# ray-project/anyscale-workshop-nyc-2023

Hardware: NVIDIA H100
Metric: generated tokens/sec (and prompts/sec) FLAN-T5-base 512->128 (higher is better)
Workload: dtype bf16

## Files before the change

### anyscale_workshop_nyc_2023_b200/csrc/b200t5.cu

```cuda
#include <cuda.h>
#include <cuda_bf16.h>
#include <cuda_fp16.h>
#include <cuda_runtime.h>
#include <math.h>
#include <stdarg.h>
#include <stdio.h>
#include <string.h>

#include <map>
#include <memory>
#include <string>
#include <vector>

#include "../../include/b200t5.h"
#include "attention_decode.cuh"
#include "attention_cross_stream.cuh"
#include "attention_encoder.cuh"
#include "elementwise.cuh"
#include "gemm.cuh"
#include "gemm_splitk.cuh"
#include "gemm_2cta.cuh"

using namespace b200;

static thread_local char g_err[512] = "";
static void set_gerr(const char* fmt, ...) {
  va_list ap;
  va_start(ap, fmt);
  vsnprintf(g_err, sizeof(g_err), fmt, ap);
  va_end(ap);
}

struct b200t5_ctx;
static int fail(b200t5_ctx* h, int code, const char* fmt, ...);

#define CU_OK(h, expr)                                                                         \
  do {                                                                                         \
    cudaError_t _e = (expr);                                                                   \
    if (_e != cudaSuccess)                                                                     \
      return fail(h, B200T5_ECUDA, "%s failed: %s (%s:%d)", #expr, cudaGetErrorString(_e), __FILE__, __LINE__); \
  } while (0)

typedef CUresult (*PFN_encodeTiled)(CUtensorMap*, CUtensorMapDataType, cuuint32_t, void*, const cuuint64_t*,
                                    const cuuint64_t*, const cuuint32_t*, const cuuint32_t*, CUtensorMapInterleave,
                                    CUtensorMapSwizzle, CUtensorMapL2promotion, CUtensorMapFloatOOBfill);
static PFN_encodeTiled get_encode_fn() {
  static PFN_encodeTiled fn = nullptr;
  if (!fn) {
    void* p = nullptr;
    cudaDriverEntryPointQueryResult q;
    if (cudaGetDriverEntryPoint("cuTensorMapEncodeTiled", &p, cudaEnableDefault, &q) == cudaSuccess &&
        q == cudaDriverEntryPointSuccess)
      fn = reinterpret_cast<PFN_encodeTiled>(p);
  }
  return fn;
}
static bool make_tmap(CUtensorMap* tm, const void* base, uint64_t rows, uint64_t cols, uint32_t box_rows, bool f32 = false) {
  PFN_encodeTiled enc = get_encode_fn();
  if (!enc) {
    set_gerr("cuTensorMapEncodeTiled entry point not available");
    return false;
  }
  cuuint64_t dims[2] = {cols, rows};
  cuuint64_t strides[1] = {cols * (f32 ? 4u : 2u)};
  cuuint32_t box[2] = {f32 ? 32u : 64u, box_rows};
  cuuint32_t estr[2] = {1, 1};
  const CUtensorMapDataType dt = f32 ? CU_TENSOR_MAP_DATA_TYPE_FLOAT32
                                     : (B200T5_F16 ? CU_TENSOR_MAP_DATA_TYPE_FLOAT16 : CU_TENSOR_MAP_DATA_TYPE_BFLOAT16);
  CUresult r = enc(tm, dt, 2, const_cast<void*>(base), dims, strides, box, estr,
                   CU_TENSOR_MAP_INTERLEAVE_NONE, CU_TENSOR_MAP_SWIZZLE_128B, CU_TENSOR_MAP_L2_PROMOTION_L2_256B,
                   CU_TENSOR_MAP_FLOAT_OOB_FILL_NONE);
  if (r != CUDA_SUCCESS) {
    set_gerr("cuTensorMapEncodeTiled failed with %d (rows=%llu cols=%llu box_rows=%u base=%p)", (int)r,
             (unsigned long long)rows, (unsigned long long)cols, box_rows, base);
    return false;
  }
  return true;
}

DEVINL float load_as_float(const void* src, int dtype, size_t i) {
  if (dtype == B200T5_DTYPE_F32) return reinterpret_cast<const float*>(src)[i];
  if (dtype == B200T5_DTYPE_F16) return __half2float(reinterpret_cast<const __half*>(src)[i]);
  return __bfloat162float(reinterpret_cast<const __nv_bfloat16*>(src)[i]);
}
__global__ void convert_to_act_kernel(const void* src, int dtype, act_t* dst, size_t n) {
  size_t i = blockIdx.x * static_cast<size_t>(blockDim.x) + threadIdx.x;
  const size_t stride = static_cast<size_t>(gridDim.x) * blockDim.x;
  for (; i < n; i += stride) dst[i] = float2act(load_as_float(src, dtype, i));
}
#if B200T5_F16
__global__ void convert_to_f32_kernel(const void* src, int dtype, float* dst, size_t n) {
  size_t i = blockIdx.x * static_cast<size_t>(blockDim.x) + threadIdx.x;
  const size_t stride = static_cast<size_t>(gridDim.x) * blockDim.x;
  for (; i < n; i += stride) dst[i] = load_as_float(src, dtype, i);
}
DEVINL float tf32_rn(float x) {
  uint32_t u = __float_as_uint(x);
  u += 0x0FFFu + ((u >> 13) & 1u);
  return __uint_as_float(u & 0xFFFFE000u);
}
__global__ void split_tf32_kernel(const float* __restrict__ w, float* __restrict__ out, int rows, int K, int Kp) {
  size_t i = blockIdx.x * static_cast<size_t>(blockDim.x) + threadIdx.x;
  const size_t n = static_cast<size_t>(rows) * Kp;
  if (i >= n) return;
  const int r = static_cast<int>(i / Kp), k = static_cast<int>(i % Kp);
  const float v = k < K ? w[static_cast<size_t>(r) * K + k] : 0.f;
  const float hi = tf32_rn(v);
  out[static_cast<size_t>(r) * 2 * Kp + k] = hi;
  out[static_cast<size_t>(r) * 2 * Kp + Kp + k] = tf32_rn(v - hi);
}
#endif
__global__ void geglu_elementwise_kernel(const act_t* gate, const act_t* up, act_t* out, long long n, int mode, GeluLut lut) {
  long long i = blockIdx.x * static_cast<long long>(blockDim.x) + threadIdx.x;
  if (i >= n) return;
  const float x = act2float(gate[i]);
  const float g = mode == 0 ? gelu_from_lut(x, lut.table, lut.lo, lut.hi) : gelu_new_act_exact(x, mode == 1 ? 1 : 0);
  out[i] = float2act(g * act2float(up[i]));
}
__global__ void build_gelu_table_kernel(uint16_t* full, int pow_mode) {
  const uint32_t bits = blockIdx.x * blockDim.x + threadIdx.x;
  if (bits >= 65536u) return;
  const float g = gelu_new_act_exact(__uint_as_float(bits << 16), pow_mode);
  full[bits] = static_cast<uint16_t>(__float_as_uint(g) >> 16);
}
__global__ void set_state_kernel(DecodeState* st, int step) {
  st->step = step;
  st->finished_rows = 0;
}

struct Cfg {
  int V, d, F, H, I, Le, Ld, nb, maxdist;
  float eps;
  int pad, eos, start;
};

struct DevBuf {
  void* p = nullptr;
  size_t bytes = 0;
  ~DevBuf() {
    if (p) cudaFree(p);
  }
  DevBuf() = default;
  DevBuf(const DevBuf&) = delete;
  DevBuf& operator=(const DevBuf&) = delete;
  DevBuf(DevBuf&& o) noexcept : p(o.p), bytes(o.bytes) {
    o.p = nullptr;
    o.bytes = 0;
  }
  cudaError_t alloc(size_t n) {
    if (p) cudaFree(p);
    p = nullptr;
    bytes = n;
    return cudaMalloc(&p, n ? n : 16);
  }
  template <class T>
  T* as() const {
    return reinterpret_cast<T*>(p);
  }
};

enum GemmKind { G_STORE256, G_RES256, G_GEGLU256, G_CROSSKV256, G_QKVDEC64, G_STORE32, G_RES32, G_GEGLU64, G_ARGMAX128, G_LOGITS128 };

struct GemmOp {
  CUtensorMap tmA, tmB;
  int M = 0, N = 0, K = 0;
  GemmKind kind = G_STORE256;
  int m_fastest = 0;
};

struct EncLayerW {
  DevBuf ln0, ln1, wqkv, wo, wi, wff_o;
  CUtensorMap tm_qkv, tm_o, tm_wi, tm_ffo;
  CUtensorMap tm2_qkv, tm2_o, tm2_wi, tm2_ffo;
};
struct DecLayerW {
  DevBuf ln0, ln1, ln2, wqkv, wo, wcq, wco, wi, wff_o;
  CUtensorMap tm_qkv, tm_o, tm_cq, tm_co, tm_wi, tm_ffo;
  int wi_rows = 0;
};

constexpr int kMaxChains = 8;
constexpr int kStepsPerGraph = 8;

struct Plan {
  int B = 0, S = 0, Tmax = 0;
  DevBuf x, xn, qkv, ctx, hff;
  DevBuf key_ok, extent, enc_bias;
  DevBuf cu, row_b, row_s;
  int* h_cu = nullptr;
  int packed_rows = 0;
  bool packed = false;
  DevBuf cross_kv;
  DevBuf dx, dxn, dq, dctx, dh;
  DevBuf self_kv;
  DevBuf dec_bias;
  DevBuf pval, pidx;
  DevBuf state, unfinished, out_ids, out_len, ids_dev, mask_dev;
  DevBuf live_extent, live_key_ok;
  DevBuf xs_stamps, xs_acc;
  DevBuf pos, out_row, admit;
  DevBuf stream_out, stream_len;
  size_t stream_cap = 0;
  bool stream_mode = false;
  int g_stream = -1;
  int g_xattn = -1;
  bool xattn_stream = false;
  long long rows_valid = 0;
  int* h_unf = nullptr;
  int* h_admit = nullptr;
  int n_vtiles = 0;
  CUtensorMap tm_xn, tm_ctx, tm_hff;
  CUtensorMap tm_cross_kv;
  struct Chain {
    int b0 = 0, nb = 0;
    CUtensorMap tm_dxn, tm_dctx, tm_dh;
  };
  int n_chains = 1;
  Chain chains[kMaxChains];
  cudaGraph_t graph = nullptr;
  cudaGraphExec_t gexec = nullptr;
  int graph_nodes = 0;
  cudaGraph_t graph8 = nullptr;
  cudaGraphExec_t gexec8 = nullptr;
  long long g_eos = -1, g_pad = -1;
  int g_min_new = -1;
  long long* h_ids = nullptr;
  long long* h_mask = nullptr;
  long long* h_out = nullptr;
  int* h_len = nullptr;
  DecodeState* h_state = nullptr;
  ~Plan() {
    if (gexec) cudaGraphExecDestroy(gexec);
    if (graph) cudaGraphDestroy(graph);
    if (gexec8) cudaGraphExecDestroy(gexec8);
    if (graph8) cudaGraphDestroy(graph8);
    if (h_ids) cudaFreeHost(h_ids);
    if (h_mask) cudaFreeHost(h_mask);
    if (h_out) cudaFreeHost(h_out);
    if (h_len) cudaFreeHost(h_len);
    if (h_state) cudaFreeHost(h_state);
    if (h_cu) cudaFreeHost(h_cu);
    if (h_unf) cudaFreeHost(h_unf);
    if (h_admit) cudaFreeHost(h_admit);
  }
};

struct b200t5_ctx {
  Cfg c;
  int device = 0;
  int num_sms = 132;
  bool finalized = false;
  int ffo_k = 0;
  char err[512] = "";
  std::map<std::string, std::unique_ptr<DevBuf>> raw;
  std::map<std::string, std::unique_ptr<DevBuf>> raw_f32;
  std::map<std::string, std::vector<int64_t>> raw_shape;
  DevBuf shared, lm_head, enc_final_ln, dec_final_ln, enc_relbias, dec_relbias, wcrosskv;
  CUtensorMap tm_lm, tm_crosskv, tm2_crosskv;
  std::vector<float> enc_relbias_h, dec_relbias_h;
  std::vector<EncLayerW> enc;
  std::vector<DecLayerW> dec;
  std::unique_ptr<Plan> plan;
  cudaStream_t cap_stream = nullptr, exec_stream = nullptr, enc_stream = nullptr;
  cudaEvent_t enc_done_ev = nullptr, admitted_ev = nullptr;
  bool admit_overlap = true;
  cudaEvent_t ev[4] = {nullptr, nullptr, nullptr, nullptr};
  bool ev_valid = false;
  int pow_mode = 0;
  bool use_pdl = true;
  GeluLut gelu_lut{nullptr, 0, 0};
  struct SkChoice {
    int bn, split;
  };
  bool pack_rows = true;
  bool use_2cta = true;
  bool self_block = true;
  int xattn_mode = 2;
  int xs_stages = 5;
  bool xs_late_pdl = true;
  bool xs_l2_prefetch = false;
  bool xattn_serialize = false;
  std::vector<cudaEvent_t> xattn_ev;
  bool profile_xattn = false;
  int small_prio = 0;
  bool sk_on = true;
  int sk_stages64 = 0, sk_stages128 = 0;
  SkChoice sk_qkv{64, 2}, sk_proj{64, 4}, sk_wi{128, 2}, sk_ffo{64, 4};
  int chains_override = 0;
  cudaStream_t chain_streams[kMaxChains] = {};
  cudaEvent_t chain_ev[kMaxChains + 1] = {};
  int64_t launches = 0;
  int last_steps = 0;
  double last_decode_bytes = 0, last_enc_flops = 0;
};

static int fail(b200t5_ctx* h, int code, const char* fmt, ...) {
  char buf[512];
  va_list ap;
  va_start(ap, fmt);
  vsnprintf(buf, sizeof(buf), fmt, ap);
  va_end(ap);
  if (h) snprintf(h->err, sizeof(h->err), "%s", buf);
  snprintf(g_err, sizeof(g_err), "%s", buf);
  return code;
}

static int check_device(b200t5_ctx* h, int device) {
  int n = 0;
  cudaError_t e = cudaGetDeviceCount(&n);
  if (e != cudaSuccess || n <= 0)
    return fail(h, B200T5_ENODEV, "no CUDA device available (%s); libb200t5 has no CPU fallback",
                e == cudaSuccess ? "count=0" : cudaGetErrorString(e));
  if (device < 0 || device >= n) return fail(h, B200T5_EINVAL, "device %d out of range (%d devices)", device, n);
  cudaDeviceProp p;
  CU_OK(h, cudaGetDeviceProperties(&p, device));
  if (p.major != 9)
    return fail(h, B200T5_ENODEV, "device %d is sm_%d%d; libb200t5 is built for sm_90a only", device, p.major, p.minor);
  CU_OK(h, cudaSetDevice(device));
  return p.multiProcessorCount;
}

extern "C" int b200t5_relative_bucket(int rel, int bidirectional, int num_buckets, int max_distance) {
  int ret = 0, n;
  if (bidirectional) {
    num_buckets /= 2;
    if (rel > 0) ret += num_buckets;
    n = rel < 0 ? -rel : rel;
  } else {
    n = rel < 0 ? -rel : 0;
  }
  const int max_exact = num_buckets / 2;
  if (n < max_exact) return ret + n;
  const float ratio = static_cast<float>(n) / static_cast<float>(max_exact);
  const float denom = static_cast<float>(log(static_cast<double>(max_distance) / static_cast<double>(max_exact)));
  const float scaled = logf(ratio) / denom * static_cast<float>(num_buckets - max_exact);
  int large = max_exact + static_cast<int>(scaled);
  if (large > num_buckets - 1) large = num_buckets - 1;
  return ret + large;
}

static cudaError_t run_gemm(b200t5_ctx* h, const GemmOp& g, const void* ep, cudaStream_t s, bool pdl = false) {
  h->launches++;
  switch (g.kind) {
    case G_STORE256:
      return launch_gemm<256, EpiStore>(g.tmA, g.tmB, g.M, g.N, g.K, g.m_fastest, *static_cast<const EpiStore::Params*>(ep), h->num_sms, s, pdl);
    case G_RES256:
      return launch_gemm<256, EpiResidual>(g.tmA, g.tmB, g.M, g.N, g.K, g.m_fastest, *static_cast<const EpiResidual::Params*>(ep), h->num_sms, s, pdl);
    case G_GEGLU256:
      return launch_gemm<256, EpiGeglu>(g.tmA, g.tmB, g.M, g.N, g.K, g.m_fastest, *static_cast<const EpiGeglu::Params*>(ep), h->num_sms, s, pdl);
    case G_CROSSKV256:
      return launch_gemm<256, EpiCrossKV>(g.tmA, g.tmB, g.M, g.N, g.K, g.m_fastest, *static_cast<const EpiCrossKV::Params*>(ep), h->num_sms, s, pdl);
    case G_QKVDEC64:
      return launch_gemm<64, EpiQkvDecode>(g.tmA, g.tmB, g.M, g.N, g.K, g.m_fastest, *static_cast<const EpiQkvDecode::Params*>(ep), h->num_sms, s, pdl);
    case G_STORE32:
      return launch_gemm<32, EpiStore>(g.tmA, g.tmB, g.M, g.N, g.K, g.m_fastest, *static_cast<const EpiStore::Params*>(ep), h->num_sms, s, pdl);
    case G_RES32:
      return launch_gemm<32, EpiResidual>(g.tmA, g.tmB, g.M, g.N, g.K, g.m_fastest, *static_cast<const EpiResidual::Params*>(ep), h->num_sms, s, pdl);
    case G_GEGLU64:
      return launch_gemm<64, EpiGeglu>(g.tmA, g.tmB, g.M, g.N, g.K, g.m_fastest, *static_cast<const EpiGeglu::Params*>(ep), h->num_sms, s, pdl);
    case G_ARGMAX128:
      return launch_gemm<128, EpiArgmax>(g.tmA, g.tmB, g.M, g.N, g.K, g.m_fastest, *static_cast<const EpiArgmax::Params*>(ep), h->num_sms, s, pdl);
    case G_LOGITS128:
      return launch_gemm<128, EpiStoreF32>(g.tmA, g.tmB, g.M, g.N, g.K, g.m_fastest, *static_cast<const EpiStoreF32::Params*>(ep), h->num_sms, s, pdl);
  }
  return cudaErrorInvalidValue;
}

template <class Epi>
static cudaError_t run_gemm_2cta(b200t5_ctx* h, const CUtensorMap& tmA, const CUtensorMap& tmB, int M, int N, int K,
                                 const typename Epi::Params& ep, cudaStream_t s) {
  h->launches++;
  return launch_gemm_2cta<Epi>(tmA, tmB, M, N, K, ep, h->num_sms, s);
}

template <class Epi>
static cudaError_t run_gemm_sk(b200t5_ctx* h, const b200t5_ctx::SkChoice& ch, const CUtensorMap& tmA,
                               const CUtensorMap& tmB, int M, int N, int K, const typename Epi::Params& ep,
                               cudaStream_t s, bool pdl) {
  h->launches++;
  const int split = splitk_factor(K, ch.split);
  if (ch.bn == 128) return launch_gemm_splitk<128, Epi>(tmA, tmB, M, N, K, split, ep, s, pdl, 0, h->sk_stages128);
  return launch_gemm_splitk<64, Epi>(tmA, tmB, M, N, K, split, ep, s, pdl, 0, h->sk_stages64);
}

static cudaError_t run_ffo_2cta(b200t5_ctx* h, const CUtensorMap& tmA, const CUtensorMap& tmB, int M, int N,
                                const EpiResidual::Params& ep, cudaStream_t s) {
  h->launches++;
  return launch_gemm_2cta<EpiResidual, B200T5_F16 != 0>(tmA, tmB, M, N, h->ffo_k, ep, h->num_sms, s, B200T5_F16 ? h->ffo_k / 64 : 0);
}
static cudaError_t run_ffo_sk(b200t5_ctx* h, const b200t5_ctx::SkChoice& ch, const CUtensorMap& tmA, const CUtensorMap& tmB,
                              int M, int N, const EpiResidual::Params& ep, cudaStream_t s, bool pdl) {
  h->launches++;
  constexpr bool tf = B200T5_F16 != 0;
  const int split = splitk_factor(h->ffo_k, ch.split, tf ? kBK / 2 : kBK);
  const int akb = tf ? h->ffo_k / 64 : 0;
  if (ch.bn == 128) return launch_gemm_splitk<128, EpiResidual, tf>(tmA, tmB, M, N, h->ffo_k, split, ep, s, pdl, akb, h->sk_stages128);
  return launch_gemm_splitk<64, EpiResidual, tf>(tmA, tmB, M, N, h->ffo_k, split, ep, s, pdl, akb, h->sk_stages64);
}

static cudaError_t run_rmsnorm(b200t5_ctx* h, const res_t* x, const act_t* w, act_t* y, int M, int d, float eps,
                               cudaStream_t s, bool pdl = false) {
  if (h) h->launches++;
  const int wpb = 8;
  const int grid = (M + wpb - 1) / wpb;
  if (d <= 1024) return launch_kernel(rmsnorm_kernel<4>, dim3(grid), dim3(wpb * 32), 0, s, pdl, x, w, y, M, d, eps);
  if (d <= 4096) return launch_kernel(rmsnorm_kernel<16>, dim3(grid), dim3(wpb * 32), 0, s, pdl, x, w, y, M, d, eps);
  return cudaErrorInvalidValue;
}

static cudaError_t init_kernel_attrs() {
  cudaError_t e;
#define PREP(BN, EPI)                         \
  if ((e = prepare_gemm<BN, EPI>()) != cudaSuccess) return e;
  PREP(256, EpiStore) PREP(256, EpiResidual) PREP(256, EpiGeglu) PREP(256, EpiCrossKV) PREP(64, EpiQkvDecode)
  PREP(32, EpiStore) PREP(32, EpiResidual) PREP(64, EpiGeglu) PREP(128, EpiArgmax) PREP(128, EpiStoreF32)
  PREP(64, EpiStore) PREP(128, EpiStore)
#undef PREP
  if ((e = prepare_gemm_2cta<EpiStore>()) != cudaSuccess) return e;
  if ((e = prepare_gemm_2cta<EpiResidual>()) != cudaSuccess) return e;
  if ((e = prepare_gemm_2cta<EpiGeglu>()) != cudaSuccess) return e;
  if ((e = prepare_gemm_2cta<EpiCrossKV>()) != cudaSuccess) return e;
#define PREPSK(BN, EPI) \
  if ((e = prepare_gemm_splitk<BN, EPI>()) != cudaSuccess) return e;
  PREPSK(64, EpiStore) PREPSK(128, EpiStore) PREPSK(64, EpiResidual) PREPSK(128, EpiResidual)
  PREPSK(64, EpiQkvDecode) PREPSK(128, EpiQkvDecode) PREPSK(64, EpiGeglu) PREPSK(128, EpiGeglu)
#undef PREPSK
  if ((e = prepare_gemm_2cta<EpiResidual, B200T5_F16 != 0>()) != cudaSuccess) return e;
  if ((e = prepare_gemm_splitk<64, EpiResidual, B200T5_F16 != 0>()) != cudaSuccess) return e;
  if ((e = prepare_gemm_splitk<128, EpiResidual, B200T5_F16 != 0>()) != cudaSuccess) return e;
  if ((e = cudaFuncSetAttribute(self_attn_decode_warp_kernel, cudaFuncAttributeMaxDynamicSharedMemorySize,
                                kSelfWarpsPerCta * 4096 * 4)) != cudaSuccess)
    return e;
  if ((e = cudaFuncSetAttribute(attn_cross_stream_kernel, cudaFuncAttributeMaxDynamicSharedMemorySize,
                                static_cast<int>(XsSmem::bytes(kXsMaxStages, 4096)))) != cudaSuccess)
    return e;
  return cudaFuncSetAttribute(encoder_attn_kernel, cudaFuncAttributeMaxDynamicSharedMemorySize, 96 * 1024);
}

struct GeluLutOwner {
  DevBuf table;
  GeluLut lut{nullptr, 0, 0};
  int pow_mode = -1;
};
static GeluLutOwner g_gelu;

[[maybe_unused]] static int ensure_gelu_lut(b200t5_ctx* h, int pow_mode, GeluLut* out) {
  if (g_gelu.lut.table && g_gelu.pow_mode == pow_mode) {
    *out = g_gelu.lut;
    return B200T5_OK;
  }
  DevBuf full;
  CU_OK(h, full.alloc(65536 * 2));
  build_gelu_table_kernel<<<256, 256>>>(full.as<uint16_t>(), pow_mode);
  CU_OK(h, cudaGetLastError());
  std::vector<uint16_t> t(65536);
  CU_OK(h, cudaMemcpy(t.data(), full.p, 65536 * 2, cudaMemcpyDeviceToHost));
  auto half_bits = [](uint16_t xb) {
    uint32_t u = static_cast<uint32_t>(xb) << 16;
    float f;
    memcpy(&f, &u, 4);
    f *= 0.5f;
    memcpy(&u, &f, 4);
    u += 0x7FFFu + ((u >> 16) & 1u);
    return static_cast<uint16_t>(u >> 16);
  };
  int lo = 0;
  while (lo < 0x7F80 && t[lo] == half_bits(static_cast<uint16_t>(lo)) && t[0x8000 | lo] == half_bits(static_cast<uint16_t>(0x8000 | lo))) ++lo;
  int hi = 0x7F80;
  while (hi > lo && t[hi - 1] == static_cast<uint16_t>(hi - 1) && t[0x8000 | (hi - 1)] == 0x8000) --hi;
  const int n = hi - lo;
  if (n < 0 || 2 * n * 2 > kEpiSmemBytes) return fail(h, B200T5_ECUDA, "gelu table window [%#x,%#x) does not fit the epilogue scratch", lo, hi);
  std::vector<uint16_t> compact(((static_cast<size_t>(2) * (n > 0 ? n : 1) + 7) / 8) * 8 + 8, 0);
  for (int i = 0; i < n; ++i) {
    compact[i] = t[lo + i];
    compact[n + i] = t[0x8000 | (lo + i)];
  }
  CU_OK(h, g_gelu.table.alloc(compact.size() * 2));
  CU_OK(h, cudaMemcpy(g_gelu.table.p, compact.data(), compact.size() * 2, cudaMemcpyHostToDevice));
  g_gelu.lut = GeluLut{g_gelu.table.as<uint16_t>(), lo, hi};
  g_gelu.pow_mode = pow_mode;
  *out = g_gelu.lut;
  return B200T5_OK;
}

extern "C" const char* b200t5_version(void) {
  return B200T5_F16 ? "b200t5 0.1 fp16 (sm_90a, wgmma/TMA)" : "b200t5 0.1 (sm_90a, wgmma/TMA)";
}
extern "C" const char* b200t5_last_global_error(void) { return g_err; }
extern "C" const char* b200t5_last_error(b200t5_handle h) { return h ? h->err : g_err; }

extern "C" int b200t5_create(const b200t5_config* cfg, int device, b200t5_handle* out) {
  if (!cfg || !out) return fail(nullptr, B200T5_EINVAL, "null argument");
  *out = nullptr;
  if (cfg->d_kv != 64) return fail(nullptr, B200T5_EINVAL, "d_kv=%d unsupported (kernels are specialised for 64)", cfg->d_kv);
  if (!cfg->is_gated_gelu) return fail(nullptr, B200T5_EINVAL, "only feed_forward_proj='gated-gelu' (T5 v1.1 / FLAN-T5) is supported");
  if (cfg->scale_decoder_outputs) return fail(nullptr, B200T5_EINVAL, "scale_decoder_outputs (tied-embedding T5 v1.0) is not supported");
  if (cfg->d_model % 8 || cfg->d_ff % 32 || cfg->d_model > 4096 || cfg->vocab_size < 2 || cfg->num_heads < 1 ||
      cfg->num_layers < 1 || cfg->num_decoder_layers < 1)
    return fail(nullptr, B200T5_EINVAL, "unsupported shape: d_model=%d d_ff=%d vocab=%d", cfg->d_model, cfg->d_ff, cfg->vocab_size);
  int sms = check_device(nullptr, device);
  if (sms < 0) return sms;
  b200t5_ctx* h = new (std::nothrow) b200t5_ctx();
  if (!h) return fail(nullptr, B200T5_ENOMEM, "out of host memory");
  h->c = Cfg{cfg->vocab_size, cfg->d_model, cfg->d_ff, cfg->num_heads, cfg->num_heads * 64, cfg->num_layers,
             cfg->num_decoder_layers, cfg->relative_attention_num_buckets, cfg->relative_attention_max_distance,
             cfg->layer_norm_epsilon, cfg->pad_token_id, cfg->eos_token_id, cfg->decoder_start_token_id};
  h->device = device;
  h->num_sms = sms;
  h->enc.resize(h->c.Le);
  h->dec.resize(h->c.Ld);
  const char* pm = getenv("B200T5_POW_MODE");
  h->pow_mode = pm ? atoi(pm) : 0;
  const char* pdl_env = getenv("B200T5_PDL");
  h->use_pdl = pdl_env ? atoi(pdl_env) != 0 : true;
  if (const char* pr_env = getenv("B200T5_PRIO")) h->small_prio = atoi(pr_env);
  if (const char* pk_env = getenv("B200T5_PACK")) h->pack_rows = atoi(pk_env) != 0;
  if (const char* tc_env = getenv("B200T5_2CTA")) h->use_2cta = atoi(tc_env) != 0;
  if (const char* sf_env = getenv("B200T5_SELF")) h->self_block = strcmp(sf_env, "warp") != 0;
  if (const char* xa_env = getenv("B200T5_XATTN")) h->xattn_mode = strcmp(xa_env, "ldg") == 0 ? 0 : strcmp(xa_env, "stream") == 0 ? 1 : 2;
  if (const char* xs_env = getenv("B200T5_XS_STAGES")) {
    const int v = atoi(xs_env);
    if (v >= 2 && v <= kXsMaxStages) h->xs_stages = v;
  }
  if (const char* lp_env = getenv("B200T5_XS_LATE_PDL")) h->xs_late_pdl = atoi(lp_env) != 0;
  if (const char* se_env = getenv("B200T5_XS_SERIALIZE")) h->xattn_serialize = atoi(se_env) != 0;
  if (const char* pf_env = getenv("B200T5_XS_L2PF")) h->xs_l2_prefetch = atoi(pf_env) != 0;
  if (const char* sk_env = getenv("B200T5_SK")) {
    int v[8];
    const int n = sscanf(sk_env, "%d,%d,%d,%d,%d,%d,%d,%d", &v[0], &v[1], &v[2], &v[3], &v[4], &v[5], &v[6], &v[7]);
    if (n == 1 && v[0] == 0) h->sk_on = false;
    if (n == 8) {
      b200t5_ctx::SkChoice* dst[4] = {&h->sk_qkv, &h->sk_proj, &h->sk_wi, &h->sk_ffo};
      for (int i = 0; i < 4; ++i) {
        dst[i]->bn = v[2 * i] == 128 ? 128 : 64;
        dst[i]->split = v[2 * i + 1] >= 8 ? 8 : (v[2 * i + 1] >= 4 ? 4 : (v[2 * i + 1] >= 2 ? 2 : 1));
      }
    }
  }
  if (const char* st_env = getenv("B200T5_SK_STAGES")) {
    int a = 0, b = 0;
    if (sscanf(st_env, "%d,%d", &a, &b) == 2) {
      h->sk_stages64 = a;
      h->sk_stages128 = b;
    }
  }
  const char* ch_env = getenv("B200T5_CHAINS");
  h->chains_override = ch_env ? atoi(ch_env) : 0;
#if B200T5_F16
  h->use_2cta = h->pack_rows = true;
  if (!h->sk_on) {
    delete h;
    return fail(nullptr, B200T5_EINVAL, "B200T5_SK=0 is not available in the fp16 build");
  }
#endif
  if (const char* ao_env = getenv("B200T5_ADMIT_OVERLAP")) h->admit_overlap = atoi(ao_env) != 0;
  int prio_lo = 0, prio_hi = 0;
  cudaDeviceGetStreamPriorityRange(&prio_lo, &prio_hi);
  if (cudaStreamCreateWithFlags(&h->cap_stream, cudaStreamNonBlocking) != cudaSuccess ||
      cudaStreamCreateWithFlags(&h->exec_stream, cudaStreamNonBlocking) != cudaSuccess ||
      cudaStreamCreateWithPriority(&h->enc_stream, cudaStreamNonBlocking, prio_lo) != cudaSuccess ||
      cudaEventCreateWithFlags(&h->enc_done_ev, cudaEventDisableTiming) != cudaSuccess ||
      cudaEventCreateWithFlags(&h->admitted_ev, cudaEventDisableTiming) != cudaSuccess) {
    delete h;
    return fail(nullptr, B200T5_ECUDA, "cudaStreamCreate failed");
  }
  {
    cudaError_t ke = init_kernel_attrs();
    if (ke != cudaSuccess) {
      delete h;
      return fail(nullptr, B200T5_ECUDA, "kernel attribute setup failed: %s", cudaGetErrorString(ke));
    }
  }
#if !B200T5_F16
  {
    int lrc = ensure_gelu_lut(nullptr, h->pow_mode, &h->gelu_lut);
    if (lrc != B200T5_OK) {
      delete h;
      return lrc;
    }
  }
#endif
  {
    cudaError_t ce = cudaSuccess;
    for (int i = 0; i < 4 && ce == cudaSuccess; ++i) ce = cudaEventCreate(&h->ev[i]);
    for (int i = 0; i < kMaxChains && ce == cudaSuccess; ++i) ce = cudaStreamCreateWithFlags(&h->chain_streams[i], cudaStreamNonBlocking);
    for (int i = 0; i <= kMaxChains && ce == cudaSuccess; ++i) ce = cudaEventCreateWithFlags(&h->chain_ev[i], cudaEventDisableTiming);
    if (ce != cudaSuccess) {
      b200t5_destroy(h);
      return fail(nullptr, B200T5_ECUDA, "stream/event creation failed: %s", cudaGetErrorString(ce));
    }
  }
  *out = h;
  return B200T5_OK;
}

extern "C" int b200t5_destroy(b200t5_handle h) {
  if (!h) return B200T5_OK;
  cudaSetDevice(h->device);
  cudaDeviceSynchronize();
  h->plan.reset();
  if (h->cap_stream) cudaStreamDestroy(h->cap_stream);
  if (h->exec_stream) cudaStreamDestroy(h->exec_stream);
  if (h->enc_stream) cudaStreamDestroy(h->enc_stream);
  if (h->enc_done_ev) cudaEventDestroy(h->enc_done_ev);
  if (h->admitted_ev) cudaEventDestroy(h->admitted_ev);
  for (int i = 0; i < kMaxChains; ++i)
    if (h->chain_streams[i]) cudaStreamDestroy(h->chain_streams[i]);
  for (int i = 0; i <= kMaxChains; ++i)
    if (h->chain_ev[i]) cudaEventDestroy(h->chain_ev[i]);
  for (cudaEvent_t e : h->xattn_ev)
    if (e) cudaEventDestroy(e);
  for (int i = 0; i < 4; ++i)
    if (h->ev[i]) cudaEventDestroy(h->ev[i]);
  delete h;
  return B200T5_OK;
}

extern "C" int b200t5_set_weight(b200t5_handle h, const char* name, const void* dev_ptr, int dtype,
                                 const int64_t* shape, int ndim) {
  if (!h || !name || !dev_ptr || !shape || ndim < 1 || ndim > 2) return fail(h, B200T5_EINVAL, "set_weight: bad argument");
  if (h->finalized) return fail(h, B200T5_ESTATE, "set_weight after finalize");
  if (dtype < 0 || dtype > 2) return fail(h, B200T5_EINVAL, "set_weight(%s): unknown dtype %d", name, dtype);
  CU_OK(h, cudaSetDevice(h->device));
  size_t n = 1;
  std::vector<int64_t> shp(shape, shape + ndim);
  for (int i = 0; i < ndim; ++i) {
    if (shape[i] <= 0) return fail(h, B200T5_EINVAL, "set_weight(%s): bad shape", name);
    n *= static_cast<size_t>(shape[i]);
  }
  std::unique_ptr<DevBuf> buf(new DevBuf());
  CU_OK(h, buf->alloc(n * sizeof(act_t)));
  if (dtype == (B200T5_F16 ? B200T5_DTYPE_F16 : B200T5_DTYPE_BF16)) {
    CU_OK(h, cudaMemcpy(buf->p, dev_ptr, n * sizeof(act_t), cudaMemcpyDeviceToDevice));
  } else {
    convert_to_act_kernel<<<1024, 256>>>(dev_ptr, dtype, buf->as<act_t>(), n);
    CU_OK(h, cudaGetLastError());
    CU_OK(h, cudaDeviceSynchronize());
  }
  h->raw[name] = std::move(buf);
  h->raw_shape[name] = shp;
#if B200T5_F16
  {
    const std::string nm(name);
    const std::string suffix = "DenseReluDense.wo.weight";
    if (nm.size() >= suffix.size() && nm.compare(nm.size() - suffix.size(), suffix.size(), suffix) == 0) {
      std::unique_ptr<DevBuf> f(new DevBuf());
      CU_OK(h, f->alloc(n * 4));
      convert_to_f32_kernel<<<1024, 256>>>(dev_ptr, dtype, f->as<float>(), n);
      CU_OK(h, cudaGetLastError());
      CU_OK(h, cudaDeviceSynchronize());
      h->raw_f32[nm] = std::move(f);
    }
  }
#endif
  return B200T5_OK;
}

static act_t* take(b200t5_ctx* h, const std::string& name, int64_t r, int64_t c, int* rc) {
  auto it = h->raw.find(name);
  if (it == h->raw.end()) {
    *rc = fail(h, B200T5_ESTATE, "finalize: missing weight '%s'", name.c_str());
    return nullptr;
  }
  const auto& s = h->raw_shape[name];
  const bool ok = (c == 0) ? (s.size() == 1 && s[0] == r) : (s.size() == 2 && s[0] == r && s[1] == c);
  if (!ok) {
    *rc = fail(h, B200T5_EINVAL, "finalize: weight '%s' has the wrong shape", name.c_str());
    return nullptr;
  }
  return it->second->as<act_t>();
}

static int interleave_geglu(b200t5_ctx* h, const act_t* wi0, const act_t* wi1, DevBuf& dst, int F, int d, int bn,
                            int* rows_out) {
  const int half = bn / 2;
  const int ntiles = (F + half - 1) / half;
  CU_OK(h, dst.alloc(static_cast<size_t>(ntiles) * bn * d * sizeof(act_t)));
  CU_OK(h, cudaMemset(dst.p, 0, dst.bytes));
  for (int j = 0; j < ntiles; ++j) {
    const int rows = (j + 1) * half <= F ? half : F - j * half;
    act_t* base = dst.as<act_t>() + static_cast<size_t>(j) * bn * d;
    CU_OK(h, cudaMemcpy(base, wi0 + static_cast<size_t>(j) * half * d, static_cast<size_t>(rows) * d * sizeof(act_t), cudaMemcpyDeviceToDevice));
    CU_OK(h, cudaMemcpy(base + static_cast<size_t>(half) * d, wi1 + static_cast<size_t>(j) * half * d, static_cast<size_t>(rows) * d * sizeof(act_t), cudaMemcpyDeviceToDevice));
  }
  *rows_out = ntiles * bn;
  return B200T5_OK;
}

static int build_ffo(b200t5_ctx* h, DevBuf& dst, const std::string& name, const act_t* src2, int d, int F, int* k_cols) {
#if B200T5_F16
  auto it = h->raw_f32.find(name);
  if (it == h->raw_f32.end()) return fail(h, B200T5_ESTATE, "finalize: missing fp32 copy of '%s'", name.c_str());
  const int Fp = (F + 31) / 32 * 32;
  CU_OK(h, dst.alloc(static_cast<size_t>(d) * 2 * Fp * 4));
  const size_t n = static_cast<size_t>(d) * Fp;
  split_tf32_kernel<<<static_cast<unsigned>((n + 255) / 256), 256>>>(it->second->as<float>(), dst.as<float>(), d, F, Fp);
  CU_OK(h, cudaGetLastError());
  CU_OK(h, cudaDeviceSynchronize());
  *k_cols = 2 * Fp;
  (void)src2;
  return B200T5_OK;
#else
  *k_cols = F;
  CU_OK(h, dst.alloc(static_cast<size_t>(d) * F * sizeof(act_t)));
  CU_OK(h, cudaMemcpy(dst.p, src2, static_cast<size_t>(d) * F * sizeof(act_t), cudaMemcpyDeviceToDevice));
  return B200T5_OK;
#endif
}

static int clone_buf(b200t5_ctx* h, DevBuf& dst, const act_t* src, size_t n) {
  CU_OK(h, dst.alloc(n * sizeof(act_t)));
  CU_OK(h, cudaMemcpy(dst.p, src, n * sizeof(act_t), cudaMemcpyDeviceToDevice));
  return B200T5_OK;
}

#define TRY(expr)            \
  do {                       \
    int _rc = (expr);        \
    if (_rc != B200T5_OK) return _rc; \
  } while (0)
#define TMAP(h, tm, base, rows, cols, box) \
  do {                                     \
    if (!make_tmap(tm, base, rows, cols, box)) return fail(h, B200T5_ECUDA, "%s", g_err); \
  } while (0)
#define TMAP_FFO(h, tm, base, rows, cols, box) \
  do {                                         \
    if (!make_tmap(tm, base, rows, cols, box, B200T5_F16 != 0)) return fail(h, B200T5_ECUDA, "%s", g_err); \
  } while (0)

extern "C" int b200t5_finalize(b200t5_handle h) {
  if (!h) return fail(nullptr, B200T5_EINVAL, "null handle");
  if (h->finalized) return B200T5_OK;
  CU_OK(h, cudaSetDevice(h->device));
  const Cfg& c = h->c;
  int rc = B200T5_OK;
  const int d = c.d, I = c.I, F = c.F;

  act_t* shared = take(h, "shared.weight", c.V, d, &rc);
  if (!shared) return rc;
  TRY(clone_buf(h, h->shared, shared, static_cast<size_t>(c.V) * d));
  const act_t* lm = h->raw.count("lm_head.weight") ? take(h, "lm_head.weight", c.V, d, &rc) : shared;
  if (!lm) return rc;
  TRY(clone_buf(h, h->lm_head, lm, static_cast<size_t>(c.V) * d));
  TMAP(h, &h->tm_lm, h->lm_head.p, c.V, d, 128);

  act_t* p;
  if (!(p = take(h, "encoder.final_layer_norm.weight", d, 0, &rc))) return rc;
  TRY(clone_buf(h, h->enc_final_ln, p, d));
  if (!(p = take(h, "decoder.final_layer_norm.weight", d, 0, &rc))) return rc;
  TRY(clone_buf(h, h->dec_final_ln, p, d));

  for (int side = 0; side < 2; ++side) {
    const std::string nm = std::string(side ? "decoder" : "encoder") + ".block.0.layer.0.SelfAttention.relative_attention_bias.weight";
    if (!(p = take(h, nm, c.nb, c.H, &rc))) return rc;
    std::vector<act_t> tmp(static_cast<size_t>(c.nb) * c.H);
    CU_OK(h, cudaMemcpy(tmp.data(), p, tmp.size() * sizeof(act_t), cudaMemcpyDeviceToHost));
    std::vector<float>& dst = side ? h->dec_relbias_h : h->enc_relbias_h;
    dst.resize(tmp.size());
    for (size_t i = 0; i < tmp.size(); ++i) dst[i] = act2float(tmp[i]);
  }

  char nm[256];
  for (int l = 0; l < c.Le; ++l) {
    EncLayerW& w = h->enc[l];
    auto key = [&](const char* suffix) {
      snprintf(nm, sizeof(nm), "encoder.block.%d.%s", l, suffix);
      return std::string(nm);
    };
    if (!(p = take(h, key("layer.0.layer_norm.weight"), d, 0, &rc))) return rc;
    TRY(clone_buf(h, w.ln0, p, d));
    if (!(p = take(h, key("layer.1.layer_norm.weight"), d, 0, &rc))) return rc;
    TRY(clone_buf(h, w.ln1, p, d));
    const act_t* q = take(h, key("layer.0.SelfAttention.q.weight"), I, d, &rc);
    const act_t* k = q ? take(h, key("layer.0.SelfAttention.k.weight"), I, d, &rc) : nullptr;
    const act_t* v = k ? take(h, key("layer.0.SelfAttention.v.weight"), I, d, &rc) : nullptr;
    if (!v) return rc;
    CU_OK(h, w.wqkv.alloc(static_cast<size_t>(3) * I * d * sizeof(act_t)));
    const size_t blk = static_cast<size_t>(I) * d;
    CU_OK(h, cudaMemcpy(w.wqkv.as<act_t>(), q, blk * 2, cudaMemcpyDeviceToDevice));
    CU_OK(h, cudaMemcpy(w.wqkv.as<act_t>() + blk, k, blk * 2, cudaMemcpyDeviceToDevice));
    CU_OK(h, cudaMemcpy(w.wqkv.as<act_t>() + 2 * blk, v, blk * 2, cudaMemcpyDeviceToDevice));
    if (!(p = take(h, key("layer.0.SelfAttention.o.weight"), d, I, &rc))) return rc;
    TRY(clone_buf(h, w.wo, p, static_cast<size_t>(d) * I));
    const act_t* wi0 = take(h, key("layer.1.DenseReluDense.wi_0.weight"), F, d, &rc);
    const act_t* wi1 = wi0 ? take(h, key("layer.1.DenseReluDense.wi_1.weight"), F, d, &rc) : nullptr;
    if (!wi1) return rc;
    int wi_rows = 0;
    TRY(interleave_geglu(h, wi0, wi1, w.wi, F, d, 256, &wi_rows));
    if (!(p = take(h, key("layer.1.DenseReluDense.wo.weight"), d, F, &rc))) return rc;
    TRY(build_ffo(h, w.wff_o, key("layer.1.DenseReluDense.wo.weight"), p, d, F, &h->ffo_k));
    TMAP(h, &w.tm_qkv, w.wqkv.p, 3 * I, d, 256);
    TMAP(h, &w.tm_o, w.wo.p, d, I, 256);
    TMAP(h, &w.tm_wi, w.wi.p, wi_rows, d, 256);
    TMAP_FFO(h, &w.tm_ffo, w.wff_o.p, d, h->ffo_k, 256);
    TMAP(h, &w.tm2_qkv, w.wqkv.p, 3 * I, d, 128);
    TMAP(h, &w.tm2_o, w.wo.p, d, I, 128);
    TMAP(h, &w.tm2_wi, w.wi.p, wi_rows, d, 128);
    TMAP_FFO(h, &w.tm2_ffo, w.wff_o.p, d, h->ffo_k, 128);
  }

  CU_OK(h, h->wcrosskv.alloc(static_cast<size_t>(c.Ld) * 2 * I * d * sizeof(act_t)));
  for (int l = 0; l < c.Ld; ++l) {
    DecLayerW& w = h->dec[l];
    auto key = [&](const char* suffix) {
      snprintf(nm, sizeof(nm), "decoder.block.%d.%s", l, suffix);
      return std::string(nm);
    };
    if (!(p = take(h, key("layer.0.layer_norm.weight"), d, 0, &rc))) return rc;
    TRY(clone_buf(h, w.ln0, p, d));
    if (!(p = take(h, key("layer.1.layer_norm.weight"), d, 0, &rc))) return rc;
    TRY(clone_buf(h, w.ln1, p, d));
    if (!(p = take(h, key("layer.2.layer_norm.weight"), d, 0, &rc))) return rc;
    TRY(clone_buf(h, w.ln2, p, d));
    const act_t* q = take(h, key("layer.0.SelfAttention.q.weight"), I, d, &rc);
    const act_t* k = q ? take(h, key("layer.0.SelfAttention.k.weight"), I, d, &rc) : nullptr;
    const act_t* v = k ? take(h, key("layer.0.SelfAttention.v.weight"), I, d, &rc) : nullptr;
    if (!v) return rc;
    const size_t blk = static_cast<size_t>(I) * d;
    CU_OK(h, w.wqkv.alloc(3 * blk * sizeof(act_t)));
    CU_OK(h, cudaMemcpy(w.wqkv.as<act_t>(), q, blk * 2, cudaMemcpyDeviceToDevice));
    CU_OK(h, cudaMemcpy(w.wqkv.as<act_t>() + blk, k, blk * 2, cudaMemcpyDeviceToDevice));
    CU_OK(h, cudaMemcpy(w.wqkv.as<act_t>() + 2 * blk, v, blk * 2, cudaMemcpyDeviceToDevice));
    if (!(p = take(h, key("layer.0.SelfAttention.o.weight"), d, I, &rc))) return rc;
    TRY(clone_buf(h, w.wo, p, static_cast<size_t>(d) * I));
    if (!(p = take(h, key("layer.1.EncDecAttention.q.weight"), I, d, &rc))) return rc;
    TRY(clone_buf(h, w.wcq, p, blk));
    const act_t* ck = take(h, key("layer.1.EncDecAttention.k.weight"), I, d, &rc);
    const act_t* cv = ck ? take(h, key("layer.1.EncDecAttention.v.weight"), I, d, &rc) : nullptr;
    if (!cv) return rc;
    CU_OK(h, cudaMemcpy(h->wcrosskv.as<act_t>() + (static_cast<size_t>(l) * 2 + 0) * blk, ck, blk * 2, cudaMemcpyDeviceToDevice));
    CU_OK(h, cudaMemcpy(h->wcrosskv.as<act_t>() + (static_cast<size_t>(l) * 2 + 1) * blk, cv, blk * 2, cudaMemcpyDeviceToDevice));
    if (!(p = take(h, key("layer.1.EncDecAttention.o.weight"), d, I, &rc))) return rc;
    TRY(clone_buf(h, w.wco, p, static_cast<size_t>(d) * I));
    const act_t* wi0 = take(h, key("layer.2.DenseReluDense.wi_0.weight"), F, d, &rc);
    const act_t* wi1 = wi0 ? take(h, key("layer.2.DenseReluDense.wi_1.weight"), F, d, &rc) : nullptr;
    if (!wi1) return rc;
    int wi_rows = 0;
    const int bn_qkv = h->sk_on ? h->sk_qkv.bn : 64, bn_proj = h->sk_on ? h->sk_proj.bn : 32;
    const int bn_wi = h->sk_on ? h->sk_wi.bn : 64, bn_ffo = h->sk_on ? h->sk_ffo.bn : 32;
    TRY(interleave_geglu(h, wi0, wi1, w.wi, F, d, bn_wi, &wi_rows));
    w.wi_rows = wi_rows;
    if (!(p = take(h, key("layer.2.DenseReluDense.wo.weight"), d, F, &rc))) return rc;
    TRY(build_ffo(h, w.wff_o, key("layer.2.DenseReluDense.wo.weight"), p, d, F, &h->ffo_k));
    TMAP(h, &w.tm_qkv, w.wqkv.p, 3 * I, d, bn_qkv);
    TMAP(h, &w.tm_o, w.wo.p, d, I, bn_proj);
    TMAP(h, &w.tm_cq, w.wcq.p, I, d, bn_proj);
    TMAP(h, &w.tm_co, w.wco.p, d, I, bn_proj);
    TMAP(h, &w.tm_wi, w.wi.p, wi_rows, d, bn_wi);
    TMAP_FFO(h, &w.tm_ffo, w.wff_o.p, d, h->ffo_k, bn_ffo);
  }
  TMAP(h, &h->tm_crosskv, h->wcrosskv.p, static_cast<uint64_t>(c.Ld) * 2 * I, d, 256);
  TMAP(h, &h->tm2_crosskv, h->wcrosskv.p, static_cast<uint64_t>(c.Ld) * 2 * I, d, 128);

  h->raw.clear();
  h->raw_f32.clear();
  h->raw_shape.clear();
  h->finalized = true;
  return B200T5_OK;
}


static int build_plan(b200t5_ctx* h, int B, int S, int Tmax) {
  const Cfg& c = h->c;
  std::unique_ptr<Plan> pl(new Plan());
  pl->B = B;
  pl->S = S;
  pl->Tmax = Tmax;
  const size_t M = static_cast<size_t>(B) * S;
  const int d = c.d, I = c.I, F = c.F, H = c.H;
  CU_OK(h, pl->x.alloc(M * d * sizeof(res_t)));
  CU_OK(h, pl->xn.alloc(M * d * 2));
  CU_OK(h, pl->qkv.alloc(M * 3 * I * 2));
  CU_OK(h, pl->ctx.alloc(M * I * 2));
  CU_OK(h, pl->hff.alloc(M * F * sizeof(ffh_t)));
  CU_OK(h, pl->key_ok.alloc(M));
  CU_OK(h, pl->extent.alloc(static_cast<size_t>(B) * 4));
  CU_OK(h, pl->cu.alloc(static_cast<size_t>(B + 1) * 4));
  CU_OK(h, pl->row_b.alloc(M * 4));
  CU_OK(h, pl->row_s.alloc(M * 4));
  CU_OK(h, cudaMallocHost(&pl->h_cu, 16));
  CU_OK(h, pl->cross_kv.alloc(static_cast<size_t>(c.Ld) * 2 * M * I * 2));
  CU_OK(h, cudaMemset(pl->cross_kv.p, 0, pl->cross_kv.bytes));
  CU_OK(h, pl->dx.alloc(static_cast<size_t>(B) * d * sizeof(res_t)));
  CU_OK(h, pl->dxn.alloc(static_cast<size_t>(B) * d * 2));
  CU_OK(h, pl->dq.alloc(static_cast<size_t>(B) * I * 2));
  CU_OK(h, pl->dctx.alloc(static_cast<size_t>(B) * I * 2));
  CU_OK(h, pl->dh.alloc(static_cast<size_t>(B) * F * sizeof(ffh_t)));
  CU_OK(h, pl->self_kv.alloc(static_cast<size_t>(c.Ld) * 2 * B * I * Tmax * 2));
  pl->n_vtiles = (c.V + 127) / 128;
  CU_OK(h, pl->pval.alloc(static_cast<size_t>(B) * pl->n_vtiles * 4));
  CU_OK(h, pl->pidx.alloc(static_cast<size_t>(B) * pl->n_vtiles * 4));
  CU_OK(h, pl->state.alloc(sizeof(DecodeState)));
  CU_OK(h, pl->unfinished.alloc(static_cast<size_t>(B) * 4));
  CU_OK(h, pl->out_ids.alloc(static_cast<size_t>(B) * (Tmax + 1) * 8));
  CU_OK(h, pl->out_len.alloc(static_cast<size_t>(B) * 4));
  CU_OK(h, pl->ids_dev.alloc(M * 8));
  CU_OK(h, pl->mask_dev.alloc(M * 8));
  CU_OK(h, cudaMallocHost(&pl->h_ids, M * 8));
  CU_OK(h, cudaMallocHost(&pl->h_mask, M * 8));
  CU_OK(h, cudaMallocHost(&pl->h_out, static_cast<size_t>(B) * (Tmax + 1) * 8));
  CU_OK(h, cudaMallocHost(&pl->h_len, static_cast<size_t>(B) * 4));
  CU_OK(h, cudaMallocHost(&pl->h_state, sizeof(DecodeState)));
  CU_OK(h, pl->live_extent.alloc(static_cast<size_t>(B) * 4));
  CU_OK(h, pl->live_key_ok.alloc(M));
  CU_OK(h, pl->pos.alloc(static_cast<size_t>(B) * 4));
  CU_OK(h, pl->out_row.alloc(static_cast<size_t>(B) * 4));
  CU_OK(h, pl->admit.alloc(static_cast<size_t>(3) * B * 4));
  CU_OK(h, cudaMemset(pl->pos.p, 0, pl->pos.bytes));
  CU_OK(h, pl->xs_stamps.alloc(static_cast<size_t>(c.Ld) * kMaxChains * 2 * 8));
  CU_OK(h, pl->xs_acc.alloc(static_cast<size_t>(c.Ld) * (kMaxChains + 1) * 2 * 8));
  CU_OK(h, cudaMemset(pl->xs_stamps.p, 0, pl->xs_stamps.bytes));
  CU_OK(h, cudaMemset(pl->xs_acc.p, 0, pl->xs_acc.bytes));
  CU_OK(h, cudaMemset(pl->out_row.p, 0, pl->out_row.bytes));
  CU_OK(h, cudaMallocHost(&pl->h_unf, static_cast<size_t>(B) * 4));
  CU_OK(h, cudaMallocHost(&pl->h_admit, static_cast<size_t>(3) * B * 4));

  {
    std::vector<float> eb(static_cast<size_t>(H) * (2 * S - 1));
    for (int rel = -(S - 1); rel <= S - 1; ++rel) {
      const int bk = b200t5_relative_bucket(rel, 1, c.nb, c.maxdist);
      for (int hh = 0; hh < H; ++hh) eb[static_cast<size_t>(hh) * (2 * S - 1) + rel + S - 1] = h->enc_relbias_h[static_cast<size_t>(bk) * H + hh];
    }
    CU_OK(h, pl->enc_bias.alloc(eb.size() * 4));
    CU_OK(h, cudaMemcpy(pl->enc_bias.p, eb.data(), eb.size() * 4, cudaMemcpyHostToDevice));
    std::vector<float> db(static_cast<size_t>(H) * Tmax);
    for (int n = 0; n < Tmax; ++n) {
      const int bk = b200t5_relative_bucket(-n, 0, c.nb, c.maxdist);
      for (int hh = 0; hh < H; ++hh) db[static_cast<size_t>(hh) * Tmax + n] = h->dec_relbias_h[static_cast<size_t>(bk) * H + hh];
    }
    CU_OK(h, pl->dec_bias.alloc(db.size() * 4));
    CU_OK(h, cudaMemcpy(pl->dec_bias.p, db.data(), db.size() * 4, cudaMemcpyHostToDevice));
  }
  TMAP(h, &pl->tm_xn, pl->xn.p, M, d, 128);
  TMAP(h, &pl->tm_ctx, pl->ctx.p, M, I, 128);
  TMAP_FFO(h, &pl->tm_hff, pl->hff.p, M, F, 128);
  TMAP(h, &pl->tm_cross_kv, pl->cross_kv.p, static_cast<uint64_t>(c.Ld) * 2 * B * H * S, 64, kXsChunkKeys);
  CU_OK(h, cudaMemset(pl->ctx.p, 0, pl->ctx.bytes));
  {
    int nc = B >= 512 ? 4 : (B >= 128 ? 2 : 1);
    if (h->chains_override > 0) nc = h->chains_override;
    if (nc > kMaxChains) nc = kMaxChains;
    if (nc > B) nc = B;
    pl->n_chains = nc;
    for (int i = 0; i < nc; ++i) {
      Plan::Chain& ch = pl->chains[i];
      ch.b0 = static_cast<int>(static_cast<long long>(B) * i / nc);
      ch.nb = static_cast<int>(static_cast<long long>(B) * (i + 1) / nc) - ch.b0;
      TMAP(h, &ch.tm_dxn, pl->dxn.as<act_t>() + static_cast<size_t>(ch.b0) * d, ch.nb, d, 128);
      TMAP(h, &ch.tm_dctx, pl->dctx.as<act_t>() + static_cast<size_t>(ch.b0) * I, ch.nb, I, 128);
      TMAP_FFO(h, &ch.tm_dh, pl->dh.as<ffh_t>() + static_cast<size_t>(ch.b0) * F, ch.nb, F, 128);
    }
  }
  h->plan = std::move(pl);
  return B200T5_OK;
}

static int ensure_plan(b200t5_ctx* h, int B, int S, int Tmax) {
  if (h->plan && h->plan->B == B && h->plan->S == S && h->plan->Tmax == Tmax) return B200T5_OK;
  CU_OK(h, cudaDeviceSynchronize());
  h->plan.reset();
  return build_plan(h, B, S, Tmax);
}

static GemmOp mk(const CUtensorMap& a, const CUtensorMap& b, int M, int N, int K, GemmKind k, int m_fastest) {
  GemmOp g;
  g.tmA = a;
  g.tmB = b;
  g.M = M;
  g.N = N;
  g.K = K;
  g.kind = k;
  g.m_fastest = m_fastest;
  return g;
}

static int run_encoder(b200t5_ctx* h, const long long* ids, const long long* mask, cudaStream_t s, const int* row_on = nullptr) {
  const Cfg& c = h->c;
  Plan& p = *h->plan;
  const int B = p.B, S = p.S, d = c.d, I = c.I, F = c.F, H = c.H;
  int M = B * S;
  prep_mask_kernel<<<B, 128, 0, s>>>(mask, p.key_ok.as<unsigned char>(), p.extent.as<int>(), B, S, row_on);
  h->launches++;
  p.packed = h->pack_rows && S <= kEncPackMaxS;
  if (row_on && !p.packed)
    return fail(h, B200T5_EINVAL, "slot-pool admission needs the packed encoder path (S <= %d, B200T5_PACK at its default)", kEncPackMaxS);
  const int* cu = nullptr;
  p.rows_valid = M;
  if (p.packed) {
    pack_offsets_kernel<<<1, 256, 0, s>>>(p.extent.as<int>(), p.cu.as<int>(), B);
    CU_OK(h, cudaMemcpyAsync(p.h_cu, p.cu.as<int>() + B, 4, cudaMemcpyDeviceToHost, s));
    CU_OK(h, cudaStreamSynchronize(s));
    M = *p.h_cu;
    p.rows_valid = M;
    cu = p.cu.as<int>();
    embed_rows_packed_kernel<<<dim3((S + 7) / 8, B), 256, 0, s>>>(ids, h->shared.as<act_t>(), p.x.as<res_t>(), cu, p.row_b.as<int>(),
                                                               p.row_s.as<int>(), S, d, c.V);
    h->launches += 2;
  } else {
    embed_rows_kernel<<<(M + 7) / 8, 256, 0, s>>>(ids, h->shared.as<act_t>(), p.x.as<res_t>(), M, d, c.V);
    h->launches++;
  }
  p.packed_rows = M;
  CU_OK(h, cudaGetLastError());
  const size_t attn_smem = encoder_attn_smem_bytes(S);
  if (attn_smem > 96 * 1024) return fail(h, B200T5_EINVAL, "encoder length S=%d too long for the attention kernel", S);
  const int wi_tiles = (F + 127) / 128;
  for (int l = 0; l < c.Le; ++l) {
    EncLayerW& w = h->enc[l];
    CU_OK(h, run_rmsnorm(h, p.x.as<res_t>(), w.ln0.as<act_t>(), p.xn.as<act_t>(), M, d, c.eps, s));
    {
      EpiStore::Params ep{p.qkv.as<act_t>(), 3 * I};
      if (h->use_2cta) CU_OK(h, run_gemm_2cta<EpiStore>(h, p.tm_xn, w.tm2_qkv, M, 3 * I, d, ep, s));
      else CU_OK(h, run_gemm(h, mk(p.tm_xn, w.tm_qkv, M, 3 * I, d, G_STORE256, 0), &ep, s));
    }
    encoder_attn_kernel<<<dim3((S + kEncQ - 1) / kEncQ, B * H), kEncThreads, attn_smem, s>>>(
        p.qkv.as<act_t>(), p.ctx.as<act_t>(), p.enc_bias.as<float>(), p.key_ok.as<unsigned char>(), p.extent.as<int>(), cu, S, H);
    h->launches++;
    CU_OK(h, cudaGetLastError());
    {
      EpiResidual::Params ep{p.x.as<res_t>(), p.x.as<res_t>(), d};
      ep.round_out = l == 0;
      if (h->use_2cta) CU_OK(h, run_gemm_2cta<EpiResidual>(h, p.tm_ctx, w.tm2_o, M, d, I, ep, s));
      else CU_OK(h, run_gemm(h, mk(p.tm_ctx, w.tm_o, M, d, I, G_RES256, 0), &ep, s));
    }
    CU_OK(h, run_rmsnorm(h, p.x.as<res_t>(), w.ln1.as<act_t>(), p.xn.as<act_t>(), M, d, c.eps, s));
    {
      EpiGeglu::Params ep{p.hff.as<ffh_t>(), F, h->gelu_lut};
      if (h->use_2cta) CU_OK(h, run_gemm_2cta<EpiGeglu>(h, p.tm_xn, w.tm2_wi, M, wi_tiles * 256, d, ep, s));
      else CU_OK(h, run_gemm(h, mk(p.tm_xn, w.tm_wi, M, wi_tiles * 256, d, G_GEGLU256, 0), &ep, s));
    }
    {
      EpiResidual::Params ep{p.x.as<res_t>(), p.x.as<res_t>(), d};
      ep.round_acc = B200T5_F16 ? 0 : 1;
      ep.round_out = B200T5_F16 ? 0 : 1;
      if (h->use_2cta) CU_OK(h, run_ffo_2cta(h, p.tm_hff, w.tm2_ffo, M, d, ep, s));
      else CU_OK(h, run_gemm(h, mk(p.tm_hff, w.tm_ffo, M, d, F, G_RES256, 0), &ep, s));
    }
  }
  CU_OK(h, run_rmsnorm(h, p.x.as<res_t>(), h->enc_final_ln.as<act_t>(), p.xn.as<act_t>(), M, d, c.eps, s));
  return B200T5_OK;
}

static int run_cross_kv(b200t5_ctx* h, cudaStream_t s) {
  const Cfg& c = h->c;
  Plan& p = *h->plan;
  EpiCrossKV::Params ep{p.cross_kv.as<act_t>(), p.B, c.H, p.S};
  if (p.packed) {
    ep.row_b = p.row_b.as<int>();
    ep.row_s = p.row_s.as<int>();
  }
  const int M = p.packed ? p.packed_rows : p.B * p.S;
  if (h->use_2cta) CU_OK(h, run_gemm_2cta<EpiCrossKV>(h, p.tm_xn, h->tm2_crosskv, M, c.Ld * 2 * c.I, c.d, ep, s));
  else CU_OK(h, run_gemm(h, mk(p.tm_xn, h->tm_crosskv, M, c.Ld * 2 * c.I, c.d, G_CROSSKV256, 0), &ep, s));
  return B200T5_OK;
}

struct ChainView {
  int b0, nb;
  res_t* dx;
  ffh_t* dh;
  act_t *dxn, *dq, *dctx;
  const Plan::Chain* ch;
};
static ChainView chain_view(b200t5_ctx* h, const Plan::Chain& ch) {
  Plan& p = *h->plan;
  const Cfg& c = h->c;
  ChainView v;
  v.b0 = ch.b0;
  v.nb = ch.nb;
  v.dx = p.dx.as<res_t>() + static_cast<size_t>(ch.b0) * c.d;
  v.dxn = p.dxn.as<act_t>() + static_cast<size_t>(ch.b0) * c.d;
  v.dq = p.dq.as<act_t>() + static_cast<size_t>(ch.b0) * c.I;
  v.dctx = p.dctx.as<act_t>() + static_cast<size_t>(ch.b0) * c.I;
  v.dh = p.dh.as<ffh_t>() + static_cast<size_t>(ch.b0) * c.F;
  v.ch = &ch;
  return v;
}

static int chain_layer_pre(b200t5_ctx* h, cudaStream_t s, const ChainView& v, int l) {
  const Cfg& c = h->c;
  Plan& p = *h->plan;
  const int B = p.B, d = c.d, I = c.I, H = c.H, T = p.Tmax;
  const bool pdl = h->use_pdl;
  const int sstride = p.stream_mode ? 1 : 0;
  const int* step = p.stream_mode ? p.pos.as<int>() + v.b0 : &p.state.as<DecodeState>()->step;
  DecLayerW& w = h->dec[l];
  act_t* skv = p.self_kv.as<act_t>() + l * (static_cast<size_t>(2) * B * I * T) + static_cast<size_t>(v.b0) * I * T;
  CU_OK(h, run_rmsnorm(h, v.dx, w.ln0.as<act_t>(), v.dxn, v.nb, d, c.eps, s, pdl));
  {
    EpiQkvDecode::Params ep{v.dq, skv, step, B, H, T, sstride};
    if (h->sk_on) CU_OK(h, run_gemm_sk<EpiQkvDecode>(h, h->sk_qkv, v.ch->tm_dxn, w.tm_qkv, v.nb, 3 * I, d, ep, s, pdl));
    else CU_OK(h, run_gemm(h, mk(v.ch->tm_dxn, w.tm_qkv, v.nb, 3 * I, d, G_QKVDEC64, 1), &ep, s, pdl));
  }
  if (h->self_block)
    CU_OK(h, launch_kernel(attn_decode_kernel<true>, dim3(v.nb * H), dim3(kAttnDecThreads), T * sizeof(float), s, pdl, v.dq, skv,
                           skv + static_cast<size_t>(B) * I * T, v.dctx, H, T, nullptr, nullptr, step, p.dec_bias.as<float>(),
                           XsStamps{nullptr, 0}, sstride));
  else
    CU_OK(h, launch_kernel(self_attn_decode_warp_kernel, dim3((v.nb * H + kSelfWarpsPerCta - 1) / kSelfWarpsPerCta),
                           dim3(kSelfWarpsPerCta * 32), kSelfWarpsPerCta * T * sizeof(float), s, pdl, v.dq, skv,
                           skv + static_cast<size_t>(B) * I * T, v.dctx, v.nb * H, H, T, step, p.dec_bias.as<float>(), sstride));
  h->launches++;
  {
    EpiResidual::Params ep{v.dx, v.dx, d};
    ep.round_out = l == 0;
    if (h->sk_on) CU_OK(h, run_gemm_sk<EpiResidual>(h, h->sk_proj, v.ch->tm_dctx, w.tm_o, v.nb, d, I, ep, s, pdl));
    else CU_OK(h, run_gemm(h, mk(v.ch->tm_dctx, w.tm_o, v.nb, d, I, G_RES32, 1), &ep, s, pdl));
  }
  CU_OK(h, run_rmsnorm(h, v.dx, w.ln1.as<act_t>(), v.dxn, v.nb, d, c.eps, s, pdl));
  {
    EpiStore::Params ep{v.dq, I};
    if (h->sk_on) CU_OK(h, run_gemm_sk<EpiStore>(h, h->sk_proj, v.ch->tm_dxn, w.tm_cq, v.nb, I, d, ep, s, pdl));
    else CU_OK(h, run_gemm(h, mk(v.ch->tm_dxn, w.tm_cq, v.nb, I, d, G_STORE32, 1), &ep, s, pdl));
  }
  return B200T5_OK;
}

static cudaError_t launch_cross_attention(b200t5_ctx* h, cudaStream_t s, bool pdl, int l, int b0, int nb, const act_t* q,
                                          act_t* ctx, const int* ext, const unsigned char* ok, int slot) {
  const Cfg& c = h->c;
  Plan& p = *h->plan;
  const int B = p.B, S = p.S, I = c.I;
  XsStamps st{slot >= 0 && p.xs_stamps.p ? p.xs_stamps.as<unsigned long long>() : nullptr, slot >= 0 ? slot : 0};
  if (p.xattn_stream) {
    const int items = nb * c.H;
    const int k_row0 = ((l * 2) * B + b0) * c.H * S, v_row0 = ((l * 2 + 1) * B + b0) * c.H * S;
    const act_t* arena = p.cross_kv.as<act_t>();
    return launch_kernel(attn_cross_stream_kernel, dim3(xs_grid(items, h->num_sms)), dim3(kXsThreads),
                         XsSmem::bytes(h->xs_stages, S), s, pdl, p.tm_cross_kv, p.tm_cross_kv, k_row0, v_row0,
                         arena + static_cast<size_t>(k_row0) * 64, arena + static_cast<size_t>(v_row0) * 64, q, ctx, items, c.H, S,
                         ext, ok, h->xs_stages, h->xs_late_pdl ? 1 : 0, h->xs_l2_prefetch ? 1 : 0, st);
  }
  const act_t* kplane = p.cross_kv.as<act_t>() + l * (static_cast<size_t>(2) * B * I * S) + static_cast<size_t>(b0) * I * S;
  return launch_kernel(attn_decode_kernel<false>, dim3(nb * c.H), dim3(kAttnDecThreads), S * sizeof(float), s, pdl, q, kplane,
                       kplane + static_cast<size_t>(B) * I * S, ctx, c.H, S, ext, ok, nullptr, nullptr, st, 0);
}

static int chain_layer_cross(b200t5_ctx* h, cudaStream_t s, const ChainView& v, int l, int chain_index, bool pdl) {
  Plan& p = *h->plan;
  const int S = p.S;
  struct PrioGuard {
    int saved;
    PrioGuard() : saved(launch_priority()) { launch_priority() = 0; }
    ~PrioGuard() { launch_priority() = saved; }
  } guard;
  CU_OK(h, launch_cross_attention(h, s, pdl, l, v.b0, v.nb, v.dq, v.dctx, p.live_extent.as<int>() + v.b0,
                                  p.live_key_ok.as<unsigned char>() + static_cast<size_t>(v.b0) * S,
                                  h->profile_xattn ? l * p.n_chains + chain_index : -1));
  h->launches++;
  return B200T5_OK;
}

static int chain_layer_post(b200t5_ctx* h, cudaStream_t s, const ChainView& v, int l) {
  const Cfg& c = h->c;
  const int d = c.d, I = c.I, F = c.F;
  const bool pdl = h->use_pdl;
  const int wi_tiles = (F + 31) / 32;
  DecLayerW& w = h->dec[l];
  {
    EpiResidual::Params ep{v.dx, v.dx, d};
    ep.round_out = l == 0;
    if (h->sk_on) CU_OK(h, run_gemm_sk<EpiResidual>(h, h->sk_proj, v.ch->tm_dctx, w.tm_co, v.nb, d, I, ep, s, pdl));
    else CU_OK(h, run_gemm(h, mk(v.ch->tm_dctx, w.tm_co, v.nb, d, I, G_RES32, 1), &ep, s, pdl));
  }
  CU_OK(h, run_rmsnorm(h, v.dx, w.ln2.as<act_t>(), v.dxn, v.nb, d, c.eps, s, pdl));
  {
    EpiGeglu::Params ep{v.dh, F, h->gelu_lut};
    if (h->sk_on) CU_OK(h, run_gemm_sk<EpiGeglu>(h, h->sk_wi, v.ch->tm_dxn, w.tm_wi, v.nb, w.wi_rows, d, ep, s, pdl));
    else CU_OK(h, run_gemm(h, mk(v.ch->tm_dxn, w.tm_wi, v.nb, wi_tiles * 64, d, G_GEGLU64, 1), &ep, s, pdl));
  }
  {
    EpiResidual::Params ep{v.dx, v.dx, d};
    ep.round_acc = B200T5_F16 ? 0 : 1;
    ep.round_out = B200T5_F16 ? 0 : 1;
    if (h->sk_on) CU_OK(h, run_ffo_sk(h, h->sk_ffo, v.ch->tm_dh, w.tm_ffo, v.nb, d, ep, s, pdl));
    else CU_OK(h, run_gemm(h, mk(v.ch->tm_dh, w.tm_ffo, v.nb, d, F, G_RES32, 1), &ep, s, pdl));
  }
  return B200T5_OK;
}

static int chain_head(b200t5_ctx* h, cudaStream_t s, const ChainView& v, float* logits_out, int ldl, long long eos,
                      long long pad, int min_new) {
  const Cfg& c = h->c;
  Plan& p = *h->plan;
  const int d = c.d, T = p.Tmax;
  const bool pdl = h->use_pdl;
  DecodeState* st = p.state.as<DecodeState>();
  CU_OK(h, run_rmsnorm(h, v.dx, h->dec_final_ln.as<act_t>(), v.dxn, v.nb, d, c.eps, s, pdl));
  if (logits_out) {
    EpiStoreF32::Params ep{logits_out + static_cast<size_t>(v.b0) * ldl, ldl};
    CU_OK(h, run_gemm(h, mk(v.ch->tm_dxn, h->tm_lm, v.nb, c.V, d, G_LOGITS128, 1), &ep, s, pdl));
  } else {
    float* pval = p.pval.as<float>() + static_cast<size_t>(v.b0) * p.n_vtiles;
    int* pidx = p.pidx.as<int>() + static_cast<size_t>(v.b0) * p.n_vtiles;
    const bool sm = p.stream_mode;
    EpiArgmax::Params ep{pval, pidx, p.n_vtiles, sm ? p.pos.as<int>() + v.b0 : &st->step, static_cast<int>(eos), min_new, sm ? 1 : 0};
    CU_OK(h, run_gemm(h, mk(v.ch->tm_dxn, h->tm_lm, v.nb, c.V, d, G_ARGMAX128, 1), &ep, s, pdl));
    long long* oid = sm ? p.stream_out.as<long long>() : p.out_ids.as<long long>() + static_cast<size_t>(v.b0) * (T + 1);
    int* olen = sm ? p.stream_len.as<int>() : p.out_len.as<int>() + v.b0;
    CU_OK(h, launch_kernel(finalize_step_kernel, dim3(v.nb), dim3(128), 0, s, pdl, pval, pidx, p.n_vtiles, st,
                           p.unfinished.as<int>() + v.b0, oid, olen, T + 1, eos, pad, h->shared.as<act_t>(), v.dx, d,
                           p.live_extent.as<int>() + v.b0, sm ? p.pos.as<int>() + v.b0 : static_cast<int*>(nullptr),
                           sm ? p.out_row.as<int>() + v.b0 : static_cast<const int*>(nullptr), T));
    h->launches++;
  }
  return B200T5_OK;
// ... 414 lines not shown
                                               p.key_ok.as<unsigned char>() + static_cast<size_t>(b0) * p.S, -1);
        if (e != cudaSuccess) le = e;
        ++launches;
      }
    }
  };
  sweep();
  CU_OK(h, le);
  cudaEvent_t e0 = nullptr, e1 = nullptr;
  struct EvGuard {
    cudaEvent_t &a, &b;
    ~EvGuard() {
      if (a) cudaEventDestroy(a);
      if (b) cudaEventDestroy(b);
    }
  } guard{e0, e1};
  CU_OK(h, cudaEventCreate(&e0));
  CU_OK(h, cudaEventCreate(&e1));
  CU_OK(h, cudaEventRecord(e0, s));
  for (int r = 0; r < reps; ++r) sweep();
  CU_OK(h, cudaEventRecord(e1, s));
  CU_OK(h, cudaEventSynchronize(e1));
  CU_OK(h, le);
  float ms = 0.f;
  CU_OK(h, cudaEventElapsedTime(&ms, e0, e1));
  CU_OK(h, cudaGetLastError());
  *avg_ms_per_launch = ms / (static_cast<float>(reps) * launches);
  std::vector<int> ext(p.B);
  CU_OK(h, cudaMemcpy(ext.data(), p.extent.p, p.B * 4, cudaMemcpyDeviceToHost));
  double sum_s = 0;
  for (int v : ext) sum_s += v;
  *bytes_per_launch = 2.0 * 2.0 * c.I * sum_s / (static_cast<double>(launches) / c.Ld);
  return B200T5_OK;
}

extern "C" int b200t5_set_option(b200t5_handle h, const char* name, int value) {
  if (!h || !name) return fail(h, B200T5_EINVAL, "null argument");
  const std::string n(name);
  if (n == "chains") h->chains_override = value < 0 ? 0 : value;
  else if (n == "xattn") h->xattn_mode = value < 0 || value > 2 ? 2 : value;
  else if (n == "xattn_stages") {
    if (value < 2 || value > kXsMaxStages) return fail(h, B200T5_EINVAL, "xattn_stages must be in [2, %d]", kXsMaxStages);
    h->xs_stages = value;
  } else if (n == "xattn_late_pdl") h->xs_late_pdl = value != 0;
  else if (n == "xattn_serialize") h->xattn_serialize = value != 0;
  else if (n == "xattn_l2pf") h->xs_l2_prefetch = value != 0;
  else if (n == "pdl") h->use_pdl = value != 0;
  else if (n == "admit_overlap") h->admit_overlap = value != 0;
  else if (n == "sk_stages64") h->sk_stages64 = value;
  else if (n == "sk_stages128") h->sk_stages128 = value;
  else if (n == "profile_xattn") h->profile_xattn = value != 0;
  else return fail(h, B200T5_EINVAL, "unknown option '%s'", name);
  CU_OK(h, cudaSetDevice(h->device));
  CU_OK(h, cudaDeviceSynchronize());
  h->plan.reset();
  return B200T5_OK;
}

extern "C" int b200t5_get_xattn_profile(b200t5_handle h, double* avg_us_per_launch, int64_t* launches, double* bytes_per_launch,
                                        double* busy_us_per_layer, double* bytes_per_layer) {
  if (!h || !avg_us_per_launch || !launches || !bytes_per_launch || !busy_us_per_layer || !bytes_per_layer)
    return fail(h, B200T5_EINVAL, "null argument");
  if (!h->plan || !h->profile_xattn) return fail(h, B200T5_ESTATE, "profiling is off (b200t5_set_option(h, \"profile_xattn\", 1), then generate)");
  CU_OK(h, cudaSetDevice(h->device));
  CU_OK(h, cudaDeviceSynchronize());
  Plan& p = *h->plan;
  const int n = h->c.Ld * p.n_chains;
  std::vector<unsigned long long> acc(static_cast<size_t>(n + h->c.Ld) * 2);
  CU_OK(h, cudaMemcpy(acc.data(), p.xs_acc.p, acc.size() * 8, cudaMemcpyDeviceToHost));
  unsigned long long ns = 0, cnt = 0, busy = 0, layers = 0;
  for (int i = 0; i < n; ++i) {
    ns += acc[2 * i];
    cnt += acc[2 * i + 1];
  }
  for (int l = 0; l < h->c.Ld; ++l) {
    busy += acc[2 * (n + l)];
    layers += acc[2 * (n + l) + 1];
  }
  *avg_us_per_launch = cnt ? static_cast<double>(ns) / static_cast<double>(cnt) / 1e3 : 0.0;
  *busy_us_per_layer = layers ? static_cast<double>(busy) / static_cast<double>(layers) / 1e3 : 0.0;
  *launches = static_cast<int64_t>(cnt);
  std::vector<int> ext(p.B);
  CU_OK(h, cudaMemcpy(ext.data(), p.extent.p, p.B * 4, cudaMemcpyDeviceToHost));
  double sum_s = 0;
  for (int v : ext) sum_s += v;
  *bytes_per_layer = 2.0 * 2.0 * h->c.I * sum_s;
  *bytes_per_launch = *bytes_per_layer / p.n_chains;
  return B200T5_OK;
}

extern "C" int b200t5_encode(b200t5_handle h, const int64_t* input_ids, const int64_t* attention_mask, int B, int S,
                             void* enc_out_bf16, void* stream) {
  TRY(validate(h, B, S, nullptr));
  if (!input_ids || !enc_out_bf16) return fail(h, B200T5_EINVAL, "null argument");
  CU_OK(h, cudaSetDevice(h->device));
  cudaStream_t s = static_cast<cudaStream_t>(stream);
  const int T = h->plan && h->plan->B == B && h->plan->S == S ? h->plan->Tmax : 1;
  TRY(ensure_plan(h, B, S, T));
  TRY(run_encoder(h, reinterpret_cast<const long long*>(input_ids), reinterpret_cast<const long long*>(attention_mask), s));
  if (h->plan->packed) {
    unpack_rows_kernel<<<dim3((S + 7) / 8, B), 256, 0, s>>>(h->plan->xn.as<act_t>(), h->plan->cu.as<int>(), static_cast<act_t*>(enc_out_bf16), S, h->c.d);
    CU_OK(h, cudaGetLastError());
  } else {
    CU_OK(h, cudaMemcpyAsync(enc_out_bf16, h->plan->xn.p, static_cast<size_t>(B) * S * h->c.d * 2, cudaMemcpyDeviceToDevice, s));
  }
  return B200T5_OK;
}

extern "C" int b200t5_decode_logits(b200t5_handle h, const int64_t* input_ids, const int64_t* attention_mask, int B,
                                    int S, const int64_t* decoder_input_ids, int T, float* logits, void* stream) {
  TRY(validate(h, B, S, nullptr));
  if (!input_ids || !decoder_input_ids || !logits || T < 1) return fail(h, B200T5_EINVAL, "bad argument");
  CU_OK(h, cudaSetDevice(h->device));
  cudaStream_t s = static_cast<cudaStream_t>(stream);
  TRY(ensure_plan(h, B, S, T));
  Plan& p = *h->plan;
  const Cfg& c = h->c;
  TRY(run_encoder(h, reinterpret_cast<const long long*>(input_ids), reinterpret_cast<const long long*>(attention_mask), s));
  TRY(run_cross_kv(h, s));
  p.stream_mode = false;
  p.xattn_stream = pick_xattn(h, static_cast<double>(p.rows_valid) / (static_cast<double>(B) * S)) != 0;
  CU_OK(h, cudaMemcpyAsync(p.live_extent.p, p.extent.p, static_cast<size_t>(B) * 4, cudaMemcpyDeviceToDevice, s));
  CU_OK(h, cudaMemcpyAsync(p.live_key_ok.p, p.key_ok.p, static_cast<size_t>(B) * S, cudaMemcpyDeviceToDevice, s));
  set_state_kernel<<<1, 1, 0, s>>>(p.state.as<DecodeState>(), 0);
  DevBuf col;
  CU_OK(h, col.alloc(static_cast<size_t>(B) * 8));
  for (int t = 0; t < T; ++t) {
    CU_OK(h, cudaMemcpy2DAsync(col.p, 8, reinterpret_cast<const long long*>(decoder_input_ids) + t, static_cast<size_t>(T) * 8, 8, B, cudaMemcpyDeviceToDevice, s));
    force_token_kernel<<<B, 128, 0, s>>>(col.as<long long>(), h->shared.as<act_t>(), p.dx.as<res_t>(), c.d);
    TRY(run_decode_step(h, s, false, logits + static_cast<size_t>(t) * c.V, T * c.V, c.eos, c.pad, 0));
  }
  CU_OK(h, cudaStreamSynchronize(s));
  return B200T5_OK;
}

[[maybe_unused]] static int hook_device(int device) {
  int sms = check_device(nullptr, device);
  if (sms < 0) return sms;
  cudaError_t e = init_kernel_attrs();
  if (e != cudaSuccess) return fail(nullptr, B200T5_ECUDA, "kernel attribute setup failed: %s", cudaGetErrorString(e));
  return sms;
}

extern "C" int b200t5_test_gemm(int device, const void* A, const void* W, void* C, int M, int N, int K, int bn, int mode,
                                int pow_mode, void* stream) {
#if B200T5_F16
  return fail(nullptr, B200T5_EINVAL, "the single-kernel test hooks exist in the bf16 build only (libb200t5.so)");
#else
  const int sms = hook_device(device);
  if (sms < 0) return sms;
  if (K % 8) return fail(nullptr, B200T5_EINVAL, "K must be a multiple of 8");
  cudaStream_t s = static_cast<cudaStream_t>(stream);
  CUtensorMap ta, tb;
  if (!make_tmap(&ta, A, M, K, 128) || !make_tmap(&tb, W, N, K, bn == 512 ? 128 : bn)) return fail(nullptr, B200T5_ECUDA, "%s", g_err);
  b200t5_ctx dummy;
  dummy.num_sms = sms;
  cudaError_t e = cudaErrorInvalidValue;
  act_t* Cb = static_cast<act_t*>(C);
  if (bn == 512) {
    if (mode == 0) {
      EpiStore::Params ep{Cb, N};
      e = run_gemm_2cta<EpiStore>(&dummy, ta, tb, M, N, K, ep, s);
    } else if (mode == 1) {
      EpiResidual::Params ep{Cb, Cb, N};
      e = run_gemm_2cta<EpiResidual>(&dummy, ta, tb, M, N, K, ep, s);
    } else if (mode == 2) {
      GeluLut lut;
      int lrc = ensure_gelu_lut(nullptr, pow_mode, &lut);
      if (lrc != B200T5_OK) return lrc;
      EpiGeglu::Params ep{Cb, N / 2, lut};
      e = run_gemm_2cta<EpiGeglu>(&dummy, ta, tb, M, N, K, ep, s);
    }
    if (e != cudaSuccess) return fail(nullptr, B200T5_ECUDA, "test_gemm(pair, mode=%d): %s", mode, cudaGetErrorString(e));
    return B200T5_OK;
  }
  if (mode == 0) {
    EpiStore::Params ep{Cb, N};
    if (bn == 256) e = run_gemm(&dummy, mk(ta, tb, M, N, K, G_STORE256, 0), &ep, s);
    else if (bn == 32) e = run_gemm(&dummy, mk(ta, tb, M, N, K, G_STORE32, 1), &ep, s);
    else if (bn == 64) e = launch_gemm<64, EpiStore>(ta, tb, M, N, K, 0, ep, sms, s);
    else if (bn == 128) e = launch_gemm<128, EpiStore>(ta, tb, M, N, K, 0, ep, sms, s);
  } else if (mode == 1) {
    EpiResidual::Params ep{Cb, Cb, N};
    if (bn == 256) e = run_gemm(&dummy, mk(ta, tb, M, N, K, G_RES256, 0), &ep, s);
    else if (bn == 32) e = run_gemm(&dummy, mk(ta, tb, M, N, K, G_RES32, 1), &ep, s);
  } else if (mode == 2) {
    GeluLut lut;
    int lrc = ensure_gelu_lut(nullptr, pow_mode, &lut);
    if (lrc != B200T5_OK) return lrc;
    EpiGeglu::Params ep{Cb, N / 2, lut};
    if (bn == 256) e = run_gemm(&dummy, mk(ta, tb, M, N, K, G_GEGLU256, 0), &ep, s);
    else if (bn == 64) e = run_gemm(&dummy, mk(ta, tb, M, N, K, G_GEGLU64, 1), &ep, s);
  } else if (mode == 3) {
    EpiStoreF32::Params ep{static_cast<float*>(C), N};
    if (bn == 128) e = run_gemm(&dummy, mk(ta, tb, M, N, K, G_LOGITS128, 1), &ep, s);
  }
  if (e != cudaSuccess) return fail(nullptr, B200T5_ECUDA, "test_gemm(bn=%d, mode=%d): %s", bn, mode, cudaGetErrorString(e));
  return B200T5_OK;
#endif
}

extern "C" int b200t5_test_lm_argmax(int device, const void* x, const void* W, int M, int V, int K, int step, int eos,
                                     int min_new, int64_t* tokens, void* stream) {
  const int sms = hook_device(device);
  if (sms < 0) return sms;
  if (!x || !W || !tokens || M < 1 || V < 2 || K % 8 || step < 0) return fail(nullptr, B200T5_EINVAL, "test_lm_argmax: bad argument");
  cudaStream_t s = static_cast<cudaStream_t>(stream);
  CUtensorMap ta, tb;
  if (!make_tmap(&ta, x, M, K, 128) || !make_tmap(&tb, W, V, K, 128)) return fail(nullptr, B200T5_ECUDA, "%s", g_err);
  const int n_tiles = (V + 127) / 128, out_ld = step + 2;
  DevBuf pval, pidx, st, unf, out, len, xn, ext;
  if (pval.alloc(static_cast<size_t>(M) * n_tiles * 4) != cudaSuccess || pidx.alloc(static_cast<size_t>(M) * n_tiles * 4) != cudaSuccess ||
      st.alloc(sizeof(DecodeState)) != cudaSuccess || unf.alloc(static_cast<size_t>(M) * 4) != cudaSuccess ||
      out.alloc(static_cast<size_t>(M) * out_ld * 8) != cudaSuccess || len.alloc(static_cast<size_t>(M) * 4) != cudaSuccess ||
      xn.alloc(static_cast<size_t>(M) * K * sizeof(res_t)) != cudaSuccess || ext.alloc(static_cast<size_t>(M) * 4) != cudaSuccess)
    return fail(nullptr, B200T5_ENOMEM, "test_lm_argmax: allocation failed");
  b200t5_ctx dummy;
  dummy.num_sms = sms;
  decode_init_kernel<<<M, 128, 0, s>>>(st.as<DecodeState>(), unf.as<int>(), out.as<long long>(), len.as<int>(), out_ld, M, 0, 0,
                                       static_cast<const act_t*>(W), xn.as<res_t>(), K);
  set_state_kernel<<<1, 1, 0, s>>>(st.as<DecodeState>(), step);
  EpiArgmax::Params ep{pval.as<float>(), pidx.as<int>(), n_tiles, &st.as<DecodeState>()->step, eos, min_new, 0};
  cudaError_t e = run_gemm(&dummy, mk(ta, tb, M, V, K, G_ARGMAX128, 1), &ep, s, false);
  if (e == cudaSuccess)
    e = launch_kernel(finalize_step_kernel, dim3(M), dim3(128), 0, s, false, pval.as<float>(), pidx.as<int>(), n_tiles, st.as<DecodeState>(),
                      unf.as<int>(), out.as<long long>(), len.as<int>(), out_ld, static_cast<long long>(-1), static_cast<long long>(0),
                      static_cast<const act_t*>(W), xn.as<res_t>(), K, ext.as<int>(), static_cast<int*>(nullptr),
                      static_cast<const int*>(nullptr), 1 << 30);
  if (e == cudaSuccess)
    e = cudaMemcpy2DAsync(tokens, 8, out.as<long long>() + step + 1, static_cast<size_t>(out_ld) * 8, 8, M, cudaMemcpyDeviceToDevice, s);
  if (e == cudaSuccess) e = cudaStreamSynchronize(s);
  if (e != cudaSuccess) return fail(nullptr, B200T5_ECUDA, "test_lm_argmax: %s", cudaGetErrorString(e));
  return B200T5_OK;
}

extern "C" int b200t5_test_gemm_splitk(int device, const void* A, const void* W, void* C, int M, int N, int K, int bn,
                                       int split, int mode, int pow_mode, void* aux, int Tmax, int step, void* stream) {
#if B200T5_F16
  return fail(nullptr, B200T5_EINVAL, "the single-kernel test hooks exist in the bf16 build only (libb200t5.so)");
#else
  const int sms = hook_device(device);
  if (sms < 0) return sms;
  if (K % 8) return fail(nullptr, B200T5_EINVAL, "K must be a multiple of 8");
  cudaStream_t s = static_cast<cudaStream_t>(stream);
  if ((bn != 64 && bn != 128) || (split != 1 && split != 2 && split != 4 && split != 8))
    return fail(nullptr, B200T5_EINVAL, "test_gemm_splitk: bn in {64,128}, split in {1,2,4,8}");
  CUtensorMap ta, tb;
  if (!make_tmap(&ta, A, M, K, 128) || !make_tmap(&tb, W, N, K, bn)) return fail(nullptr, B200T5_ECUDA, "%s", g_err);
  b200t5_ctx dummy;
  dummy.num_sms = sms;
  b200t5_ctx::SkChoice ch{bn, split};
  cudaError_t e = cudaErrorInvalidValue;
  act_t* Cb = static_cast<act_t*>(C);
  DevBuf st;
  if (mode == 0) {
    EpiStore::Params ep{Cb, N};
    e = run_gemm_sk<EpiStore>(&dummy, ch, ta, tb, M, N, K, ep, s, false);
  } else if (mode == 1) {
    EpiResidual::Params ep{Cb, Cb, N};
    e = run_gemm_sk<EpiResidual>(&dummy, ch, ta, tb, M, N, K, ep, s, false);
  } else if (mode == 2) {
    GeluLut lut;
    int lrc = ensure_gelu_lut(nullptr, pow_mode, &lut);
    if (lrc != B200T5_OK) return lrc;
    EpiGeglu::Params ep{Cb, N / 2, lut};
    e = run_gemm_sk<EpiGeglu>(&dummy, ch, ta, tb, M, N, K, ep, s, false);
  } else if (mode == 4) {
    if (!aux || N % 192 || Tmax <= step) return fail(nullptr, B200T5_EINVAL, "test_gemm_splitk: bad QKV arguments");
    if (st.alloc(sizeof(DecodeState)) != cudaSuccess) return fail(nullptr, B200T5_ECUDA, "alloc");
    set_state_kernel<<<1, 1, 0, s>>>(st.as<DecodeState>(), step);
    EpiQkvDecode::Params ep{Cb, static_cast<act_t*>(aux), &st.as<DecodeState>()->step, M, N / 192, Tmax};
    e = run_gemm_sk<EpiQkvDecode>(&dummy, ch, ta, tb, M, N, K, ep, s, false);
    if (e == cudaSuccess) e = cudaStreamSynchronize(s);
  }
  if (e != cudaSuccess) return fail(nullptr, B200T5_ECUDA, "test_gemm_splitk(bn=%d, split=%d, mode=%d): %s", bn, split, mode, cudaGetErrorString(e));
  return B200T5_OK;
#endif
}

extern "C" int b200t5_test_ffo(int device, const void* A, const void* W, void* R, int M, int N, int F, int kernel, int bn,
                               int split, void* stream) {
#if !B200T5_F16
  return fail(nullptr, B200T5_EINVAL, "b200t5_test_ffo exists in the fp16 build only (libb200t5_f16.so)");
#else
  const int sms = hook_device(device);
  if (sms < 0) return sms;
  if (F % 4 || N % 4) return fail(nullptr, B200T5_EINVAL, "F and N must be multiples of 4");
  cudaStream_t s = static_cast<cudaStream_t>(stream);
  const int Fp = (F + 31) / 32 * 32;
  DevBuf wsplit;
  if (wsplit.alloc(static_cast<size_t>(N) * 2 * Fp * 4) != cudaSuccess) return fail(nullptr, B200T5_ENOMEM, "alloc failed");
  const size_t n = static_cast<size_t>(N) * Fp;
  split_tf32_kernel<<<static_cast<unsigned>((n + 255) / 256), 256, 0, s>>>(static_cast<const float*>(W), wsplit.as<float>(), N, F, Fp);
  CUtensorMap ta, tb;
  const int box_b = kernel == 0 ? 128 : bn;
  if (!make_tmap(&ta, A, M, F, 128, true) || !make_tmap(&tb, wsplit.p, N, 2 * Fp, box_b, true))
    return fail(nullptr, B200T5_ECUDA, "%s", g_err);
  EpiResidual::Params ep{static_cast<float*>(R), static_cast<const float*>(R), N};
  ep.round_acc = 0;
  ep.round_out = 0;
  cudaError_t e;
  if (kernel == 0) {
    e = launch_gemm_2cta<EpiResidual, true>(ta, tb, M, N, 2 * Fp, ep, sms, s, Fp / 32);
  } else {
    const int sp = splitk_factor(2 * Fp, split, kBK / 2);
    e = bn == 128 ? launch_gemm_splitk<128, EpiResidual, true>(ta, tb, M, N, 2 * Fp, sp, ep, s, false, Fp / 32)
                  : launch_gemm_splitk<64, EpiResidual, true>(ta, tb, M, N, 2 * Fp, sp, ep, s, false, Fp / 32);
  }
  if (e == cudaSuccess) e = cudaStreamSynchronize(s);
  if (e != cudaSuccess) return fail(nullptr, B200T5_ECUDA, "test_ffo: %s", cudaGetErrorString(e));
  return B200T5_OK;
#endif
}

extern "C" int b200t5_test_rmsnorm(int device, const void* x, const void* w, void* y, int M, int d, float eps, void* stream) {
#if B200T5_F16
  return fail(nullptr, B200T5_EINVAL, "the single-kernel test hooks exist in the bf16 build only (libb200t5.so)");
#else
  const int sms = hook_device(device);
  if (sms < 0) return sms;
  cudaError_t e = run_rmsnorm(nullptr, static_cast<const act_t*>(x), static_cast<const act_t*>(w), static_cast<act_t*>(y), M, d, eps, static_cast<cudaStream_t>(stream));
  if (e != cudaSuccess) return fail(nullptr, B200T5_ECUDA, "rmsnorm: %s", cudaGetErrorString(e));
  return B200T5_OK;
#endif
}

extern "C" int b200t5_test_attn_decode(int device, int self, const void* q, const void* K, const void* V, void* ctx,
                                       int B, int H, int Tk, const int32_t* extent, const uint8_t* key_ok, int step,
                                       const float* dist_bias, void* stream) {
#if B200T5_F16
  return fail(nullptr, B200T5_EINVAL, "the single-kernel test hooks exist in the bf16 build only (libb200t5.so)");
#else
  const int sms = hook_device(device);
  if (sms < 0) return sms;
  cudaStream_t s = static_cast<cudaStream_t>(stream);
  if (self == 1) {
    DevBuf st;
    if (st.alloc(sizeof(DecodeState)) != cudaSuccess) return fail(nullptr, B200T5_ECUDA, "alloc");
    set_state_kernel<<<1, 1, 0, s>>>(st.as<DecodeState>(), step);
    self_attn_decode_warp_kernel<<<(B * H + kSelfWarpsPerCta - 1) / kSelfWarpsPerCta, kSelfWarpsPerCta * 32,
                                   kSelfWarpsPerCta * Tk * sizeof(float), s>>>(
        static_cast<const act_t*>(q), static_cast<const act_t*>(K), static_cast<const act_t*>(V), static_cast<act_t*>(ctx),
        B * H, H, Tk, &st.as<DecodeState>()->step, dist_bias);
    cudaStreamSynchronize(s);
  } else if (self == 2) {
    const int stages = step > 0 ? step : 5;
    if (stages < 2 || stages > kXsMaxStages || Tk > 4096) return fail(nullptr, B200T5_EINVAL, "attn_decode(stream): 2 <= stages <= %d, Tk <= 4096", kXsMaxStages);
    const int items = B * H;
    CUtensorMap tk, tv;
    if (!make_tmap(&tk, K, static_cast<uint64_t>(items) * Tk, 64, kXsChunkKeys) || !make_tmap(&tv, V, static_cast<uint64_t>(items) * Tk, 64, kXsChunkKeys))
      return fail(nullptr, B200T5_ECUDA, "%s", g_err);
    attn_cross_stream_kernel<<<xs_grid(items, sms), kXsThreads, XsSmem::bytes(stages, Tk), s>>>(
        tk, tv, 0, 0, static_cast<const act_t*>(K), static_cast<const act_t*>(V), static_cast<const act_t*>(q), static_cast<act_t*>(ctx), items, H,
        Tk, extent, key_ok, stages, 1, 1, XsStamps{nullptr, 0});
  } else {
    attn_decode_kernel<false><<<B * H, kAttnDecThreads, Tk * sizeof(float), s>>>(
        static_cast<const act_t*>(q), static_cast<const act_t*>(K), static_cast<const act_t*>(V), static_cast<act_t*>(ctx), H,
        Tk, extent, key_ok, nullptr, nullptr, XsStamps{nullptr, 0});
  }
  cudaError_t e = cudaGetLastError();
  if (e != cudaSuccess) return fail(nullptr, B200T5_ECUDA, "attn_decode: %s", cudaGetErrorString(e));
  return B200T5_OK;
#endif
}

extern "C" int b200t5_test_encoder_attn(int device, const void* qkv, void* ctx, const float* rel_bias,
                                        const uint8_t* key_ok, const int32_t* extent, int B, int S, int H, int impl,
                                        void* stream) {
#if B200T5_F16
  return fail(nullptr, B200T5_EINVAL, "the single-kernel test hooks exist in the bf16 build only (libb200t5.so)");
#else
  const int sms = hook_device(device);
  if (sms < 0) return sms;
  DevBuf cu;
  if (impl == 1) {
    std::vector<int> hcu(B);
    for (int b = 0; b < B; ++b) hcu[b] = b * S;
    if (cu.alloc(B * sizeof(int)) != cudaSuccess || cudaMemcpy(cu.p, hcu.data(), B * sizeof(int), cudaMemcpyHostToDevice) != cudaSuccess)
      return fail(nullptr, B200T5_ECUDA, "encoder_attn: offsets");
  }
  const size_t smem = encoder_attn_smem_bytes(S);
  cudaError_t e = smem <= 96 * 1024 ? cudaSuccess : cudaErrorInvalidValue;
  if (e == cudaSuccess) {
    encoder_attn_kernel<<<dim3((S + kEncQ - 1) / kEncQ, B * H), kEncThreads, smem, static_cast<cudaStream_t>(stream)>>>(
        static_cast<const act_t*>(qkv), static_cast<act_t*>(ctx), rel_bias, key_ok, extent, impl == 1 ? cu.as<int>() : nullptr, S, H);
    e = cudaGetLastError();
  }
  if (e != cudaSuccess) return fail(nullptr, B200T5_ECUDA, "encoder_attn: %s", cudaGetErrorString(e));
  return B200T5_OK;
#endif
}

extern "C" int b200t5_test_geglu(int device, const void* gate, const void* up, void* out, int64_t n, int pow_mode, void* stream) {
#if B200T5_F16
  return fail(nullptr, B200T5_EINVAL, "the single-kernel test hooks exist in the bf16 build only (libb200t5.so)");
#else
  const int sms = hook_device(device);
  if (sms < 0) return sms;
  GeluLut lut;
  int lrc = ensure_gelu_lut(nullptr, 0, &lut);
  if (lrc != B200T5_OK) return lrc;
  geglu_elementwise_kernel<<<static_cast<unsigned>((n + 255) / 256), 256, 0, static_cast<cudaStream_t>(stream)>>>(
      static_cast<const act_t*>(gate), static_cast<const act_t*>(up), static_cast<act_t*>(out), n, pow_mode, lut);
  cudaError_t e = cudaGetLastError();
  if (e != cudaSuccess) return fail(nullptr, B200T5_ECUDA, "geglu: %s", cudaGetErrorString(e));
  return B200T5_OK;
#endif
}
```

### anyscale_workshop_nyc_2023_b200/csrc/gemm.cuh

```cuda
#pragma once
#include "ptx.cuh"

namespace b200 {

constexpr int kBM = 128;
constexpr int kBK = 64;
constexpr int kGemmThreads = 288;
constexpr int kGemmConsumers = 256;
constexpr int kEpiSmemBytes = 8192;

template <int BN>
struct GemmCfg {
  static_assert(BN == 32 || BN == 64 || BN == 128 || BN == 256, "BN");
  static constexpr int kABytes = kBM * kBK * 2;
  static constexpr int kBBytes = BN * kBK * 2;
  static constexpr int kStageBytes = kABytes + kBBytes;
  static constexpr int kStages = BN >= 256 ? 4 : (96 * 1024) / kStageBytes;
  static constexpr int kRingBytes = kStages * kStageBytes;
  static constexpr int kStageLd = BN + 4;
  static constexpr int kStagingBytes = kBM * kStageLd * 4;
  static_assert(kStagingBytes <= kRingBytes, "the staged tile aliases the ring");
  static constexpr int kSmemBytes = kRingBytes + 1024  + 256  + kEpiSmemBytes;
  static constexpr int kCtasPerSm = BN <= 128 ? 2 : 1;
};
// ... 22 lines not shown
#pragma unroll
  for (int k = 0; k < kBK / 16; ++k) wgmma_k32B<BN, kTf32>(acc, a_desc + 2 * k, b_desc + 2 * k);
}

template <int BN>
DEVINL void stage_acc(float* stg, int row0, const float (&acc)[BN / 2]) {
  const int t = threadIdx.x & 127;
  const int r = row0 + 16 * (t >> 5) + ((t & 31) >> 2);
  const int c = 2 * (t & 3);
#pragma unroll
  for (int j = 0; j < BN / 8; ++j) {
    *reinterpret_cast<float2*>(stg + r * GemmCfg<BN>::kStageLd + 8 * j + c) = make_float2(acc[4 * j], acc[4 * j + 1]);
    *reinterpret_cast<float2*>(stg + (r + 8) * GemmCfg<BN>::kStageLd + 8 * j + c) = make_float2(acc[4 * j + 2], acc[4 * j + 3]);
  }
}

template <int BN, class Epi, bool kTf32 = false, int kBBox = BN>
__global__ void __launch_bounds__(kGemmThreads, GemmCfg<BN>::kCtasPerSm)
gemm_bf16_tn_kernel(const __grid_constant__ CUtensorMap tmA, const __grid_constant__ CUtensorMap tmB, int M, int N,
                    int K, int m_fastest, typename Epi::Params ep, int a_kblocks) {
  using Cfg = GemmCfg<BN>;
  static_assert(BN % kBBox == 0, "box");
  constexpr int kbk = kTf32 ? kBK / 2 : kBK;
  extern __shared__ uint8_t smem_raw[];
  uint8_t* smem = reinterpret_cast<uint8_t*>((reinterpret_cast<uintptr_t>(smem_raw) + 1023) & ~uintptr_t(1023));
  uint64_t* bars = reinterpret_cast<uint64_t*>(smem + Cfg::kRingBytes);
  uint64_t* full = bars;
  uint64_t* empty = bars + Cfg::kStages;
  uint64_t* stg_free = bars + 2 * Cfg::kStages;
  uint8_t* epi_smem = smem + Cfg::kRingBytes + 256;
  float* stg = reinterpret_cast<float*>(smem);

  const int warp = threadIdx.x >> 5;
  const int lane = threadIdx.x & 31;
  const int tiles_m = (M + kBM - 1) / kBM;
  const int tiles_n = (N + BN - 1) / BN;
  const int num_tiles = tiles_m * tiles_n;
  const int kblocks = (K + kbk - 1) / kbk;
  if (a_kblocks <= 0) a_kblocks = kblocks;

  pdl_launch_dependents();
  if (threadIdx.x == 0) {
    for (int i = 0; i < Cfg::kStages; ++i) {
      mbar_init(&full[i], 1);
      mbar_init(&empty[i], 2);
    }
    mbar_init(stg_free, kGemmConsumers);
    mbar_fence_init();
  }
  __syncthreads();

  if (warp == 8) {
    if (lane == 0) {
      tma_prefetch_desc(&tmA);
      tma_prefetch_desc(&tmB);
      if (static_cast<int>(blockIdx.x) < num_tiles) {
        const TileCoord tc0 = tile_coord(blockIdx.x, tiles_m, tiles_n, m_fastest);
        for (int kb = 0; kb < kblocks; ++kb)
          for (int p = 0; p < BN / kBBox; ++p) tma_prefetch_l2_2d(&tmB, kb * kbk, tc0.n_tile * BN + p * kBBox);
      }
      pdl_wait();
      int stage = 0;
      uint32_t phase = 0, sphase = 0;
      for (int tile = blockIdx.x; tile < num_tiles; tile += gridDim.x) {
        if (tile != static_cast<int>(blockIdx.x)) {
          mbar_wait(stg_free, sphase);
          sphase ^= 1u;
        }
        const TileCoord tc = tile_coord(tile, tiles_m, tiles_n, m_fastest);
        const int m0 = tc.m_tile * kBM, n0 = tc.n_tile * BN;
        for (int kb = 0; kb < kblocks; ++kb) {
          mbar_wait(&empty[stage], phase ^ 1u);
          uint8_t* sA = smem + stage * Cfg::kStageBytes;
          uint8_t* sB = sA + Cfg::kABytes;
          mbar_arrive_expect_tx(&full[stage], Cfg::kStageBytes);
          tma_load_2d(sA, &tmA, &full[stage], (kb % a_kblocks) * kbk, m0);
#pragma unroll
          for (int p = 0; p < BN / kBBox; ++p) tma_load_2d(sB + p * kBBox * 128, &tmB, &full[stage], kb * kbk, n0 + p * kBBox);
          if (++stage == Cfg::kStages) {
            stage = 0;
            phase ^= 1u;
          }
        }
      }
    }
  } else {
    const int wg = warp >> 2;
    const int et = threadIdx.x;
    Epi::prologue(ep, epi_smem, et, kGemmConsumers);
    pdl_wait();
    int stage = 0;
    uint32_t phase = 0;
    for (int tile = blockIdx.x; tile < num_tiles; tile += gridDim.x) {
      const TileCoord tc = tile_coord(tile, tiles_m, tiles_n, m_fastest);
      float acc[BN / 2];
#pragma unroll
      for (int i = 0; i < BN / 2; ++i) acc[i] = 0.f;
      int prev = -1;
      for (int kb = 0; kb < kblocks; ++kb) {
        mbar_wait(&full[stage], phase);
        const uint32_t a_addr = smem_u32(smem + stage * Cfg::kStageBytes) + wg * 64 * 128;
        wgmma_fence_acc(acc);
        wgmma_fence();
        wgmma_kblock<BN, kTf32>(acc, a_addr, smem_u32(smem + stage * Cfg::kStageBytes + Cfg::kABytes));
        wgmma_commit();
        wgmma_wait<1>();
        wgmma_fence_acc(acc);
        if (prev >= 0 && (threadIdx.x & 127) == 0) mbar_arrive(&empty[prev]);
        prev = stage;
        if (++stage == Cfg::kStages) {
          stage = 0;
          phase ^= 1u;
        }
      }
      wgmma_wait<0>();
      wgmma_fence_acc(acc);
      if (prev >= 0 && (threadIdx.x & 127) == 0) mbar_arrive(&empty[prev]);
      consumers_sync();
      stage_acc<BN>(stg, wg * 64, acc);
      consumers_sync();
      const int row = et & (kBM - 1), part = et >> 7;
      const int m = tc.m_tile * kBM + row;
      const uint32_t waddr = (smem_u32(stg) >> 2) + static_cast<uint32_t>(row * Cfg::kStageLd);
      Epi::template run<BN>(ep, waddr, m, m < M, tc.n_tile, N, epi_smem, part, 2);
      mbar_arrive(stg_free);
    }
  }
}


DEVINL void round_pack_32(const uint32_t (&acc)[32], uint32_t (&out)[16]) {
#pragma unroll
  for (int i = 0; i < 16; ++i) out[i] = pack_act2(__uint_as_float(acc[2 * i]), __uint_as_float(acc[2 * i + 1]));
}

DEVINL void store_row_chunk(act_t* dst, const uint32_t (&p)[16], int n0, int N) {
  uint4* d4 = reinterpret_cast<uint4*>(dst);
#pragma unroll
  for (int g = 0; g < 4; ++g) {
    if (n0 + g * 8 + 8 <= N) d4[g] = make_uint4(p[4 * g], p[4 * g + 1], p[4 * g + 2], p[4 * g + 3]);
  }
}

DEVINL void store_row_chunk_f32(float* dst, const float (&v)[32], int n0, int N) {
  float4* d4 = reinterpret_cast<float4*>(dst);
#pragma unroll
  for (int g = 0; g < 8; ++g) {
    if (n0 + g * 4 + 4 <= N) d4[g] = make_float4(v[4 * g], v[4 * g + 1], v[4 * g + 2], v[4 * g + 3]);
  }
}

struct NoPre {};

template <int BN, class Epi>
DEVINL void run_chunks(const typename Epi::Params& p, uint32_t taddr, int m, bool m_ok, int n_tile, int N,
                                 const uint8_t* epi_smem, int part, int parts) {
  constexpr int C = BN / 32;
  const int c_lo = part * C / parts, c_hi = (part + 1) * C / parts;
  typename Epi::ChunkPre pre[2];
  if (m_ok && n_tile * BN + c_lo * 32 < N) Epi::chunk_pre(p, m, n_tile * BN + c_lo * 32, N, pre[0]);
#pragma unroll 1
  for (int c = c_lo; c < c_hi; c += 2) {
#pragma unroll
    for (int u = 0; u < 2; ++u) {
      if (c + u < c_hi) {
        uint32_t acc[32];
        acc_ld_32(taddr + (c + u) * 32, acc);
        const int n0 = n_tile * BN + (c + u) * 32;
        if (m_ok && c + u + 1 < c_hi && n0 + 32 < N) Epi::chunk_pre(p, m, n0 + 32, N, pre[(u + 1) & 1]);
        if (m_ok && n0 < N) Epi::chunk(p, acc, m, n0, N, epi_smem, pre[u & 1]);
      }
    }
  }
}

struct EpiStore {
  struct Params {
    act_t* C;
    int ldc;
  };
  static constexpr bool kPaired = false;
  typedef NoPre ChunkPre;
  static DEVINL void prologue(const Params&, uint8_t*, int, int = 128) {}
  static DEVINL void chunk_pre(const Params&, int, int, int, ChunkPre&) {}
  static DEVINL void chunk(const Params& p, const uint32_t (&acc)[32], int m, int n0, int N, const uint8_t*,
                           const ChunkPre&) {
    uint32_t o[16];
    round_pack_32(acc, o);
    store_row_chunk(p.C + static_cast<size_t>(m) * p.ldc + n0, o, n0, N);
  }
  template <int BN>
  static DEVINL void run(const Params& p, uint32_t taddr, int m, bool m_ok, int n_tile, int N, const uint8_t* es,
                         int part, int parts) {
    run_chunks<BN, EpiStore>(p, taddr, m, m_ok, n_tile, N, es, part, parts);
  }
};

#if B200T5_F16
struct EpiResidual {
  struct Params {
    res_t* C;
    const res_t* R;
    int ld;
    float* ss = nullptr;
    int ss_ld = 0;
    int round_acc = 1;
    int round_out = 0;
  };
  static constexpr bool kPaired = false;
  struct ChunkPre {
    float4 r[8];
  };
  static DEVINL void prologue(const Params&, uint8_t*, int, int = 128) {}
  static DEVINL void chunk_pre(const Params& p, int m, int n0, int N, ChunkPre& pre) {
    const float4* r4 = reinterpret_cast<const float4*>(p.R + static_cast<size_t>(m) * p.ld + n0);
#pragma unroll
    for (int g = 0; g < 8; ++g) pre.r[g] = (n0 + g * 4 + 4 <= N) ? r4[g] : make_float4(0.f, 0.f, 0.f, 0.f);
  }
  static DEVINL void chunk(const Params& p, const uint32_t (&acc)[32], int m, int n0, int N, const uint8_t*,
                           const ChunkPre& pre) {
    float o[32];
#pragma unroll
    for (int g = 0; g < 8; ++g) {
      const float rw[4] = {pre.r[g].x, pre.r[g].y, pre.r[g].z, pre.r[g].w};
#pragma unroll
      for (int j = 0; j < 4; ++j) {
        float y = __uint_as_float(acc[g * 4 + j]);
        if (p.round_acc) y = act_round(y);
        float v = rw[j] + y;
        if (p.round_out) v = act_round(v);
        o[g * 4 + j] = v;
      }
    }
    store_row_chunk_f32(p.C + static_cast<size_t>(m) * p.ld + n0, o, n0, N);
  }
  template <int BN>
  static DEVINL void run(const Params& p, uint32_t taddr, int m, bool m_ok, int n_tile, int N, const uint8_t* es,
                         int part, int parts) {
    run_chunks<BN, EpiResidual>(p, taddr, m, m_ok, n_tile, N, es, part, parts);
  }
};
#else
struct EpiResidual {
  struct Params {
    act_t* C;
    const act_t* R;
    int ld;
    float* ss = nullptr;
    int ss_ld = 0;
    int round_acc = 1, round_out = 1;
  };
  static constexpr bool kPaired = false;
  struct ChunkPre {
    uint4 r[4];
  };
  static DEVINL void prologue(const Params&, uint8_t*, int, int = 128) {}
  static DEVINL void chunk_pre(const Params& p, int m, int n0, int N, ChunkPre& pre) {
    const uint4* r4 = reinterpret_cast<const uint4*>(p.R + static_cast<size_t>(m) * p.ld + n0);
#pragma unroll
    for (int g = 0; g < 4; ++g) pre.r[g] = (n0 + g * 8 + 8 <= N) ? r4[g] : make_uint4(0, 0, 0, 0);
  }
  static DEVINL void chunk(const Params& p, const uint32_t (&acc)[32], int m, int n0, int N, const uint8_t*,
                           const ChunkPre& pre) {
    uint32_t o[16];
#pragma unroll
    for (int g = 0; g < 4; ++g) {
      const uint32_t rw[4] = {pre.r[g].x, pre.r[g].y, pre.r[g].z, pre.r[g].w};
#pragma unroll
      for (int j = 0; j < 4; ++j) {
        const float y0 = act_round(__uint_as_float(acc[g * 8 + 2 * j]));
        const float y1 = act_round(__uint_as_float(acc[g * 8 + 2 * j + 1]));
        o[g * 4 + j] = pack_act2(act_lo(rw[j]) + y0, act_hi(rw[j]) + y1);
      }
    }
    store_row_chunk(p.C + static_cast<size_t>(m) * p.ld + n0, o, n0, N);
    if (p.ss) {
      float sq = 0.f;
#pragma unroll
      for (int i = 0; i < 16; ++i) {
        if (n0 + 2 * i + 2 <= N) {
          const float a = act_lo(o[i]), b = act_hi(o[i]);
          sq = fmaf(a, a, sq);
          sq = fmaf(b, b, sq);
        }
      }
      p.ss[static_cast<size_t>(m) * p.ss_ld + (n0 >> 5)] = sq;
    }
  }
  template <int BN>
  static DEVINL void run(const Params& p, uint32_t taddr, int m, bool m_ok, int n_tile, int N, const uint8_t* es,
                         int part, int parts) {
    run_chunks<BN, EpiResidual>(p, taddr, m, m_ok, n_tile, N, es, part, parts);
  }
};

#endif

DEVINL float gelu_new_act_exact(float x, int pow_mode) {
  const float half_x = act_round(0.5f * x);
  const float x3 = (pow_mode == 0 && !B200T5_F16) ? act_round(act_round(x * x) * x) : act_round(x * x * x);
  const float t1 = act_round(0.044715f * x3);
  const float t2 = act_round(x + t1);
  const float t3 = act_round(0.7978845608028654f * t2);
  const float t4 = act_round(tanhf(t3));
  const float t5 = act_round(1.0f + t4);
  return act_round(half_x * t5);
}

struct GeluLut {
  const uint16_t* table;
  int lo, hi;
};

DEVINL float gelu_from_lut_sel(float x, const uint16_t* lut, int lo, int n ) {
  const uint32_t bits = __float_as_uint(x) >> 16;
  const int mag = static_cast<int>(bits & 0x7FFFu);
  const bool neg = (bits >> 15) != 0;
  const int rel = mag - lo;
  const int idx = min(max(rel, 0), n - 1) + (neg ? n : 0);
  const float tab = __uint_as_float(static_cast<uint32_t>(lut[idx]) << 16);
  const float half = act_round(0.5f * x);
  float sat = neg ? (mag == 0x7F80 ? __int_as_float(0x7FC00000) : -0.0f) : x;
  sat = mag > 0x7F80 ? x : sat;
  return rel < 0 ? half : (rel >= n ? sat : tab);
}

DEVINL float gelu_from_lut(float x, const uint16_t* lut, int lo, int hi) {
  const uint32_t bits = __float_as_uint(x) >> 16;
  const int mag = static_cast<int>(bits & 0x7FFFu);
  const int neg = static_cast<int>(bits >> 15);
  if (mag < lo) return act_round(0.5f * x);
  if (mag >= hi) {
    if (mag > 0x7F80) return x;
    if (!neg) return x;
    return mag == 0x7F80 ? __int_as_float(0x7FC00000) : -0.0f;
  }
  return __uint_as_float(static_cast<uint32_t>(lut[neg * (hi - lo) + (mag - lo)]) << 16);
}

struct EpiGeglu {
  struct Params {
    ffh_t* out;
    int F;
    GeluLut lut;
  };
  static constexpr bool kPaired = true;
  typedef NoPre ChunkPre;
  static DEVINL void prologue(const Params& p, uint8_t* epi_smem, int tid, int nthreads = 128) {
#if B200T5_F16
    return;
#endif
    const int nvec = (2 * (p.lut.hi - p.lut.lo) * 2 + 15) / 16;
    const uint4* src = reinterpret_cast<const uint4*>(p.lut.table);
    uint4* dst = reinterpret_cast<uint4*>(epi_smem);
    for (int i = tid; i < nvec; i += nthreads) dst[i] = src[i];
    asm volatile("bar.sync 2, %0;" ::"r"(nthreads) : "memory");
  }
  static DEVINL void chunk2(const Params& p, const uint32_t (&g)[32], const uint32_t (&u)[32], int m, int f0,
                            const uint8_t* epi_smem) {
#if B200T5_F16
    float o[32];
#pragma unroll
    for (int i = 0; i < 32; ++i) {
      const float x = act_round(__uint_as_float(g[i]));
      const float lin = act_round(__uint_as_float(u[i]));
      o[i] = act_round(gelu_new_act_exact(x, 1) * lin);
    }
    store_row_chunk_f32(p.out + static_cast<size_t>(m) * p.F + f0, o, f0, p.F);
#else
    const uint16_t* lut = reinterpret_cast<const uint16_t*>(epi_smem);
    const int lo = p.lut.lo, n = p.lut.hi - p.lut.lo;
    uint32_t o[16];
#pragma unroll
    for (int i = 0; i < 16; ++i) {
      float r[2];
#pragma unroll
      for (int e = 0; e < 2; ++e) {
        const float x = act_round(__uint_as_float(g[2 * i + e]));
        const float lin = act_round(__uint_as_float(u[2 * i + e]));
        r[e] = (n > 0 ? gelu_from_lut_sel(x, lut, lo, n) : gelu_from_lut(x, lut, lo, p.lut.hi)) * lin;
      }
      o[i] = pack_act2(r[0], r[1]);
    }
    store_row_chunk(p.out + static_cast<size_t>(m) * p.F + f0, o, f0, p.F);
#endif
  }
  template <int BN>
  static DEVINL void run(const Params& p, uint32_t taddr, int m, bool m_ok, int n_tile, int , const uint8_t* epi_smem,
                         int part, int parts) {
    constexpr int HALF = BN / 2;
    constexpr int C = HALF / 32;
#pragma unroll 1
    for (int c = part * C / parts; c < (part + 1) * C / parts; ++c) {
      uint32_t g[32], u[32];
      acc_ld_32(taddr + c * 32, g);
      acc_ld_32(taddr + HALF + c * 32, u);
      const int f0 = n_tile * HALF + c * 32;
      if (m_ok && f0 < p.F) chunk2(p, g, u, m, f0, epi_smem);
    }
  }
};

struct EpiCrossKV {
  struct Params {
    act_t* arena;
    int B, H, S;
    const int* row_b = nullptr;
    const int* row_s = nullptr;
  };
  static constexpr bool kPaired = false;
  typedef NoPre ChunkPre;
  static DEVINL void prologue(const Params&, uint8_t*, int, int = 128) {}
  static DEVINL void chunk_pre(const Params&, int, int, int, ChunkPre&) {}
  static DEVINL void chunk(const Params& p, const uint32_t (&acc)[32], int m, int n0, int N, const uint8_t*,
                           const ChunkPre&) {
    const int b = p.row_b ? p.row_b[m] : m / p.S;
    const int s = p.row_s ? p.row_s[m] : m - b * p.S;
    const int hd = p.H * 64;
    const int lkv = n0 / hd;
    const int rem = n0 - lkv * hd;
    const int h = rem >> 6, d0 = rem & 63;
    uint32_t o[16];
    round_pack_32(acc, o);
    act_t* dst = p.arena + ((((static_cast<size_t>(lkv) * p.B + b) * p.H + h) * p.S + s) << 6) + d0;
    store_row_chunk(dst, o, n0, N);
  }
  template <int BN>
  static DEVINL void run(const Params& p, uint32_t taddr, int m, bool m_ok, int n_tile, int N, const uint8_t* es,
                         int part, int parts) {
    run_chunks<BN, EpiCrossKV>(p, taddr, m, m_ok, n_tile, N, es, part, parts);
  }
};

struct EpiQkvDecode {
  struct Params {
    act_t* q;
    act_t* cache;
    const int* step;
    int B, H, Tmax;
    int step_stride = 0;
  };
  static constexpr bool kPaired = false;
  typedef NoPre ChunkPre;
  static DEVINL void prologue(const Params&, uint8_t*, int, int = 128) {}
  static DEVINL void chunk_pre(const Params&, int, int, int, ChunkPre&) {}
  static DEVINL void chunk(const Params& p, const uint32_t (&acc)[32], int m, int n0, int N, const uint8_t*,
                           const ChunkPre&) {
    const int I = p.H * 64;
    uint32_t o[16];
    round_pack_32(acc, o);
    act_t* dst;
    if (n0 < I) {
      dst = p.q + static_cast<size_t>(m) * I + n0;
    } else {
      const int t = p.step[m * p.step_stride];
      const int r = n0 - I;
      const int kv = r / I;
      const int rem = r - kv * I;
      const int h = rem >> 6, d0 = rem & 63;
      dst = p.cache + ((((static_cast<size_t>(kv) * p.B + m) * p.H + h) * p.Tmax + t) << 6) + d0;
    }
    store_row_chunk(dst, o, n0, N);
  }
  template <int BN>
  static DEVINL void run(const Params& p, uint32_t taddr, int m, bool m_ok, int n_tile, int N, const uint8_t* es,
                         int part, int parts) {
    run_chunks<BN, EpiQkvDecode>(p, taddr, m, m_ok, n_tile, N, es, part, parts);
  }
};

struct EpiArgmax {
  struct Params {
    float* pval;
    int* pidx;
    int n_tiles;
    const int* step;
    int eos, min_new;
    int step_stride = 0;
  };
  static DEVINL void prologue(const Params&, uint8_t*, int, int = 128) {}
  template <int BN>
  static DEVINL void run(const Params& p, uint32_t taddr, int m, bool m_ok, int n_tile, int N, const uint8_t*, int part, int) {
    if (part != 0) return;
    float best = -INFINITY;
    int bidx = n_tile * BN;
    const bool block_eos = m_ok && p.step[m * p.step_stride] < p.min_new;
#pragma unroll 1
    for (int c = 0; c < BN / 32; ++c) {
      uint32_t acc[32];
      acc_ld_32(taddr + c * 32, acc);
      const int n0 = n_tile * BN + c * 32;
#pragma unroll
      for (int j = 0; j < 32; ++j) {
        const int n = n0 + j;
        float v = act_round(__uint_as_float(acc[j]));
        if (n >= N || (block_eos && n == p.eos)) v = -INFINITY;
        if (v > best) {
          best = v;
          bidx = n;
        }
      }
    }
    if (m_ok) {
      p.pval[static_cast<size_t>(m) * p.n_tiles + n_tile] = best;
      p.pidx[static_cast<size_t>(m) * p.n_tiles + n_tile] = bidx;
    }
  }
};

struct EpiStoreF32 {
  struct Params {
    float* C;
    int ldc;
  };
  static DEVINL void prologue(const Params&, uint8_t*, int, int = 128) {}
  template <int BN>
  static DEVINL void run(const Params& p, uint32_t taddr, int m, bool m_ok, int n_tile, int N, const uint8_t*, int part, int parts) {
#pragma unroll 1
    for (int c = part * (BN / 32) / parts; c < (part + 1) * (BN / 32) / parts; ++c) {
      uint32_t acc[32];
      acc_ld_32(taddr + c * 32, acc);
      const int n0 = n_tile * BN + c * 32;
      if (m_ok) {
#pragma unroll
        for (int j = 0; j < 32; ++j)
          if (n0 + j < N) p.C[static_cast<size_t>(m) * p.ldc + n0 + j] = act_round(__uint_as_float(acc[j]));
      }
    }
  }
};

template <int BN, class Epi, bool kTf32 = false, int kBBox = BN>
cudaError_t prepare_gemm() {
  return cudaFuncSetAttribute(gemm_bf16_tn_kernel<BN, Epi, kTf32, kBBox>, cudaFuncAttributeMaxDynamicSharedMemorySize,
                              GemmCfg<BN>::kSmemBytes);
}

inline int& launch_priority() {
  static thread_local int prio = 0;
  return prio;
}

template <class... KArgs, class... Args>
cudaError_t launch_kernel(void (*kern)(KArgs...), dim3 grid, dim3 block, size_t smem, cudaStream_t stream, bool pdl,
                          Args... args) {
  cudaLaunchConfig_t cfg{};
  cfg.gridDim = grid;
  cfg.blockDim = block;
  cfg.dynamicSmemBytes = smem;
  cfg.stream = stream;
  cudaLaunchAttribute attr[2];
  int na = 0;
  if (pdl) {
    attr[na].id = cudaLaunchAttributeProgrammaticStreamSerialization;
    attr[na].val.programmaticStreamSerializationAllowed = 1;
    ++na;
  }
  if (launch_priority() != 0) {
    attr[na].id = cudaLaunchAttributePriority;
    attr[na].val.priority = launch_priority();
    ++na;
  }
  cfg.attrs = attr;
  cfg.numAttrs = na;
  return cudaLaunchKernelEx(&cfg, kern, static_cast<KArgs>(args)...);
}

template <int BN, class Epi, bool kTf32 = false, int kBBox = BN>
cudaError_t launch_gemm(const CUtensorMap& tmA, const CUtensorMap& tmB, int M, int N, int K, int m_fastest,
                        const typename Epi::Params& ep, int num_sms, cudaStream_t stream, bool pdl = false, int a_kblocks = 0) {
  using Cfg = GemmCfg<BN>;
  const int tiles = ((M + kBM - 1) / kBM) * ((N + BN - 1) / BN);
  const int slots = num_sms * Cfg::kCtasPerSm;
  const int grid = tiles < slots ? tiles : slots;
  return launch_kernel(gemm_bf16_tn_kernel<BN, Epi, kTf32, kBBox>, dim3(grid), dim3(kGemmThreads), Cfg::kSmemBytes, stream, pdl,
                       tmA, tmB, M, N, K, m_fastest, ep, a_kblocks);
}

}
```

### anyscale_workshop_nyc_2023_b200/csrc/gemm_2cta.cuh

```cuda
#pragma once
#include "gemm.cuh"

namespace b200 {

constexpr int k2ctaBN = 256;
constexpr int k2ctaBox = 128;

template <class Epi, bool kTf32 = false>
cudaError_t prepare_gemm_2cta() {
  return prepare_gemm<k2ctaBN, Epi, kTf32, k2ctaBox>();
}

template <class Epi, bool kTf32 = false>
cudaError_t launch_gemm_2cta(const CUtensorMap& tmA, const CUtensorMap& tmB, int M, int N, int K,
                             const typename Epi::Params& ep, int num_sms, cudaStream_t stream, int a_kblocks = 0) {
  return launch_gemm<k2ctaBN, Epi, kTf32, k2ctaBox>(tmA, tmB, M, N, K, 0, ep, num_sms, stream, false, a_kblocks);
}

}
```

### anyscale_workshop_nyc_2023_b200/csrc/gemm_splitk.cuh

```cuda
#pragma once
#include "gemm.cuh"

namespace b200 {

constexpr int kSkThreads = kGemmThreads;
constexpr int kSkMaxRegs = 152;
constexpr int kSkMaxSplit = 8;
constexpr int kSkMaxStages = 4;

template <int BN>
struct SkCfg {
  static_assert(BN == 64 || BN == 128, "BN");
  static constexpr int kABytes = kBM * kBK * 2;
  static constexpr int kBBytes = BN * kBK * 2;
  static constexpr int kStageBytes = kABytes + kBBytes;
  static constexpr int kDefaultStages = BN == 64 ? 4 : 3;
  static constexpr int kRedLd = BN + 4;
  static constexpr int kRedBytes = kBM * kRedLd * 4;
  static constexpr int smem_bytes(int stages, bool epi) {
    return stages * kStageBytes + 1024  + 256  + kRedBytes + (epi ? kEpiSmemBytes : 0);
  }
  static constexpr int kMaxSmemBytes = smem_bytes(kSkMaxStages, true);
};

DEVINL uint32_t cluster_ctarank() {
  uint32_t r;
  asm volatile("mov.u32 %0, %%cluster_ctarank;" : "=r"(r));
  return r;
}
DEVINL uint32_t cluster_nctarank() {
  uint32_t r;
  asm volatile("mov.u32 %0, %%cluster_nctarank;" : "=r"(r));
  return r;
}
DEVINL void cluster_arrive_relaxed() { asm volatile("barrier.cluster.arrive.relaxed.aligned;" ::: "memory"); }
DEVINL void cluster_arrive_release() { asm volatile("barrier.cluster.arrive.release.aligned;" ::: "memory"); }
DEVINL void cluster_wait_acquire() { asm volatile("barrier.cluster.wait.acquire.aligned;" ::: "memory"); }
DEVINL uint32_t mapa_shared(uint32_t cta_addr, uint32_t rank) {
  uint32_t r;
  asm volatile("mapa.shared::cluster.u32 %0, %1, %2;" : "=r"(r) : "r"(cta_addr), "r"(rank));
  return r;
}
DEVINL void st_cluster_v2(uint32_t addr, float a, float b) {
  asm volatile("st.shared::cluster.v2.f32 [%0], {%1, %2};" ::"r"(addr), "f"(a), "f"(b) : "memory");
}

DEVINL void add32_smem(uint32_t (&acc)[32], const float* src) {
  const float4* r4 = reinterpret_cast<const float4*>(src);
#pragma unroll
  for (int v = 0; v < 8; ++v) {
    const float4 a = r4[v];
    acc[4 * v] = __float_as_uint(__uint_as_float(acc[4 * v]) + a.x);
    acc[4 * v + 1] = __float_as_uint(__uint_as_float(acc[4 * v + 1]) + a.y);
    acc[4 * v + 2] = __float_as_uint(__uint_as_float(acc[4 * v + 2]) + a.z);
    acc[4 * v + 3] = __float_as_uint(__uint_as_float(acc[4 * v + 3]) + a.w);
  }
}

template <int BN, class Epi, bool kTf32 = false>
__global__ void __maxnreg__(kSkMaxRegs)
gemm_splitk_kernel(const __grid_constant__ CUtensorMap tmA, const __grid_constant__ CUtensorMap tmB, int M, int N,
                   int K, typename Epi::Params ep, int a_kblocks, int stages) {
  using Cfg = SkCfg<BN>;
  constexpr int kbk = kTf32 ? kBK / 2 : kBK;
  extern __shared__ uint8_t smem_raw[];
  uint8_t* smem = reinterpret_cast<uint8_t*>((reinterpret_cast<uintptr_t>(smem_raw) + 1023) & ~uintptr_t(1023));
  uint64_t* bars = reinterpret_cast<uint64_t*>(smem + stages * Cfg::kStageBytes);
  uint64_t* full = bars;
  uint64_t* empty = bars + kSkMaxStages;
  float* red = reinterpret_cast<float*>(smem + stages * Cfg::kStageBytes + 256);

  const int warp = threadIdx.x >> 5;
  const int lane = threadIdx.x & 31;
  const int S = static_cast<int>(cluster_nctarank());
  const int rank = static_cast<int>(cluster_ctarank());
  uint8_t* epi_smem = reinterpret_cast<uint8_t*>(red) + Cfg::kRedBytes;
  const int n_tile = blockIdx.y, m_tile = blockIdx.z;
  const int kblocks = (K + kbk - 1) / kbk;
  if (a_kblocks <= 0) a_kblocks = kblocks;
  const int kb_per = (kblocks + S - 1) / S;
  const int kb0 = rank * kb_per;
  const int kb1 = (kb0 + kb_per) < kblocks ? (kb0 + kb_per) : kblocks;
  const int nkb = kb1 - kb0;
  const int m0 = m_tile * kBM, n0t = n_tile * BN;

  pdl_launch_dependents();
  cluster_arrive_relaxed();
  if (threadIdx.x == 0) {
    for (int i = 0; i < stages; ++i) {
      mbar_init(&full[i], 1);
      mbar_init(&empty[i], 2);
    }
    mbar_fence_init();
  }
  __syncthreads();

  if (warp == 8) {
    if (lane == 0) {
      tma_prefetch_desc(&tmA);
      tma_prefetch_desc(&tmB);
      const int first = nkb < stages ? nkb : stages;
      for (int i = 0; i < first; ++i) {
        uint8_t* sA = smem + i * Cfg::kStageBytes;
        mbar_arrive_expect_tx(&full[i], Cfg::kStageBytes);
        tma_load_2d(sA + Cfg::kABytes, &tmB, &full[i], (kb0 + i) * kbk, n0t);
      }
      pdl_wait();
      for (int i = 0; i < first; ++i) tma_load_2d(smem + i * Cfg::kStageBytes, &tmA, &full[i], ((kb0 + i) % a_kblocks) * kbk, m0);
      int stage = first == stages ? 0 : first;
      uint32_t phase = first == stages ? 1u : 0u;
      for (int i = first; i < nkb; ++i) {
        mbar_wait(&empty[stage], phase ^ 1u);
        uint8_t* sA = smem + stage * Cfg::kStageBytes;
        mbar_arrive_expect_tx(&full[stage], Cfg::kStageBytes);
        tma_load_2d(sA, &tmA, &full[stage], ((kb0 + i) % a_kblocks) * kbk, m0);
        tma_load_2d(sA + Cfg::kABytes, &tmB, &full[stage], (kb0 + i) * kbk, n0t);
        if (++stage == stages) {
          stage = 0;
          phase ^= 1u;
        }
      }
    }
    __syncwarp();
    cluster_wait_acquire();
    cluster_arrive_release();
    cluster_wait_acquire();
  } else {
    const int et = threadIdx.x;
    const int wg = warp >> 2;
    const int rows_per = kBM / S;
    if constexpr (Epi::kPaired) Epi::prologue(ep, epi_smem, et, kGemmConsumers);
    constexpr int kChunks = Epi::kPaired ? BN / 64 : BN / 32;
    const int items = rows_per * kChunks;
    pdl_wait();
    typename Epi::ChunkPre pre0;
    {
      const int rl = et / kChunks, c = et - rl * kChunks;
      const int m = m0 + rank * rows_per + rl;
      if constexpr (!Epi::kPaired) {
        if (et < items && m < M && n0t + c * 32 < N) Epi::chunk_pre(ep, m, n0t + c * 32, N, pre0);
      }
    }
    float acc[BN / 2];
#pragma unroll
    for (int i = 0; i < BN / 2; ++i) acc[i] = 0.f;
    {
      int stage = 0, prev = -1;
      uint32_t phase = 0;
      for (int i = 0; i < nkb; ++i) {
        mbar_wait(&full[stage], phase);
        const uint32_t a_addr = smem_u32(smem + stage * Cfg::kStageBytes) + wg * 64 * 128;
        wgmma_fence_acc(acc);
        wgmma_fence();
        wgmma_kblock<BN, kTf32>(acc, a_addr, smem_u32(smem + stage * Cfg::kStageBytes + Cfg::kABytes));
        wgmma_commit();
        wgmma_wait<1>();
        wgmma_fence_acc(acc);
        if (prev >= 0 && (et & 127) == 0) mbar_arrive(&empty[prev]);
        prev = stage;
        if (++stage == stages) {
          stage = 0;
          phase ^= 1u;
        }
      }
      wgmma_wait<0>();
      wgmma_fence_acc(acc);
    }
    cluster_wait_acquire();
    {
      const int t = et & 127;
      const int rbase = wg * 64 + 16 * (t >> 5) + ((t & 31) >> 2);
      const int c = 2 * (t & 3);
#pragma unroll
      for (int half = 0; half < 2; ++half) {
        const int row = rbase + 8 * half;
        const int dst_rank = row / rows_per;
        const int slot = rank * rows_per + (row - dst_rank * rows_per);
        const uint32_t dst = mapa_shared(smem_u32(red + static_cast<size_t>(slot) * Cfg::kRedLd + c), static_cast<uint32_t>(dst_rank));
#pragma unroll
        for (int j = 0; j < BN / 8; ++j) st_cluster_v2(dst + 32 * j, acc[4 * j + 2 * half], acc[4 * j + 2 * half + 1]);
      }
    }
    cluster_arrive_release();
    cluster_wait_acquire();
#pragma unroll 1
    for (int it = et; it < items; it += kGemmConsumers) {
      const int rl = it / kChunks, c = it - rl * kChunks;
      const int m = m0 + rank * rows_per + rl;
      if (m >= M) continue;
      if constexpr (Epi::kPaired) {
        constexpr int HALF = BN / 2;
        const int f0 = n_tile * HALF + c * 32;
        if (f0 >= ep.F) continue;
        uint32_t g[32], u[32];
#pragma unroll
        for (int j = 0; j < 32; ++j) g[j] = u[j] = 0u;
        for (int src = 0; src < S; ++src) {
          const float* base = red + static_cast<size_t>(src * rows_per + rl) * Cfg::kRedLd;
// ... 71 lines not shown
```

### anyscale_workshop_nyc_2023_b200/csrc/ptx.cuh

```cuda
#pragma once
#include <cuda.h>
#include <cuda_bf16.h>
#include <cuda_fp16.h>
#include <cuda_runtime.h>
#include <stdint.h>

namespace b200 {

#define DEVINL __device__ __forceinline__

DEVINL uint32_t smem_u32(const void* p) {
  return static_cast<uint32_t>(__cvta_generic_to_shared(p));
}

DEVINL uint32_t lane_id() { return threadIdx.x & 31u; }

DEVINL bool elect_one() {
  uint32_t pred = 0;
  asm volatile(
      "{\n\t.reg .pred P;\n\t"
      "elect.sync _|P, 0xffffffff;\n\t"
      "selp.b32 %0, 1, 0, P;\n\t}\n"
      : "=r"(pred));
  return pred != 0;
}

DEVINL void pdl_launch_dependents() { asm volatile("griddepcontrol.launch_dependents;" ::: "memory"); }
DEVINL void pdl_wait() { asm volatile("griddepcontrol.wait;" ::: "memory"); }

DEVINL void mbar_init(uint64_t* bar, uint32_t count) {
  asm volatile("mbarrier.init.shared::cta.b64 [%0], %1;" ::"r"(smem_u32(bar)), "r"(count) : "memory");
}
DEVINL void mbar_fence_init() {
  asm volatile("fence.mbarrier_init.release.cluster;" ::: "memory");
}
DEVINL void mbar_arrive(uint64_t* bar) {
  asm volatile("mbarrier.arrive.shared::cta.b64 _, [%0];" ::"r"(smem_u32(bar)) : "memory");
}
DEVINL void mbar_arrive_expect_tx(uint64_t* bar, uint32_t bytes) {
  asm volatile("mbarrier.arrive.expect_tx.shared::cta.b64 _, [%0], %1;" ::"r"(smem_u32(bar)), "r"(bytes)
               : "memory");
}
DEVINL bool mbar_try_wait(uint64_t* bar, uint32_t parity) {
  uint32_t ok;
  asm volatile(
      "{\n\t.reg .pred P;\n\t"
      "mbarrier.try_wait.parity.shared::cta.b64 P, [%1], %2;\n\t"
      "selp.b32 %0, 1, 0, P;\n\t}\n"
      : "=r"(ok)
      : "r"(smem_u32(bar)), "r"(parity)
      : "memory");
  return ok != 0;
}
DEVINL uint64_t global_timer_ns() {
  uint64_t t;
  asm volatile("mov.u64 %0, %%globaltimer;" : "=l"(t));
  return t;
}
DEVINL void mbar_wait(uint64_t* bar, uint32_t parity) {
  uint32_t spins = 0;
  uint64_t t0 = 0;
  while (!mbar_try_wait(bar, parity)) {
    if ((++spins & 0x3FFu) == 0) {
      const uint64_t now = global_timer_ns();
      if (t0 == 0) t0 = now;
      else if (now - t0 > 2000000000ull) __trap();
    }
  }
}

DEVINL void fence_proxy_async_smem() { asm volatile("fence.proxy.async.shared::cta;" ::: "memory"); }

DEVINL void tma_prefetch_desc(const CUtensorMap* m) {
  asm volatile("prefetch.tensormap [%0];" ::"l"(reinterpret_cast<uint64_t>(m)) : "memory");
}
DEVINL void tma_load_2d(void* smem_dst, const CUtensorMap* m, uint64_t* bar, int32_t c0, int32_t c1) {
  asm volatile(
      "cp.async.bulk.tensor.2d.shared::cluster.global.mbarrier::complete_tx::bytes"
      " [%0], [%1, {%3, %4}], [%2];"
      ::"r"(smem_u32(smem_dst)), "l"(reinterpret_cast<uint64_t>(m)), "r"(smem_u32(bar)), "r"(c0), "r"(c1)
      : "memory");
}
DEVINL void tma_prefetch_l2_2d(const CUtensorMap* m, int32_t c0, int32_t c1) {
  asm volatile("cp.async.bulk.prefetch.tensor.2d.L2.global.tile [%0, {%1, %2}];" ::"l"(reinterpret_cast<uint64_t>(m)),
               "r"(c0), "r"(c1)
               : "memory");
}
DEVINL void tma_load_3d(void* smem_dst, const CUtensorMap* m, uint64_t* bar, int32_t c0, int32_t c1,
                        int32_t c2) {
  asm volatile(
      "cp.async.bulk.tensor.3d.shared::cluster.global.mbarrier::complete_tx::bytes"
      " [%0], [%1, {%3, %4, %5}], [%2];"
      ::"r"(smem_u32(smem_dst)), "l"(reinterpret_cast<uint64_t>(m)), "r"(smem_u32(bar)), "r"(c0), "r"(c1),
      "r"(c2)
      : "memory");
}
DEVINL void bulk_load_1d(void* smem_dst, const void* gsrc, uint32_t bytes, uint64_t* bar) {
  asm volatile(
      "cp.async.bulk.shared::cluster.global.mbarrier::complete_tx::bytes [%0], [%1], %2, [%3];"
      ::"r"(smem_u32(smem_dst)), "l"(reinterpret_cast<uint64_t>(gsrc)), "r"(bytes), "r"(smem_u32(bar))
      : "memory");
}

DEVINL void wgmma_fence() { asm volatile("wgmma.fence.sync.aligned;" ::: "memory"); }
DEVINL void wgmma_commit() { asm volatile("wgmma.commit_group.sync.aligned;" ::: "memory"); }
template <int N>
DEVINL void wgmma_wait() { asm volatile("wgmma.wait_group.sync.aligned %0;" ::"n"(N) : "memory"); }
template <int R>
DEVINL void wgmma_fence_acc(float (&d)[R]) {
#pragma unroll
  for (int i = 0; i < R; ++i) asm volatile("" : "+f"(d[i])::"memory");
}

#if B200T5_F16
#define WGMMA_ACT_TYPES ".f32.f16.f16"
#else
#define WGMMA_ACT_TYPES ".f32.bf16.bf16"
#endif
DEVINL void wgmma_act_n32(float (&d)[16], uint64_t desc_a, uint64_t desc_b) {
  asm volatile(
      "{\n\t.reg .pred p;\n\tsetp.ne.b32 p, 1, 0;\n\t"
      "wgmma.mma_async.sync.aligned.m64n32k16" WGMMA_ACT_TYPES " "
      "{" 
      "%0, %1, %2, %3, %4, %5, %6, %7, %8, %9, %10, %11, %12, %13, %14, %15"
      "}, %16, %17, p, 1, 1, 0, 0;\n\t}\n"
      : "+f"(d[0]), "+f"(d[1]), "+f"(d[2]), "+f"(d[3]), "+f"(d[4]), "+f"(d[5]), "+f"(d[6]), "+f"(d[7]),
        "+f"(d[8]), "+f"(d[9]), "+f"(d[10]), "+f"(d[11]), "+f"(d[12]), "+f"(d[13]), "+f"(d[14]), "+f"(d[15])
      : "l"(desc_a), "l"(desc_b));
}
DEVINL void wgmma_tf32_n32(float (&d)[16], uint64_t desc_a, uint64_t desc_b) {
  asm volatile(
      "{\n\t.reg .pred p;\n\tsetp.ne.b32 p, 1, 0;\n\t"
      "wgmma.mma_async.sync.aligned.m64n32k8" ".f32.tf32.tf32" " "
      "{" 
      "%0, %1, %2, %3, %4, %5, %6, %7, %8, %9, %10, %11, %12, %13, %14, %15"
      "}, %16, %17, p, 1, 1;\n\t}\n"
      : "+f"(d[0]), "+f"(d[1]), "+f"(d[2]), "+f"(d[3]), "+f"(d[4]), "+f"(d[5]), "+f"(d[6]), "+f"(d[7]),
        "+f"(d[8]), "+f"(d[9]), "+f"(d[10]), "+f"(d[11]), "+f"(d[12]), "+f"(d[13]), "+f"(d[14]), "+f"(d[15])
      : "l"(desc_a), "l"(desc_b));
}
DEVINL void wgmma_act_n64(float (&d)[32], uint64_t desc_a, uint64_t desc_b) {
  asm volatile(
      "{\n\t.reg .pred p;\n\tsetp.ne.b32 p, 1, 0;\n\t"
      "wgmma.mma_async.sync.aligned.m64n64k16" WGMMA_ACT_TYPES " "
      "{" 
      "%0, %1, %2, %3, %4, %5, %6, %7, %8, %9, %10, %11, %12, %13, %14, %15, "
      "%16, %17, %18, %19, %20, %21, %22, %23, %24, %25, %26, %27, %28, %29, %30, %31"
      "}, %32, %33, p, 1, 1, 0, 0;\n\t}\n"
      : "+f"(d[0]), "+f"(d[1]), "+f"(d[2]), "+f"(d[3]), "+f"(d[4]), "+f"(d[5]), "+f"(d[6]), "+f"(d[7]),
        "+f"(d[8]), "+f"(d[9]), "+f"(d[10]), "+f"(d[11]), "+f"(d[12]), "+f"(d[13]), "+f"(d[14]), "+f"(d[15]),
        "+f"(d[16]), "+f"(d[17]), "+f"(d[18]), "+f"(d[19]), "+f"(d[20]), "+f"(d[21]), "+f"(d[22]), "+f"(d[23]),
        "+f"(d[24]), "+f"(d[25]), "+f"(d[26]), "+f"(d[27]), "+f"(d[28]), "+f"(d[29]), "+f"(d[30]), "+f"(d[31])
      : "l"(desc_a), "l"(desc_b));
}
DEVINL void wgmma_tf32_n64(float (&d)[32], uint64_t desc_a, uint64_t desc_b) {
  asm volatile(
      "{\n\t.reg .pred p;\n\tsetp.ne.b32 p, 1, 0;\n\t"
      "wgmma.mma_async.sync.aligned.m64n64k8" ".f32.tf32.tf32" " "
      "{" 
      "%0, %1, %2, %3, %4, %5, %6, %7, %8, %9, %10, %11, %12, %13, %14, %15, "
      "%16, %17, %18, %19, %20, %21, %22, %23, %24, %25, %26, %27, %28, %29, %30, %31"
      "}, %32, %33, p, 1, 1;\n\t}\n"
      : "+f"(d[0]), "+f"(d[1]), "+f"(d[2]), "+f"(d[3]), "+f"(d[4]), "+f"(d[5]), "+f"(d[6]), "+f"(d[7]),
        "+f"(d[8]), "+f"(d[9]), "+f"(d[10]), "+f"(d[11]), "+f"(d[12]), "+f"(d[13]), "+f"(d[14]), "+f"(d[15]),
        "+f"(d[16]), "+f"(d[17]), "+f"(d[18]), "+f"(d[19]), "+f"(d[20]), "+f"(d[21]), "+f"(d[22]), "+f"(d[23]),
        "+f"(d[24]), "+f"(d[25]), "+f"(d[26]), "+f"(d[27]), "+f"(d[28]), "+f"(d[29]), "+f"(d[30]), "+f"(d[31])
      : "l"(desc_a), "l"(desc_b));
}
DEVINL void wgmma_act_n128(float (&d)[64], uint64_t desc_a, uint64_t desc_b) {
  asm volatile(
      "{\n\t.reg .pred p;\n\tsetp.ne.b32 p, 1, 0;\n\t"
      "wgmma.mma_async.sync.aligned.m64n128k16" WGMMA_ACT_TYPES " "
      "{" 
      "%0, %1, %2, %3, %4, %5, %6, %7, %8, %9, %10, %11, %12, %13, %14, %15, "
      "%16, %17, %18, %19, %20, %21, %22, %23, %24, %25, %26, %27, %28, %29, %30, %31, "
      "%32, %33, %34, %35, %36, %37, %38, %39, %40, %41, %42, %43, %44, %45, %46, %47, "
      "%48, %49, %50, %51, %52, %53, %54, %55, %56, %57, %58, %59, %60, %61, %62, %63"
      "}, %64, %65, p, 1, 1, 0, 0;\n\t}\n"
      : "+f"(d[0]), "+f"(d[1]), "+f"(d[2]), "+f"(d[3]), "+f"(d[4]), "+f"(d[5]), "+f"(d[6]), "+f"(d[7]),
        "+f"(d[8]), "+f"(d[9]), "+f"(d[10]), "+f"(d[11]), "+f"(d[12]), "+f"(d[13]), "+f"(d[14]), "+f"(d[15]),
        "+f"(d[16]), "+f"(d[17]), "+f"(d[18]), "+f"(d[19]), "+f"(d[20]), "+f"(d[21]), "+f"(d[22]), "+f"(d[23]),
        "+f"(d[24]), "+f"(d[25]), "+f"(d[26]), "+f"(d[27]), "+f"(d[28]), "+f"(d[29]), "+f"(d[30]), "+f"(d[31]),
        "+f"(d[32]), "+f"(d[33]), "+f"(d[34]), "+f"(d[35]), "+f"(d[36]), "+f"(d[37]), "+f"(d[38]), "+f"(d[39]),
        "+f"(d[40]), "+f"(d[41]), "+f"(d[42]), "+f"(d[43]), "+f"(d[44]), "+f"(d[45]), "+f"(d[46]), "+f"(d[47]),
        "+f"(d[48]), "+f"(d[49]), "+f"(d[50]), "+f"(d[51]), "+f"(d[52]), "+f"(d[53]), "+f"(d[54]), "+f"(d[55]),
        "+f"(d[56]), "+f"(d[57]), "+f"(d[58]), "+f"(d[59]), "+f"(d[60]), "+f"(d[61]), "+f"(d[62]), "+f"(d[63])
      : "l"(desc_a), "l"(desc_b));
}
DEVINL void wgmma_tf32_n128(float (&d)[64], uint64_t desc_a, uint64_t desc_b) {
  asm volatile(
      "{\n\t.reg .pred p;\n\tsetp.ne.b32 p, 1, 0;\n\t"
      "wgmma.mma_async.sync.aligned.m64n128k8" ".f32.tf32.tf32" " "
      "{" 
      "%0, %1, %2, %3, %4, %5, %6, %7, %8, %9, %10, %11, %12, %13, %14, %15, "
      "%16, %17, %18, %19, %20, %21, %22, %23, %24, %25, %26, %27, %28, %29, %30, %31, "
      "%32, %33, %34, %35, %36, %37, %38, %39, %40, %41, %42, %43, %44, %45, %46, %47, "
      "%48, %49, %50, %51, %52, %53, %54, %55, %56, %57, %58, %59, %60, %61, %62, %63"
      "}, %64, %65, p, 1, 1;\n\t}\n"
      : "+f"(d[0]), "+f"(d[1]), "+f"(d[2]), "+f"(d[3]), "+f"(d[4]), "+f"(d[5]), "+f"(d[6]), "+f"(d[7]),
        "+f"(d[8]), "+f"(d[9]), "+f"(d[10]), "+f"(d[11]), "+f"(d[12]), "+f"(d[13]), "+f"(d[14]), "+f"(d[15]),
        "+f"(d[16]), "+f"(d[17]), "+f"(d[18]), "+f"(d[19]), "+f"(d[20]), "+f"(d[21]), "+f"(d[22]), "+f"(d[23]),
        "+f"(d[24]), "+f"(d[25]), "+f"(d[26]), "+f"(d[27]), "+f"(d[28]), "+f"(d[29]), "+f"(d[30]), "+f"(d[31]),
        "+f"(d[32]), "+f"(d[33]), "+f"(d[34]), "+f"(d[35]), "+f"(d[36]), "+f"(d[37]), "+f"(d[38]), "+f"(d[39]),
        "+f"(d[40]), "+f"(d[41]), "+f"(d[42]), "+f"(d[43]), "+f"(d[44]), "+f"(d[45]), "+f"(d[46]), "+f"(d[47]),
        "+f"(d[48]), "+f"(d[49]), "+f"(d[50]), "+f"(d[51]), "+f"(d[52]), "+f"(d[53]), "+f"(d[54]), "+f"(d[55]),
        "+f"(d[56]), "+f"(d[57]), "+f"(d[58]), "+f"(d[59]), "+f"(d[60]), "+f"(d[61]), "+f"(d[62]), "+f"(d[63])
      : "l"(desc_a), "l"(desc_b));
}
DEVINL void wgmma_act_n256(float (&d)[128], uint64_t desc_a, uint64_t desc_b) {
  asm volatile(
      "{\n\t.reg .pred p;\n\tsetp.ne.b32 p, 1, 0;\n\t"
      "wgmma.mma_async.sync.aligned.m64n256k16" WGMMA_ACT_TYPES " "
      "{" 
      "%0, %1, %2, %3, %4, %5, %6, %7, %8, %9, %10, %11, %12, %13, %14, %15, "
      "%16, %17, %18, %19, %20, %21, %22, %23, %24, %25, %26, %27, %28, %29, %30, %31, "
      "%32, %33, %34, %35, %36, %37, %38, %39, %40, %41, %42, %43, %44, %45, %46, %47, "
      "%48, %49, %50, %51, %52, %53, %54, %55, %56, %57, %58, %59, %60, %61, %62, %63, "
      "%64, %65, %66, %67, %68, %69, %70, %71, %72, %73, %74, %75, %76, %77, %78, %79, "
      "%80, %81, %82, %83, %84, %85, %86, %87, %88, %89, %90, %91, %92, %93, %94, %95, "
      "%96, %97, %98, %99, %100, %101, %102, %103, %104, %105, %106, %107, %108, %109, %110, %111, "
      "%112, %113, %114, %115, %116, %117, %118, %119, %120, %121, %122, %123, %124, %125, %126, %127"
      "}, %128, %129, p, 1, 1, 0, 0;\n\t}\n"
      : "+f"(d[0]), "+f"(d[1]), "+f"(d[2]), "+f"(d[3]), "+f"(d[4]), "+f"(d[5]), "+f"(d[6]), "+f"(d[7]),
        "+f"(d[8]), "+f"(d[9]), "+f"(d[10]), "+f"(d[11]), "+f"(d[12]), "+f"(d[13]), "+f"(d[14]), "+f"(d[15]),
        "+f"(d[16]), "+f"(d[17]), "+f"(d[18]), "+f"(d[19]), "+f"(d[20]), "+f"(d[21]), "+f"(d[22]), "+f"(d[23]),
        "+f"(d[24]), "+f"(d[25]), "+f"(d[26]), "+f"(d[27]), "+f"(d[28]), "+f"(d[29]), "+f"(d[30]), "+f"(d[31]),
        "+f"(d[32]), "+f"(d[33]), "+f"(d[34]), "+f"(d[35]), "+f"(d[36]), "+f"(d[37]), "+f"(d[38]), "+f"(d[39]),
        "+f"(d[40]), "+f"(d[41]), "+f"(d[42]), "+f"(d[43]), "+f"(d[44]), "+f"(d[45]), "+f"(d[46]), "+f"(d[47]),
        "+f"(d[48]), "+f"(d[49]), "+f"(d[50]), "+f"(d[51]), "+f"(d[52]), "+f"(d[53]), "+f"(d[54]), "+f"(d[55]),
        "+f"(d[56]), "+f"(d[57]), "+f"(d[58]), "+f"(d[59]), "+f"(d[60]), "+f"(d[61]), "+f"(d[62]), "+f"(d[63]),
        "+f"(d[64]), "+f"(d[65]), "+f"(d[66]), "+f"(d[67]), "+f"(d[68]), "+f"(d[69]), "+f"(d[70]), "+f"(d[71]),
        "+f"(d[72]), "+f"(d[73]), "+f"(d[74]), "+f"(d[75]), "+f"(d[76]), "+f"(d[77]), "+f"(d[78]), "+f"(d[79]),
        "+f"(d[80]), "+f"(d[81]), "+f"(d[82]), "+f"(d[83]), "+f"(d[84]), "+f"(d[85]), "+f"(d[86]), "+f"(d[87]),
        "+f"(d[88]), "+f"(d[89]), "+f"(d[90]), "+f"(d[91]), "+f"(d[92]), "+f"(d[93]), "+f"(d[94]), "+f"(d[95]),
        "+f"(d[96]), "+f"(d[97]), "+f"(d[98]), "+f"(d[99]), "+f"(d[100]), "+f"(d[101]), "+f"(d[102]), "+f"(d[103]),
        "+f"(d[104]), "+f"(d[105]), "+f"(d[106]), "+f"(d[107]), "+f"(d[108]), "+f"(d[109]), "+f"(d[110]), "+f"(d[111]),
        "+f"(d[112]), "+f"(d[113]), "+f"(d[114]), "+f"(d[115]), "+f"(d[116]), "+f"(d[117]), "+f"(d[118]), "+f"(d[119]),
        "+f"(d[120]), "+f"(d[121]), "+f"(d[122]), "+f"(d[123]), "+f"(d[124]), "+f"(d[125]), "+f"(d[126]), "+f"(d[127])
      : "l"(desc_a), "l"(desc_b));
}
DEVINL void wgmma_tf32_n256(float (&d)[128], uint64_t desc_a, uint64_t desc_b) {
  asm volatile(
      "{\n\t.reg .pred p;\n\tsetp.ne.b32 p, 1, 0;\n\t"
      "wgmma.mma_async.sync.aligned.m64n256k8" ".f32.tf32.tf32" " "
      "{" 
      "%0, %1, %2, %3, %4, %5, %6, %7, %8, %9, %10, %11, %12, %13, %14, %15, "
      "%16, %17, %18, %19, %20, %21, %22, %23, %24, %25, %26, %27, %28, %29, %30, %31, "
      "%32, %33, %34, %35, %36, %37, %38, %39, %40, %41, %42, %43, %44, %45, %46, %47, "
      "%48, %49, %50, %51, %52, %53, %54, %55, %56, %57, %58, %59, %60, %61, %62, %63, "
      "%64, %65, %66, %67, %68, %69, %70, %71, %72, %73, %74, %75, %76, %77, %78, %79, "
      "%80, %81, %82, %83, %84, %85, %86, %87, %88, %89, %90, %91, %92, %93, %94, %95, "
      "%96, %97, %98, %99, %100, %101, %102, %103, %104, %105, %106, %107, %108, %109, %110, %111, "
      "%112, %113, %114, %115, %116, %117, %118, %119, %120, %121, %122, %123, %124, %125, %126, %127"
      "}, %128, %129, p, 1, 1;\n\t}\n"
      : "+f"(d[0]), "+f"(d[1]), "+f"(d[2]), "+f"(d[3]), "+f"(d[4]), "+f"(d[5]), "+f"(d[6]), "+f"(d[7]),
        "+f"(d[8]), "+f"(d[9]), "+f"(d[10]), "+f"(d[11]), "+f"(d[12]), "+f"(d[13]), "+f"(d[14]), "+f"(d[15]),
        "+f"(d[16]), "+f"(d[17]), "+f"(d[18]), "+f"(d[19]), "+f"(d[20]), "+f"(d[21]), "+f"(d[22]), "+f"(d[23]),
        "+f"(d[24]), "+f"(d[25]), "+f"(d[26]), "+f"(d[27]), "+f"(d[28]), "+f"(d[29]), "+f"(d[30]), "+f"(d[31]),
        "+f"(d[32]), "+f"(d[33]), "+f"(d[34]), "+f"(d[35]), "+f"(d[36]), "+f"(d[37]), "+f"(d[38]), "+f"(d[39]),
        "+f"(d[40]), "+f"(d[41]), "+f"(d[42]), "+f"(d[43]), "+f"(d[44]), "+f"(d[45]), "+f"(d[46]), "+f"(d[47]),
        "+f"(d[48]), "+f"(d[49]), "+f"(d[50]), "+f"(d[51]), "+f"(d[52]), "+f"(d[53]), "+f"(d[54]), "+f"(d[55]),
        "+f"(d[56]), "+f"(d[57]), "+f"(d[58]), "+f"(d[59]), "+f"(d[60]), "+f"(d[61]), "+f"(d[62]), "+f"(d[63]),
        "+f"(d[64]), "+f"(d[65]), "+f"(d[66]), "+f"(d[67]), "+f"(d[68]), "+f"(d[69]), "+f"(d[70]), "+f"(d[71]),
        "+f"(d[72]), "+f"(d[73]), "+f"(d[74]), "+f"(d[75]), "+f"(d[76]), "+f"(d[77]), "+f"(d[78]), "+f"(d[79]),
        "+f"(d[80]), "+f"(d[81]), "+f"(d[82]), "+f"(d[83]), "+f"(d[84]), "+f"(d[85]), "+f"(d[86]), "+f"(d[87]),
        "+f"(d[88]), "+f"(d[89]), "+f"(d[90]), "+f"(d[91]), "+f"(d[92]), "+f"(d[93]), "+f"(d[94]), "+f"(d[95]),
        "+f"(d[96]), "+f"(d[97]), "+f"(d[98]), "+f"(d[99]), "+f"(d[100]), "+f"(d[101]), "+f"(d[102]), "+f"(d[103]),
        "+f"(d[104]), "+f"(d[105]), "+f"(d[106]), "+f"(d[107]), "+f"(d[108]), "+f"(d[109]), "+f"(d[110]), "+f"(d[111]),
        "+f"(d[112]), "+f"(d[113]), "+f"(d[114]), "+f"(d[115]), "+f"(d[116]), "+f"(d[117]), "+f"(d[118]), "+f"(d[119]),
        "+f"(d[120]), "+f"(d[121]), "+f"(d[122]), "+f"(d[123]), "+f"(d[124]), "+f"(d[125]), "+f"(d[126]), "+f"(d[127])
      : "l"(desc_a), "l"(desc_b));
}

template <int N, bool kTf32>
DEVINL void wgmma_k32B(float (&d)[N / 2], uint64_t desc_a, uint64_t desc_b) {
  if constexpr (kTf32) {
    if constexpr (N == 32) wgmma_tf32_n32(d, desc_a, desc_b);
    else if constexpr (N == 64) wgmma_tf32_n64(d, desc_a, desc_b);
    else if constexpr (N == 128) wgmma_tf32_n128(d, desc_a, desc_b);
    else wgmma_tf32_n256(d, desc_a, desc_b);
  } else {
    if constexpr (N == 32) wgmma_act_n32(d, desc_a, desc_b);
    else if constexpr (N == 64) wgmma_act_n64(d, desc_a, desc_b);
    else if constexpr (N == 128) wgmma_act_n128(d, desc_a, desc_b);
    else wgmma_act_n256(d, desc_a, desc_b);
  }
}

DEVINL uint64_t make_desc_sw128_kmajor(uint32_t smem_addr) {
  uint64_t d = 0;
  d |= static_cast<uint64_t>((smem_addr & 0x3FFFFu) >> 4);
  d |= static_cast<uint64_t>(1) << 16;
  d |= static_cast<uint64_t>(1024 >> 4) << 32;
  d |= static_cast<uint64_t>(1) << 62;
  return d;
}

DEVINL void acc_ld_32(uint32_t waddr, uint32_t (&r)[32]) {
#pragma unroll
  for (int v = 0; v < 8; ++v)
    asm volatile("ld.shared.v4.b32 {%0, %1, %2, %3}, [%4];"
                 : "=r"(r[4 * v]), "=r"(r[4 * v + 1]), "=r"(r[4 * v + 2]), "=r"(r[4 * v + 3])
                 : "r"((waddr + 4u * v) << 2)
                 : "memory");
}
#ifndef B200T5_F16
#define B200T5_F16 0
#endif
#if B200T5_F16
typedef __half act_t;
typedef __half2 act2_t;
typedef float res_t;
typedef float ffh_t;
DEVINL act_t float2act(float x) { return __float2half_rn(x); }
__host__ __device__ inline float act2float(act_t x) { return __half2float(x); }
DEVINL act2_t floats2act2(float lo, float hi) { return __floats2half2_rn(lo, hi); }
DEVINL float act_lo(uint32_t w) { return __half2float(__ushort_as_half(static_cast<unsigned short>(w & 0xFFFFu))); }
DEVINL float act_hi(uint32_t w) { return __half2float(__ushort_as_half(static_cast<unsigned short>(w >> 16))); }
#else
typedef __nv_bfloat16 act_t;
typedef __nv_bfloat162 act2_t;
typedef __nv_bfloat16 res_t;
typedef __nv_bfloat16 ffh_t;
DEVINL act_t float2act(float x) { return __float2bfloat16_rn(x); }
__host__ __device__ inline float act2float(act_t x) { return __bfloat162float(x); }
DEVINL act2_t floats2act2(float lo, float hi) { return __floats2bfloat162_rn(lo, hi); }
DEVINL float act_lo(uint32_t w) { return __uint_as_float(w << 16); }
DEVINL float act_hi(uint32_t w) { return __uint_as_float(w & 0xFFFF0000u); }
#endif
DEVINL float act_round(float x) { return act2float(float2act(x)); }
DEVINL uint32_t pack_act2(float lo, float hi) {
  act2_t v = floats2act2(lo, hi);
  return *reinterpret_cast<uint32_t*>(&v);
}

DEVINL uint4 ldg_nc_v4(const void* p) {
  uint4 r;
  asm volatile("ld.global.nc.L1::no_allocate.v4.u32 {%0, %1, %2, %3}, [%4];"
               : "=r"(r.x), "=r"(r.y), "=r"(r.z), "=r"(r.w)
               : "l"(p));
  return r;
}

DEVINL uint64_t l2_policy_evict_first() {
  uint64_t p;
  asm volatile("createpolicy.fractional.L2::evict_first.b64 %0, 1.0;" : "=l"(p));
  return p;
}
DEVINL uint64_t l2_policy_evict_last() {
  uint64_t p;
  asm volatile("createpolicy.fractional.L2::evict_last.b64 %0, 1.0;" : "=l"(p));
  return p;
}
DEVINL uint4 ldg_nc_v4_hint(const void* p, uint64_t policy) {
  uint4 r;
  asm volatile("ld.global.nc.L1::no_allocate.L2::cache_hint.v4.u32 {%0, %1, %2, %3}, [%4], %5;"
               : "=r"(r.x), "=r"(r.y), "=r"(r.z), "=r"(r.w)
               : "l"(p), "l"(policy));
  return r;
}
DEVINL void prefetch_l2_bulk(const void* p, uint32_t bytes, uint64_t policy) {
  asm volatile("cp.async.bulk.prefetch.L2.global.L2::cache_hint [%0], %1, %2;" ::"l"(p), "r"(bytes), "l"(policy) : "memory");
}

}
```

Before: 80060.

## Replace encoder 256/2CTA GEMM paths with a clustered wgmma encoder GEMM

Removes the BN=256 single-CTA and 2-CTA encoder GEMM variants and routes all encoder projections, the FFN and the cross-KV GEMM through a new 2-CTA cluster kernel. The new kernel multicasts the shared weight tile over TMA, runs a warp-specialized wgmma mainloop, and stages accumulators in shared memory as bf16 so a separate epilogue warp group overlaps with the next tile's math. The aim is to halve weight-tile loads per cluster and hide epilogue cost. The trade-off is a rounding of accumulators to activation precision before the epilogue, plus cross-CTA barrier overhead, and the loss of the env toggle back to the old path.

After: 79670 (median of 6 runs). About the same (-0.5%).

```diff
diff --git a/anyscale_workshop_nyc_2023_b200/csrc/b200t5.cu b/anyscale_workshop_nyc_2023_b200/csrc/b200t5.cu
--- a/anyscale_workshop_nyc_2023_b200/csrc/b200t5.cu
+++ b/anyscale_workshop_nyc_2023_b200/csrc/b200t5.cu
@@ -19,7 +19,7 @@
 #include "elementwise.cuh"
 #include "gemm.cuh"
 #include "gemm_splitk.cuh"
-#include "gemm_2cta.cuh"
+#include "gemm_encoder.cuh"
 
 using namespace b200;
 
@@ -159,19 +159,18 @@
   }
 };
 
-enum GemmKind { G_STORE256, G_RES256, G_GEGLU256, G_CROSSKV256, G_QKVDEC64, G_STORE32, G_RES32, G_GEGLU64, G_ARGMAX128, G_LOGITS128 };
+enum GemmKind { G_QKVDEC64, G_STORE32, G_RES32, G_GEGLU64, G_ARGMAX128, G_LOGITS128 };
 
 struct GemmOp {
   CUtensorMap tmA, tmB;
   int M = 0, N = 0, K = 0;
-  GemmKind kind = G_STORE256;
+  GemmKind kind = G_STORE32;
   int m_fastest = 0;
 };
 
 struct EncLayerW {
   DevBuf ln0, ln1, wqkv, wo, wi, wff_o;
   CUtensorMap tm_qkv, tm_o, tm_wi, tm_ffo;
-  CUtensorMap tm2_qkv, tm2_o, tm2_wi, tm2_ffo;
 };
 struct DecLayerW {
   DevBuf ln0, ln1, ln2, wqkv, wo, wcq, wco, wi, wff_o;
@@ -256,7 +255,7 @@
   std::map<std::string, std::unique_ptr<DevBuf>> raw_f32;
   std::map<std::string, std::vector<int64_t>> raw_shape;
   DevBuf shared, lm_head, enc_final_ln, dec_final_ln, enc_relbias, dec_relbias, wcrosskv;
-  CUtensorMap tm_lm, tm_crosskv, tm2_crosskv;
+  CUtensorMap tm_lm, tm_crosskv;
   std::vector<float> enc_relbias_h, dec_relbias_h;
   std::vector<EncLayerW> enc;
   std::vector<DecLayerW> dec;
@@ -273,7 +272,6 @@
     int bn, split;
   };
   bool pack_rows = true;
-  bool use_2cta = true;
   bool self_block = true;
   int xattn_mode = 2;
   int xs_stages = 5;
@@ -342,14 +340,6 @@
 static cudaError_t run_gemm(b200t5_ctx* h, const GemmOp& g, const void* ep, cudaStream_t s, bool pdl = false) {
   h->launches++;
   switch (g.kind) {
-    case G_STORE256:
-      return launch_gemm<256, EpiStore>(g.tmA, g.tmB, g.M, g.N, g.K, g.m_fastest, *static_cast<const EpiStore::Params*>(ep), h->num_sms, s, pdl);
-    case G_RES256:
-      return launch_gemm<256, EpiResidual>(g.tmA, g.tmB, g.M, g.N, g.K, g.m_fastest, *static_cast<const EpiResidual::Params*>(ep), h->num_sms, s, pdl);
-    case G_GEGLU256:
-      return launch_gemm<256, EpiGeglu>(g.tmA, g.tmB, g.M, g.N, g.K, g.m_fastest, *static_cast<const EpiGeglu::Params*>(ep), h->num_sms, s, pdl);
-    case G_CROSSKV256:
-      return launch_gemm<256, EpiCrossKV>(g.tmA, g.tmB, g.M, g.N, g.K, g.m_fastest, *static_cast<const EpiCrossKV::Params*>(ep), h->num_sms, s, pdl);
     case G_QKVDEC64:
       return launch_gemm<64, EpiQkvDecode>(g.tmA, g.tmB, g.M, g.N, g.K, g.m_fastest, *static_cast<const EpiQkvDecode::Params*>(ep), h->num_sms, s, pdl);
     case G_STORE32:
@@ -367,10 +357,10 @@
 }
 
 template <class Epi>
-static cudaError_t run_gemm_2cta(b200t5_ctx* h, const CUtensorMap& tmA, const CUtensorMap& tmB, int M, int N, int K,
-                                 const typename Epi::Params& ep, cudaStream_t s) {
+static cudaError_t run_gemm_encoder(b200t5_ctx* h, const CUtensorMap& tmA, const CUtensorMap& tmB, int M, int N, int K,
+                                    const typename Epi::Params& ep, cudaStream_t s) {
   h->launches++;
-  return launch_gemm_2cta<Epi>(tmA, tmB, M, N, K, ep, h->num_sms, s);
+  return launch_gemm_encoder<Epi>(tmA, tmB, M, N, K, ep, s);
 }
 
 template <class Epi>
@@ -383,10 +373,14 @@
   return launch_gemm_splitk<64, Epi>(tmA, tmB, M, N, K, split, ep, s, pdl, 0, h->sk_stages64);
 }
 
-static cudaError_t run_ffo_2cta(b200t5_ctx* h, const CUtensorMap& tmA, const CUtensorMap& tmB, int M, int N,
-                                const EpiResidual::Params& ep, cudaStream_t s) {
+static cudaError_t run_ffo_encoder(b200t5_ctx* h, const CUtensorMap& tmA, const CUtensorMap& tmB, int M, int N,
+                                   const EpiResidual::Params& ep, cudaStream_t s) {
   h->launches++;
-  return launch_gemm_2cta<EpiResidual, B200T5_F16 != 0>(tmA, tmB, M, N, h->ffo_k, ep, h->num_sms, s, B200T5_F16 ? h->ffo_k / 64 : 0);
+#if B200T5_F16
+  return launch_gemm_encoder_tf32(tmA, tmB, M, N, h->ffo_k, ep, h->num_sms, s, h->ffo_k / 64);
+#else
+  return launch_gemm_encoder<EpiResidual>(tmA, tmB, M, N, h->ffo_k, ep, s);
+#endif
 }
 static cudaError_t run_ffo_sk(b200t5_ctx* h, const b200t5_ctx::SkChoice& ch, const CUtensorMap& tmA, const CUtensorMap& tmB,
                               int M, int N, const EpiResidual::Params& ep, cudaStream_t s, bool pdl) {
@@ -412,20 +406,22 @@
   cudaError_t e;
 #define PREP(BN, EPI)                         \
   if ((e = prepare_gemm<BN, EPI>()) != cudaSuccess) return e;
-  PREP(256, EpiStore) PREP(256, EpiResidual) PREP(256, EpiGeglu) PREP(256, EpiCrossKV) PREP(64, EpiQkvDecode)
+  PREP(64, EpiQkvDecode)
   PREP(32, EpiStore) PREP(32, EpiResidual) PREP(64, EpiGeglu) PREP(128, EpiArgmax) PREP(128, EpiStoreF32)
   PREP(64, EpiStore) PREP(128, EpiStore)
 #undef PREP
-  if ((e = prepare_gemm_2cta<EpiStore>()) != cudaSuccess) return e;
-  if ((e = prepare_gemm_2cta<EpiResidual>()) != cudaSuccess) return e;
-  if ((e = prepare_gemm_2cta<EpiGeglu>()) != cudaSuccess) return e;
-  if ((e = prepare_gemm_2cta<EpiCrossKV>()) != cudaSuccess) return e;
+  if ((e = prepare_gemm_encoder<EpiStore>()) != cudaSuccess) return e;
+  if ((e = prepare_gemm_encoder<EpiResidual>()) != cudaSuccess) return e;
+  if ((e = prepare_gemm_encoder<EpiGeglu>()) != cudaSuccess) return e;
+  if ((e = prepare_gemm_encoder<EpiCrossKV>()) != cudaSuccess) return e;
 #define PREPSK(BN, EPI) \
   if ((e = prepare_gemm_splitk<BN, EPI>()) != cudaSuccess) return e;
   PREPSK(64, EpiStore) PREPSK(128, EpiStore) PREPSK(64, EpiResidual) PREPSK(128, EpiResidual)
   PREPSK(64, EpiQkvDecode) PREPSK(128, EpiQkvDecode) PREPSK(64, EpiGeglu) PREPSK(128, EpiGeglu)
 #undef PREPSK
-  if ((e = prepare_gemm_2cta<EpiResidual, B200T5_F16 != 0>()) != cudaSuccess) return e;
+#if B200T5_F16
+  if ((e = prepare_gemm_encoder_tf32()) != cudaSuccess) return e;
+#endif
   if ((e = prepare_gemm_splitk<64, EpiResidual, B200T5_F16 != 0>()) != cudaSuccess) return e;
   if ((e = prepare_gemm_splitk<128, EpiResidual, B200T5_F16 != 0>()) != cudaSuccess) return e;
   if ((e = cudaFuncSetAttribute(self_attn_decode_warp_kernel, cudaFuncAttributeMaxDynamicSharedMemorySize,
@@ -515,7 +511,6 @@
   h->use_pdl = pdl_env ? atoi(pdl_env) != 0 : true;
   if (const char* pr_env = getenv("B200T5_PRIO")) h->small_prio = atoi(pr_env);
   if (const char* pk_env = getenv("B200T5_PACK")) h->pack_rows = atoi(pk_env) != 0;
-  if (const char* tc_env = getenv("B200T5_2CTA")) h->use_2cta = atoi(tc_env) != 0;
   if (const char* sf_env = getenv("B200T5_SELF")) h->self_block = strcmp(sf_env, "warp") != 0;
   if (const char* xa_env = getenv("B200T5_XATTN")) h->xattn_mode = strcmp(xa_env, "ldg") == 0 ? 0 : strcmp(xa_env, "stream") == 0 ? 1 : 2;
   if (const char* xs_env = getenv("B200T5_XS_STAGES")) {
@@ -547,7 +542,7 @@
   const char* ch_env = getenv("B200T5_CHAINS");
   h->chains_override = ch_env ? atoi(ch_env) : 0;
 #if B200T5_F16
-  h->use_2cta = h->pack_rows = true;
+  h->pack_rows = true;
   if (!h->sk_on) {
     delete h;
     return fail(nullptr, B200T5_EINVAL, "B200T5_SK=0 is not available in the fp16 build");
@@ -789,14 +784,10 @@
     TRY(interleave_geglu(h, wi0, wi1, w.wi, F, d, 256, &wi_rows));
     if (!(p = take(h, key("layer.1.DenseReluDense.wo.weight"), d, F, &rc))) return rc;
     TRY(build_ffo(h, w.wff_o, key("layer.1.DenseReluDense.wo.weight"), p, d, F, &h->ffo_k));
-    TMAP(h, &w.tm_qkv, w.wqkv.p, 3 * I, d, 256);
-    TMAP(h, &w.tm_o, w.wo.p, d, I, 256);
-    TMAP(h, &w.tm_wi, w.wi.p, wi_rows, d, 256);
-    TMAP_FFO(h, &w.tm_ffo, w.wff_o.p, d, h->ffo_k, 256);
-    TMAP(h, &w.tm2_qkv, w.wqkv.p, 3 * I, d, 128);
-    TMAP(h, &w.tm2_o, w.wo.p, d, I, 128);
-    TMAP(h, &w.tm2_wi, w.wi.p, wi_rows, d, 128);
-    TMAP_FFO(h, &w.tm2_ffo, w.wff_o.p, d, h->ffo_k, 128);
+    TMAP(h, &w.tm_qkv, w.wqkv.p, 3 * I, d, kEncBox);
+    TMAP(h, &w.tm_o, w.wo.p, d, I, kEncBox);
+    TMAP(h, &w.tm_wi, w.wi.p, wi_rows, d, kEncBox);
+    TMAP_FFO(h, &w.tm_ffo, w.wff_o.p, d, h->ffo_k, kEncBox);
   }
 
   CU_OK(h, h->wcrosskv.alloc(static_cast<size_t>(c.Ld) * 2 * I * d * sizeof(act_t)));
@@ -849,8 +840,7 @@
     TMAP(h, &w.tm_wi, w.wi.p, wi_rows, d, bn_wi);
     TMAP_FFO(h, &w.tm_ffo, w.wff_o.p, d, h->ffo_k, bn_ffo);
   }
-  TMAP(h, &h->tm_crosskv, h->wcrosskv.p, static_cast<uint64_t>(c.Ld) * 2 * I, d, 256);
-  TMAP(h, &h->tm2_crosskv, h->wcrosskv.p, static_cast<uint64_t>(c.Ld) * 2 * I, d, 128);
+  TMAP(h, &h->tm_crosskv, h->wcrosskv.p, static_cast<uint64_t>(c.Ld) * 2 * I, d, kEncBox);
 
   h->raw.clear();
   h->raw_f32.clear();
@@ -1010,8 +1000,7 @@
     CU_OK(h, run_rmsnorm(h, p.x.as<res_t>(), w.ln0.as<act_t>(), p.xn.as<act_t>(), M, d, c.eps, s));
     {
       EpiStore::Params ep{p.qkv.as<act_t>(), 3 * I};
-      if (h->use_2cta) CU_OK(h, run_gemm_2cta<EpiStore>(h, p.tm_xn, w.tm2_qkv, M, 3 * I, d, ep, s));
-      else CU_OK(h, run_gemm(h, mk(p.tm_xn, w.tm_qkv, M, 3 * I, d, G_STORE256, 0), &ep, s));
+      CU_OK(h, run_gemm_encoder<EpiStore>(h, p.tm_xn, w.tm_qkv, M, 3 * I, d, ep, s));
     }
     encoder_attn_kernel<<<dim3((S + kEncQ - 1) / kEncQ, B * H), kEncThreads, attn_smem, s>>>(
         p.qkv.as<act_t>(), p.ctx.as<act_t>(), p.enc_bias.as<float>(), p.key_ok.as<unsigned char>(), p.extent.as<int>(), cu, S, H);
@@ -1020,21 +1009,18 @@
     {
       EpiResidual::Params ep{p.x.as<res_t>(), p.x.as<res_t>(), d};
       ep.round_out = l == 0;
-      if (h->use_2cta) CU_OK(h, run_gemm_2cta<EpiResidual>(h, p.tm_ctx, w.tm2_o, M, d, I, ep, s));
-      else CU_OK(h, run_gemm(h, mk(p.tm_ctx, w.tm_o, M, d, I, G_RES256, 0), &ep, s));
+      CU_OK(h, run_gemm_encoder<EpiResidual>(h, p.tm_ctx, w.tm_o, M, d, I, ep, s));
     }
     CU_OK(h, run_rmsnorm(h, p.x.as<res_t>(), w.ln1.as<act_t>(), p.xn.as<act_t>(), M, d, c.eps, s));
     {
       EpiGeglu::Params ep{p.hff.as<ffh_t>(), F, h->gelu_lut};
-      if (h->use_2cta) CU_OK(h, run_gemm_2cta<EpiGeglu>(h, p.tm_xn, w.tm2_wi, M, wi_tiles * 256, d, ep, s));
-      else CU_OK(h, run_gemm(h, mk(p.tm_xn, w.tm_wi, M, wi_tiles * 256, d, G_GEGLU256, 0), &ep, s));
+      CU_OK(h, run_gemm_encoder<EpiGeglu>(h, p.tm_xn, w.tm_wi, M, wi_tiles * 256, d, ep, s));
     }
     {
       EpiResidual::Params ep{p.x.as<res_t>(), p.x.as<res_t>(), d};
       ep.round_acc = B200T5_F16 ? 0 : 1;
       ep.round_out = B200T5_F16 ? 0 : 1;
-      if (h->use_2cta) CU_OK(h, run_ffo_2cta(h, p.tm_hff, w.tm2_ffo, M, d, ep, s));
-      else CU_OK(h, run_gemm(h, mk(p.tm_hff, w.tm_ffo, M, d, F, G_RES256, 0), &ep, s));
+      CU_OK(h, run_ffo_encoder(h, p.tm_hff, w.tm_ffo, M, d, ep, s));
     }
   }
   CU_OK(h, run_rmsnorm(h, p.x.as<res_t>(), h->enc_final_ln.as<act_t>(), p.xn.as<act_t>(), M, d, c.eps, s));
@@ -1050,8 +1036,7 @@
     ep.row_s = p.row_s.as<int>();
   }
   const int M = p.packed ? p.packed_rows : p.B * p.S;
-  if (h->use_2cta) CU_OK(h, run_gemm_2cta<EpiCrossKV>(h, p.tm_xn, h->tm2_crosskv, M, c.Ld * 2 * c.I, c.d, ep, s));
-  else CU_OK(h, run_gemm(h, mk(p.tm_xn, h->tm_crosskv, M, c.Ld * 2 * c.I, c.d, G_CROSSKV256, 0), &ep, s));
+  CU_OK(h, run_gemm_encoder<EpiCrossKV>(h, p.tm_xn, h->tm_crosskv, M, c.Ld * 2 * c.I, c.d, ep, s));
   return B200T5_OK;
 }
 
@@ -1772,45 +1757,43 @@
   if (K % 8) return fail(nullptr, B200T5_EINVAL, "K must be a multiple of 8");
   cudaStream_t s = static_cast<cudaStream_t>(stream);
   CUtensorMap ta, tb;
-  if (!make_tmap(&ta, A, M, K, 128) || !make_tmap(&tb, W, N, K, bn == 512 ? 128 : bn)) return fail(nullptr, B200T5_ECUDA, "%s", g_err);
+  const bool enc = bn == 256 || bn == 512;
+  if (!make_tmap(&ta, A, M, K, 128) || !make_tmap(&tb, W, N, K, enc ? kEncBox : bn)) return fail(nullptr, B200T5_ECUDA, "%s", g_err);
   b200t5_ctx dummy;
   dummy.num_sms = sms;
   cudaError_t e = cudaErrorInvalidValue;
   act_t* Cb = static_cast<act_t*>(C);
-  if (bn == 512) {
+  if (enc) {
     if (mode == 0) {
       EpiStore::Params ep{Cb, N};
-      e = run_gemm_2cta<EpiStore>(&dummy, ta, tb, M, N, K, ep, s);
+      e = run_gemm_encoder<EpiStore>(&dummy, ta, tb, M, N, K, ep, s);
     } else if (mode == 1) {
       EpiResidual::Params ep{Cb, Cb, N};
-      e = run_gemm_2cta<EpiResidual>(&dummy, ta, tb, M, N, K, ep, s);
+      e = run_gemm_encoder<EpiResidual>(&dummy, ta, tb, M, N, K, ep, s);
     } else if (mode == 2) {
       GeluLut lut;
       int lrc = ensure_gelu_lut(nullptr, pow_mode, &lut);
       if (lrc != B200T5_OK) return lrc;
       EpiGeglu::Params ep{Cb, N / 2, lut};
-      e = run_gemm_2cta<EpiGeglu>(&dummy, ta, tb, M, N, K, ep, s);
-    }
-    if (e != cudaSuccess) return fail(nullptr, B200T5_ECUDA, "test_gemm(pair, mode=%d): %s", mode, cudaGetErrorString(e));
+      e = run_gemm_encoder<EpiGeglu>(&dummy, ta, tb, M, N, K, ep, s);
+    }
+    if (e != cudaSuccess) return fail(nullptr, B200T5_ECUDA, "test_gemm(encoder, mode=%d): %s", mode, cudaGetErrorString(e));
     return B200T5_OK;
   }
   if (mode == 0) {
     EpiStore::Params ep{Cb, N};
-    if (bn == 256) e = run_gemm(&dummy, mk(ta, tb, M, N, K, G_STORE256, 0), &ep, s);
-    else if (bn == 32) e = run_gemm(&dummy, mk(ta, tb, M, N, K, G_STORE32, 1), &ep, s);
+    if (bn == 32) e = run_gemm(&dummy, mk(ta, tb, M, N, K, G_STORE32, 1), &ep, s);
     else if (bn == 64) e = launch_gemm<64, EpiStore>(ta, tb, M, N, K, 0, ep, sms, s);
     else if (bn == 128) e = launch_gemm<128, EpiStore>(ta, tb, M, N, K, 0, ep, sms, s);
   } else if (mode == 1) {
     EpiResidual::Params ep{Cb, Cb, N};
-    if (bn == 256) e = run_gemm(&dummy, mk(ta, tb, M, N, K, G_RES256, 0), &ep, s);
-    else if (bn == 32) e = run_gemm(&dummy, mk(ta, tb, M, N, K, G_RES32, 1), &ep, s);
+    if (bn == 32) e = run_gemm(&dummy, mk(ta, tb, M, N, K, G_RES32, 1), &ep, s);
   } else if (mode == 2) {
     GeluLut lut;
     int lrc = ensure_gelu_lut(nullptr, pow_mode, &lut);
     if (lrc != B200T5_OK) return lrc;
     EpiGeglu::Params ep{Cb, N / 2, lut};
-    if (bn == 256) e = run_gemm(&dummy, mk(ta, tb, M, N, K, G_GEGLU256, 0), &ep, s);
-    else if (bn == 64) e = run_gemm(&dummy, mk(ta, tb, M, N, K, G_GEGLU64, 1), &ep, s);
+    if (bn == 64) e = run_gemm(&dummy, mk(ta, tb, M, N, K, G_GEGLU64, 1), &ep, s);
   } else if (mode == 3) {
     EpiStoreF32::Params ep{static_cast<float*>(C), N};
     if (bn == 128) e = run_gemm(&dummy, mk(ta, tb, M, N, K, G_LOGITS128, 1), &ep, s);
@@ -1913,7 +1896,7 @@
   const size_t n = static_cast<size_t>(N) * Fp;
   split_tf32_kernel<<<static_cast<unsigned>((n + 255) / 256), 256, 0, s>>>(static_cast<const float*>(W), wsplit.as<float>(), N, F, Fp);
   CUtensorMap ta, tb;
-  const int box_b = kernel == 0 ? 128 : bn;
+  const int box_b = kernel == 0 ? kEncBox : bn;
   if (!make_tmap(&ta, A, M, F, 128, true) || !make_tmap(&tb, wsplit.p, N, 2 * Fp, box_b, true))
     return fail(nullptr, B200T5_ECUDA, "%s", g_err);
   EpiResidual::Params ep{static_cast<float*>(R), static_cast<const float*>(R), N};
@@ -1921,7 +1904,7 @@
   ep.round_out = 0;
   cudaError_t e;
   if (kernel == 0) {
-    e = launch_gemm_2cta<EpiResidual, true>(ta, tb, M, N, 2 * Fp, ep, sms, s, Fp / 32);
+    e = launch_gemm_encoder_tf32(ta, tb, M, N, 2 * Fp, ep, sms, s, Fp / 32);
   } else {
     const int sp = splitk_factor(2 * Fp, split, kBK / 2);
     e = bn == 128 ? launch_gemm_splitk<128, EpiResidual, true>(ta, tb, M, N, 2 * Fp, sp, ep, s, false, Fp / 32)
diff --git a/anyscale_workshop_nyc_2023_b200/csrc/gemm.cuh b/anyscale_workshop_nyc_2023_b200/csrc/gemm.cuh
--- a/anyscale_workshop_nyc_2023_b200/csrc/gemm.cuh
+++ b/anyscale_workshop_nyc_2023_b200/csrc/gemm.cuh
@@ -198,7 +198,14 @@
 
 struct NoPre {};
 
-template <int BN, class Epi>
+struct StageF32 {
+  static DEVINL void ld32(uint32_t addr, uint32_t (&r)[32]) { acc_ld_32(addr, r); }
+};
+struct StageAct {
+  static DEVINL void ld32(uint32_t addr, uint32_t (&r)[32]) { act_ld_32(addr, r); }
+};
+
+template <int BN, class Epi, class Ld = StageF32>
 DEVINL void run_chunks(const typename Epi::Params& p, uint32_t taddr, int m, bool m_ok, int n_tile, int N,
                                  const uint8_t* epi_smem, int part, int parts) {
   constexpr int C = BN / 32;
@@ -211,7 +218,7 @@
     for (int u = 0; u < 2; ++u) {
       if (c + u < c_hi) {
         uint32_t acc[32];
-        acc_ld_32(taddr + (c + u) * 32, acc);
+        Ld::ld32(taddr + (c + u) * 32, acc);
         const int n0 = n_tile * BN + (c + u) * 32;
         if (m_ok && c + u + 1 < c_hi && n0 + 32 < N) Epi::chunk_pre(p, m, n0 + 32, N, pre[(u + 1) & 1]);
         if (m_ok && n0 < N) Epi::chunk(p, acc, m, n0, N, epi_smem, pre[u & 1]);
@@ -235,10 +242,10 @@
     round_pack_32(acc, o);
     store_row_chunk(p.C + static_cast<size_t>(m) * p.ldc + n0, o, n0, N);
   }
-  template <int BN>
+  template <int BN, class Ld = StageF32>
   static DEVINL void run(const Params& p, uint32_t taddr, int m, bool m_ok, int n_tile, int N, const uint8_t* es,
                          int part, int parts) {
-    run_chunks<BN, EpiStore>(p, taddr, m, m_ok, n_tile, N, es, part, parts);
+    run_chunks<BN, EpiStore, Ld>(p, taddr, m, m_ok, n_tile, N, es, part, parts);
   }
 };
 
@@ -280,10 +287,10 @@
     }
     store_row_chunk_f32(p.C + static_cast<size_t>(m) * p.ld + n0, o, n0, N);
   }
-  template <int BN>
+  template <int BN, class Ld = StageF32>
   static DEVINL void run(const Params& p, uint32_t taddr, int m, bool m_ok, int n_tile, int N, const uint8_t* es,
                          int part, int parts) {
-    run_chunks<BN, EpiResidual>(p, taddr, m, m_ok, n_tile, N, es, part, parts);
+    run_chunks<BN, EpiResidual, Ld>(p, taddr, m, m_ok, n_tile, N, es, part, parts);
   }
 };
 #else
@@ -333,10 +340,10 @@
       p.ss[static_cast<size_t>(m) * p.ss_ld + (n0 >> 5)] = sq;
     }
   }
-  template <int BN>
+  template <int BN, class Ld = StageF32>
   static DEVINL void run(const Params& p, uint32_t taddr, int m, bool m_ok, int n_tile, int N, const uint8_t* es,
                          int part, int parts) {
-    run_chunks<BN, EpiResidual>(p, taddr, m, m_ok, n_tile, N, es, part, parts);
+    run_chunks<BN, EpiResidual, Ld>(p, taddr, m, m_ok, n_tile, N, es, part, parts);
   }
 };
 
@@ -431,7 +438,7 @@
     store_row_chunk(p.out + static_cast<size_t>(m) * p.F + f0, o, f0, p.F);
 #endif
   }
-  template <int BN>
+  template <int BN, class Ld = StageF32>
   static DEVINL void run(const Params& p, uint32_t taddr, int m, bool m_ok, int n_tile, int , const uint8_t* epi_smem,
                          int part, int parts) {
     constexpr int HALF = BN / 2;
@@ -439,8 +446,8 @@
 #pragma unroll 1
     for (int c = part * C / parts; c < (part + 1) * C / parts; ++c) {
       uint32_t g[32], u[32];
-      acc_ld_32(taddr + c * 32, g);
-      acc_ld_32(taddr + HALF + c * 32, u);
+      Ld::ld32(taddr + c * 32, g);
+      Ld::ld32(taddr + HALF + c * 32, u);
       const int f0 = n_tile * HALF + c * 32;
       if (m_ok && f0 < p.F) chunk2(p, g, u, m, f0, epi_smem);
     }
@@ -471,10 +478,10 @@
     act_t* dst = p.arena + ((((static_cast<size_t>(lkv) * p.B + b) * p.H + h) * p.S + s) << 6) + d0;
     store_row_chunk(dst, o, n0, N);
   }
-  template <int BN>
+  template <int BN, class Ld = StageF32>
   static DEVINL void run(const Params& p, uint32_t taddr, int m, bool m_ok, int n_tile, int N, const uint8_t* es,
                          int part, int parts) {
-    run_chunks<BN, EpiCrossKV>(p, taddr, m, m_ok, n_tile, N, es, part, parts);
+    run_chunks<BN, EpiCrossKV, Ld>(p, taddr, m, m_ok, n_tile, N, es, part, parts);
   }
 };
 
@@ -508,10 +515,10 @@
     }
     store_row_chunk(dst, o, n0, N);
   }
-  template <int BN>
+  template <int BN, class Ld = StageF32>
   static DEVINL void run(const Params& p, uint32_t taddr, int m, bool m_ok, int n_tile, int N, const uint8_t* es,
                          int part, int parts) {
-    run_chunks<BN, EpiQkvDecode>(p, taddr, m, m_ok, n_tile, N, es, part, parts);
+    run_chunks<BN, EpiQkvDecode, Ld>(p, taddr, m, m_ok, n_tile, N, es, part, parts);
   }
 };
 
diff --git a/anyscale_workshop_nyc_2023_b200/csrc/gemm_2cta.cuh b/anyscale_workshop_nyc_2023_b200/csrc/gemm_2cta.cuh
--- a/anyscale_workshop_nyc_2023_b200/csrc/gemm_2cta.cuh
+++ /dev/null
@@ -1,20 +0,0 @@
-#pragma once
-#include "gemm.cuh"
-
-namespace b200 {
-
-constexpr int k2ctaBN = 256;
-constexpr int k2ctaBox = 128;
-
-template <class Epi, bool kTf32 = false>
-cudaError_t prepare_gemm_2cta() {
-  return prepare_gemm<k2ctaBN, Epi, kTf32, k2ctaBox>();
-}
-
-template <class Epi, bool kTf32 = false>
-cudaError_t launch_gemm_2cta(const CUtensorMap& tmA, const CUtensorMap& tmB, int M, int N, int K,
-                             const typename Epi::Params& ep, int num_sms, cudaStream_t stream, int a_kblocks = 0) {
-  return launch_gemm<k2ctaBN, Epi, kTf32, k2ctaBox>(tmA, tmB, M, N, K, 0, ep, num_sms, stream, false, a_kblocks);
-}
-
-}
diff --git a/anyscale_workshop_nyc_2023_b200/csrc/gemm_encoder.cuh b/anyscale_workshop_nyc_2023_b200/csrc/gemm_encoder.cuh
--- /dev/null
+++ b/anyscale_workshop_nyc_2023_b200/csrc/gemm_encoder.cuh
@@ -0,0 +1,206 @@
+#pragma once
+#include "gemm.cuh"
+
+namespace b200 {
+
+constexpr int kEncBN = 256;
+constexpr int kEncBox = 128;
+constexpr int kGemmEncThreads = 384;
+constexpr int kEncEpiThreads = 96;
+constexpr int kEncEpiParts = 3;
+
+struct GemmEncCfg {
+  static constexpr int kABytes = kBM * kBK * 2;
+  static constexpr int kBBytes = kEncBN * kBK * 2;
+  static constexpr int kStageBytes = kABytes + kBBytes;
+  static constexpr int kStages = 3;
+  static constexpr int kRingBytes = kStages * kStageBytes;
+  static constexpr int kStageLd = kEncBN + 8;
+  static constexpr int kStagingBytes = kBM * kStageLd * 2;
+  static constexpr int kSmemBytes = kRingBytes + kStagingBytes + 1024  + 256  + kEpiSmemBytes;
+  static_assert(kSmemBytes <= 227 * 1024, "shared memory");
+};
+
+DEVINL void stage_act(act_t* stg, int row0, const float (&acc)[kEncBN / 2]) {
+  const int t = threadIdx.x & 127;
+  const int r = row0 + 16 * (t >> 5) + ((t & 31) >> 2);
+  const int c = 2 * (t & 3);
+#pragma unroll
+  for (int j = 0; j < kEncBN / 8; ++j) {
+    *reinterpret_cast<uint32_t*>(stg + r * GemmEncCfg::kStageLd + 8 * j + c) = pack_act2(acc[4 * j], acc[4 * j + 1]);
+    *reinterpret_cast<uint32_t*>(stg + (r + 8) * GemmEncCfg::kStageLd + 8 * j + c) = pack_act2(acc[4 * j + 2], acc[4 * j + 3]);
+  }
+}
+
+template <class Epi>
+__global__ void __launch_bounds__(kGemmEncThreads, 1)
+gemm_encoder_kernel(const __grid_constant__ CUtensorMap tmA, const __grid_constant__ CUtensorMap tmB, int M, int N,
+                    int K, typename Epi::Params ep) {
+  using Cfg = GemmEncCfg;
+  extern __shared__ uint8_t smem_raw[];
+  uint8_t* smem = reinterpret_cast<uint8_t*>((reinterpret_cast<uintptr_t>(smem_raw) + 1023) & ~uintptr_t(1023));
+  act_t* stg = reinterpret_cast<act_t*>(smem + Cfg::kRingBytes);
+  uint64_t* bars = reinterpret_cast<uint64_t*>(smem + Cfg::kRingBytes + Cfg::kStagingBytes);
+  uint64_t* full = bars;
+  uint64_t* empty = bars + Cfg::kStages;
+  uint64_t* stg_full = bars + 2 * Cfg::kStages;
+  uint64_t* stg_empty = stg_full + 1;
+  uint8_t* epi_smem = smem + Cfg::kRingBytes + Cfg::kStagingBytes + 256;
+
+  const int warp = threadIdx.x >> 5;
+  const uint32_t rank = cluster_ctarank();
+  const int tiles_m = (M + kBM - 1) / kBM;
+  const int tiles_n = (N + kEncBN - 1) / kEncBN;
+  const int num_units = ((tiles_m + 1) / 2) * tiles_n;
+  const int first = blockIdx.x / 2, step = gridDim.x / 2;
+  const int kblocks = (K + kBK - 1) / kBK;
+
+  pdl_launch_dependents();
+  if (threadIdx.x == 0) {
+    for (int i = 0; i < Cfg::kStages; ++i) {
+      mbar_init(&full[i], 1);
+      mbar_init(&empty[i], 4);
+    }
+    mbar_init(stg_full, kGemmConsumers);
+    mbar_init(stg_empty, kEncEpiThreads);
+    mbar_fence_init();
+  }
+  cluster_arrive_release();
+  cluster_wait_acquire();
+
+  if (warp == 8) {
+    if (threadIdx.x == 8 * 32) {
+      tma_prefetch_desc(&tmA);
+      tma_prefetch_desc(&tmB);
+      const int bh = static_cast<int>(rank) * kEncBox;
+      if (first < num_units) {
+        const int n0 = (first % tiles_n) * kEncBN;
+        for (int kb = 0; kb < kblocks; ++kb) tma_prefetch_l2_2d(&tmB, kb * kBK, n0 + bh);
+      }
+      pdl_wait();
+      int stage = 0;
+      uint32_t phase = 0;
+      for (int unit = first; unit < num_units; unit += step) {
+        const int m_tile = min(2 * (unit / tiles_n) + static_cast<int>(rank), tiles_m - 1);
+        const int m0 = m_tile * kBM, n0 = (unit % tiles_n) * kEncBN;
+        for (int kb = 0; kb < kblocks; ++kb) {
+          mbar_wait(&empty[stage], phase ^ 1u);
+          uint8_t* sA = smem + stage * Cfg::kStageBytes;
+          uint8_t* sB = sA + Cfg::kABytes;
+          mbar_arrive_expect_tx(&full[stage], Cfg::kStageBytes);
+          tma_load_2d(sA, &tmA, &full[stage], kb * kBK, m0);
+          tma_load_2d_multicast(sB + bh * 128, &tmB, &full[stage], kb * kBK, n0 + bh, 0x3);
+          if (++stage == Cfg::kStages) {
+            stage = 0;
+            phase ^= 1u;
+          }
+        }
+      }
+    }
+  } else if (warp > 8) {
+    const int et = threadIdx.x - 9 * 32;
+    Epi::prologue(ep, epi_smem, et, kEncEpiThreads);
+    pdl_wait();
+    const uint32_t stg_h = smem_u32(stg) >> 1;
+    uint32_t phase = 0;
+    for (int unit = first; unit < num_units; unit += step) {
+      const int m0 = (2 * (unit / tiles_n) + static_cast<int>(rank)) * kBM;
+      mbar_wait(stg_full, phase);
+      phase ^= 1u;
+#pragma unroll 1
+      for (int piece = et; piece < kBM * kEncEpiParts; piece += kEncEpiThreads) {
+        const int row = piece & (kBM - 1), part = piece / kBM;
+        Epi::template run<kEncBN, StageAct>(ep, stg_h + static_cast<uint32_t>(row * Cfg::kStageLd), m0 + row,
+                                            m0 + row < M, unit % tiles_n, N, epi_smem, part, kEncEpiParts);
+      }
+      mbar_arrive(stg_empty);
+    }
+  } else {
+    const int wg = warp >> 2;
+    const bool leader = (threadIdx.x & 127) == 0;
+    auto release = [&](int s) {
+      mbar_arrive(&empty[s]);
+      mbar_arrive_cluster(mapa_shared(smem_u32(&empty[s]), rank ^ 1u));
+    };
+    int stage = 0;
+    uint32_t phase = 0, sphase = 0;
+    for (int unit = first; unit < num_units; unit += step) {
+      float acc[kEncBN / 2];
+#pragma unroll
+      for (int i = 0; i < kEncBN / 2; ++i) acc[i] = 0.f;
+      int prev = -1;
+      for (int kb = 0; kb < kblocks; ++kb) {
+        mbar_wait(&full[stage], phase);
+        const uint32_t a_addr = smem_u32(smem + stage * Cfg::kStageBytes) + wg * 64 * 128;
+        wgmma_fence_acc(acc);
+        wgmma_fence();
+        wgmma_kblock<kEncBN, false>(acc, a_addr, smem_u32(smem + stage * Cfg::kStageBytes + Cfg::kABytes));
+        wgmma_commit();
+        wgmma_wait<1>();
+        wgmma_fence_acc(acc);
+        if (prev >= 0 && leader) release(prev);
+        prev = stage;
+        if (++stage == Cfg::kStages) {
+          stage = 0;
+          phase ^= 1u;
+        }
+      }
+      wgmma_wait<0>();
+      wgmma_fence_acc(acc);
+      if (prev >= 0 && leader) release(prev);
+      mbar_wait(stg_empty, sphase ^ 1u);
+      sphase ^= 1u;
+      stage_act(stg, wg * 64, acc);
+      mbar_arrive(stg_full);
+    }
+  }
+  __syncwarp();
+  cluster_arrive_release();
+  cluster_wait_acquire();
+}
+
+template <class Epi>
+cudaError_t prepare_gemm_encoder() {
+  return cudaFuncSetAttribute(gemm_encoder_kernel<Epi>, cudaFuncAttributeMaxDynamicSharedMemorySize, GemmEncCfg::kSmemBytes);
+}
+
+template <class Epi>
+cudaError_t launch_gemm_encoder(const CUtensorMap& tmA, const CUtensorMap& tmB, int M, int N, int K,
+                                const typename Epi::Params& ep, cudaStream_t stream) {
+  cudaLaunchConfig_t cfg{};
+  cfg.blockDim = dim3(kGemmEncThreads);
+  cfg.dynamicSmemBytes = GemmEncCfg::kSmemBytes;
+  cfg.stream = stream;
+  cudaLaunchAttribute attr[1];
+  attr[0].id = cudaLaunchAttributeClusterDimension;
+  attr[0].val.clusterDim.x = 2;
+  attr[0].val.clusterDim.y = 1;
+  attr[0].val.clusterDim.z = 1;
+  cfg.attrs = attr;
+  cfg.numAttrs = 1;
+  static int max_clusters = 0;
+  if (max_clusters == 0) {
+    int dev = 0, sms = 0;
+    cudaError_t e = cudaGetDevice(&dev);
+    if (e == cudaSuccess) e = cudaDeviceGetAttribute(&sms, cudaDevAttrMultiProcessorCount, dev);
+    if (e != cudaSuccess) return e;
+    cfg.gridDim = dim3(sms & ~1);
+    e = cudaOccupancyMaxActiveClusters(&max_clusters, gemm_encoder_kernel<Epi>, &cfg);
+    if (e != cudaSuccess) return e;
+    if (max_clusters < 1) return cudaErrorInvalidConfiguration;
+  }
+  const int units = ((M + 2 * kBM - 1) / (2 * kBM)) * ((N + kEncBN - 1) / kEncBN);
+  cfg.gridDim = dim3(2 * (units < max_clusters ? units : max_clusters));
+  return cudaLaunchKernelEx(&cfg, gemm_encoder_kernel<Epi>, tmA, tmB, M, N, K, ep);
+}
+
+#if B200T5_F16
+inline cudaError_t prepare_gemm_encoder_tf32() { return prepare_gemm<kEncBN, EpiResidual, true, kEncBox>(); }
+
+inline cudaError_t launch_gemm_encoder_tf32(const CUtensorMap& tmA, const CUtensorMap& tmB, int M, int N, int K,
+                                            const EpiResidual::Params& ep, int num_sms, cudaStream_t stream, int a_kblocks) {
+  return launch_gemm<kEncBN, EpiResidual, true, kEncBox>(tmA, tmB, M, N, K, 0, ep, num_sms, stream, false, a_kblocks);
+}
+#endif
+
+}
diff --git a/anyscale_workshop_nyc_2023_b200/csrc/gemm_splitk.cuh b/anyscale_workshop_nyc_2023_b200/csrc/gemm_splitk.cuh
--- a/anyscale_workshop_nyc_2023_b200/csrc/gemm_splitk.cuh
+++ b/anyscale_workshop_nyc_2023_b200/csrc/gemm_splitk.cuh
@@ -22,28 +22,6 @@
   }
   static constexpr int kMaxSmemBytes = smem_bytes(kSkMaxStages, true);
 };
-
-DEVINL uint32_t cluster_ctarank() {
-  uint32_t r;
-  asm volatile("mov.u32 %0, %%cluster_ctarank;" : "=r"(r));
-  return r;
-}
-DEVINL uint32_t cluster_nctarank() {
-  uint32_t r;
-  asm volatile("mov.u32 %0, %%cluster_nctarank;" : "=r"(r));
-  return r;
-}
-DEVINL void cluster_arrive_relaxed() { asm volatile("barrier.cluster.arrive.relaxed.aligned;" ::: "memory"); }
-DEVINL void cluster_arrive_release() { asm volatile("barrier.cluster.arrive.release.aligned;" ::: "memory"); }
-DEVINL void cluster_wait_acquire() { asm volatile("barrier.cluster.wait.acquire.aligned;" ::: "memory"); }
-DEVINL uint32_t mapa_shared(uint32_t cta_addr, uint32_t rank) {
-  uint32_t r;
-  asm volatile("mapa.shared::cluster.u32 %0, %1, %2;" : "=r"(r) : "r"(cta_addr), "r"(rank));
-  return r;
-}
-DEVINL void st_cluster_v2(uint32_t addr, float a, float b) {
-  asm volatile("st.shared::cluster.v2.f32 [%0], {%1, %2};" ::"r"(addr), "f"(a), "f"(b) : "memory");
-}
 
 DEVINL void add32_smem(uint32_t (&acc)[32], const float* src) {
   const float4* r4 = reinterpret_cast<const float4*>(src);
diff --git a/anyscale_workshop_nyc_2023_b200/csrc/ptx.cuh b/anyscale_workshop_nyc_2023_b200/csrc/ptx.cuh
--- a/anyscale_workshop_nyc_2023_b200/csrc/ptx.cuh
+++ b/anyscale_workshop_nyc_2023_b200/csrc/ptx.cuh
@@ -69,6 +69,32 @@
   }
 }
 
+DEVINL uint32_t cluster_ctarank() {
+  uint32_t r;
+  asm volatile("mov.u32 %0, %%cluster_ctarank;" : "=r"(r));
+  return r;
+}
+DEVINL uint32_t cluster_nctarank() {
+  uint32_t r;
+  asm volatile("mov.u32 %0, %%cluster_nctarank;" : "=r"(r));
+  return r;
+}
+DEVINL void cluster_arrive_relaxed() { asm volatile("barrier.cluster.arrive.relaxed.aligned;" ::: "memory"); }
+DEVINL void cluster_arrive_release() { asm volatile("barrier.cluster.arrive.release.aligned;" ::: "memory"); }
+DEVINL void cluster_wait_acquire() { asm volatile("barrier.cluster.wait.acquire.aligned;" ::: "memory"); }
+DEVINL uint32_t mapa_shared(uint32_t cta_addr, uint32_t rank) {
+  uint32_t r;
+  asm volatile("mapa.shared::cluster.u32 %0, %1, %2;" : "=r"(r) : "r"(cta_addr), "r"(rank));
+  return r;
+}
+DEVINL void st_cluster_v2(uint32_t addr, float a, float b) {
+  asm volatile("st.shared::cluster.v2.f32 [%0], {%1, %2};" ::"r"(addr), "f"(a), "f"(b) : "memory");
+}
+
+DEVINL void mbar_arrive_cluster(uint32_t cluster_addr) {
+  asm volatile("mbarrier.arrive.release.cluster.shared::cluster.b64 _, [%0];" ::"r"(cluster_addr) : "memory");
+}
+
 DEVINL void fence_proxy_async_smem() { asm volatile("fence.proxy.async.shared::cta;" ::: "memory"); }
 
 DEVINL void tma_prefetch_desc(const CUtensorMap* m) {
@@ -79,6 +105,14 @@
       "cp.async.bulk.tensor.2d.shared::cluster.global.mbarrier::complete_tx::bytes"
       " [%0], [%1, {%3, %4}], [%2];"
       ::"r"(smem_u32(smem_dst)), "l"(reinterpret_cast<uint64_t>(m)), "r"(smem_u32(bar)), "r"(c0), "r"(c1)
+      : "memory");
+}
+DEVINL void tma_load_2d_multicast(void* smem_dst, const CUtensorMap* m, uint64_t* bar, int32_t c0, int32_t c1,
+                                  uint16_t cta_mask) {
+  asm volatile(
+      "cp.async.bulk.tensor.2d.shared::cluster.global.mbarrier::complete_tx::bytes.multicast::cluster"
+      " [%0], [%1, {%3, %4}], [%2], %5;"
+      ::"r"(smem_u32(smem_dst)), "l"(reinterpret_cast<uint64_t>(m)), "r"(smem_u32(bar)), "r"(c0), "r"(c1), "h"(cta_mask)
       : "memory");
 }
 DEVINL void tma_prefetch_l2_2d(const CUtensorMap* m, int32_t c0, int32_t c1) {
@@ -334,6 +368,22 @@
   return *reinterpret_cast<uint32_t*>(&v);
 }
 
+DEVINL void act_ld_32(uint32_t haddr, uint32_t (&r)[32]) {
+#pragma unroll
+  for (int v = 0; v < 4; ++v) {
+    uint32_t w[4];
+    asm volatile("ld.shared.v4.b32 {%0, %1, %2, %3}, [%4];"
+                 : "=r"(w[0]), "=r"(w[1]), "=r"(w[2]), "=r"(w[3])
+                 : "r"((haddr + 8u * v) << 1)
+                 : "memory");
+#pragma unroll
+    for (int i = 0; i < 4; ++i) {
+      r[8 * v + 2 * i] = __float_as_uint(act_lo(w[i]));
+      r[8 * v + 2 * i + 1] = __float_as_uint(act_hi(w[i]));
+    }
+  }
+}
+
 DEVINL uint4 ldg_nc_v4(const void* p) {
   uint4 r;
   asm volatile("ld.global.nc.L1::no_allocate.v4.u32 {%0, %1, %2, %3}, [%4];"
```
